# jnbraun/bcnn

Hardware: AMD Instinct MI355X
Metric: images/sec fwd+bwd (higher is better)
Workload: dtype f32; 1 GPU; ResNet-18 224x224 (BASELINE configs[2]), N=128 per GPU, fwd+bwd+SGD through bcnn_net C API; CIFAR-example topology + ImageNet stem, fc-1000; batch_per_gpu=128, global_batch=128, parallelism=dp1, comm=none (one rank)

## Files before the change

### bcnn_amd/_lib.py

```python
import ctypes as C
import os
import subprocess

_HERE = os.path.dirname(os.path.abspath(__file__))
LIB_PATH = os.environ.get("BCNN_HIP_LIB", os.path.join(_HERE, "lib", "libbcnn_hip.so"))
CSRC = os.path.join(_HERE, "csrc")

vp, i, f, sz, u64 = C.c_void_p, C.c_int, C.c_float, C.c_size_t, C.c_uint64

SIGNATURES = {
    "bcnn_hip_device_count": (i, []),
    "bcnn_hip_set_device": (None, [i]),
    "bcnn_hip_get_device": (i, []),
    "bcnn_hip_device_name": (C.c_char_p, []),
    "bcnn_hip_malloc_f32": (vp, [sz]),
    "bcnn_hip_malloc_i32": (vp, [sz]),
    "bcnn_hip_free": (None, [vp]),
    "bcnn_hip_memcpy_h2d": (None, [vp, vp, sz]),
    "bcnn_hip_memcpy_d2h": (None, [vp, vp, sz]),
    "bcnn_hip_memcpy_d2d": (None, [vp, vp, sz]),
    "bcnn_hip_fill_f32": (None, [vp, sz, f]),
    "bcnn_hip_sync": (None, []),
    "bcnn_hip_stream_create": (vp, []),
    "bcnn_hip_stream_destroy": (None, [vp]),
    "bcnn_hip_set_stream": (None, [vp]),
    "bcnn_hip_get_stream": (vp, []),
    "bcnn_hip_event_create": (vp, []),
    "bcnn_hip_event_destroy": (None, [vp]),
    "bcnn_hip_event_record": (None, [vp]),
    "bcnn_hip_event_sync": (None, [vp]),
    "bcnn_hip_event_elapsed_ms": (f, [vp, vp]),
    "bcnn_hip_profile_enable": (None, [i]),
    "bcnn_hip_profile_reset": (None, []),
    "bcnn_hip_profile_num_classes": (i, []),
    "bcnn_hip_profile_class_name": (C.c_char_p, [i]),
    "bcnn_hip_profile_read": (None, [i, C.POINTER(C.c_double), C.POINTER(C.c_longlong), C.POINTER(C.c_double), C.POINTER(C.c_double)]),
    "bcnn_hip_profile_read_useful_flops": (C.c_double, [i]),
    "bcnn_hip_conv_side_stream_mode": (i, [i]),
    "bcnn_hip_conv_side_join": (None, []),
    "bcnn_hip_trace_enable": (None, [i]),
    "bcnn_hip_trace_read": (C.c_size_t, [C.c_char_p, C.c_size_t]),
    "bcnn_hip_axpy": (None, [sz, f, vp, vp]),
    "bcnn_hip_scal": (None, [sz, f, vp]),
    "bcnn_hip_copy_f32": (None, [sz, vp, vp]),
    "bcnn_hip_add_bias": (None, [vp, vp, i, i, i]),
    "bcnn_hip_grad_bias": (None, [vp, vp, i, i, i]),
    "bcnn_hip_scales": (None, [vp, vp, i, i, i]),
    "bcnn_hip_grad_scales": (None, [vp, vp, i, i, i, vp]),
    "bcnn_hip_gemm": (None, [i, i, i, i, i, f, vp, i, vp, i, f, vp, i]),
    "bcnn_hip_im2col": (None, [vp, i, i, i, i, i, i, vp]),
    "bcnn_hip_col2im": (None, [vp, i, i, i, i, i, i, vp]),
    "bcnn_hip_activation_forward": (None, [vp, sz, i, vp, i, i]),
    "bcnn_hip_activation_backward": (None, [vp, vp, sz, i, vp, vp, i, i]),
    "bcnn_hip_batchnorm_forward": (None, [vp] * 10 + [i, i, i, i, i]),
    "bcnn_hip_batchnorm_backward": (None, [vp, vp, vp, i] + [vp] * 9 + [i, i, i]),
    "bcnn_hip_conv_workspace_size": (sz, [i] * 9),
    "bcnn_hip_conv_forward": (None, [vp, vp, vp, vp] + [i] * 10 + [vp, i, vp, vp, vp, vp, vp, vp, vp, i]),
    "bcnn_hip_conv_forward_bf16": (i, [vp, vp, vp, vp] + [i] * 10 + [vp, i, vp, vp, vp, vp, vp, vp, vp, i]),
    "bcnn_hip_conv_backward": (None, [vp] * 8 + [i] * 10 + [vp, vp, i] + [vp] * 8 + [vp, sz]),
    "bcnn_hip_maxpool_forward": (None, [vp, vp, vp] + [i] * 8),
    "bcnn_hip_maxpool_backward": (None, [vp, vp, vp] + [i] * 9),
    "bcnn_hip_avgpool_forward": (None, [vp, vp, i, i, i, i]),
    "bcnn_hip_avgpool_backward": (None, [vp, vp, i, i, i, i]),
    "bcnn_hip_depthwise_forward": (None, [vp, vp, vp, vp] + [i] * 8),
    "bcnn_hip_depthwise_backward": (None, [vp] * 7 + [i] * 9),
    "bcnn_hip_depthwise_stats_size": (sz, [i] * 7),
    "bcnn_hip_depthwise_forward_stats": (i, [vp, vp, vp, vp] + [i] * 8 + [vp, sz]),
    "bcnn_hip_batchnorm_forward_stats": (None, [vp] * 10 + [i, i, i, i, i, vp, i]),
    "bcnn_hip_batchnorm_forward_stats_only": (None, [vp] * 7 + [i, i, i, vp, i]),
    "bcnn_hip_conv_bnfold_fusable": (i, [i] * 5), "bcnn_hip_conv_set_input_bnfold": (None, [vp] * 4),
    "bcnn_hip_depthwise_bn_fusable": (i, [i] * 8),
    "bcnn_hip_batchnorm_backward_sums": (None, [vp] * 9 + [i, i, i]),
    "bcnn_hip_depthwise_backward_bn": (None, [vp] * 7 + [i] * 9 + [vp] * 5),
    "bcnn_hip_batchnorm_backward_apply": (None, [vp] * 8 + [i, i, i]),
    "bcnn_hip_depthwise_bnin_fusable": (i, [i] * 9),
    "bcnn_hip_conv_bnsums_size": (sz, [i] * 4),
    "bcnn_hip_conv_backward_bnsums": (i, [vp] * 8 + [i] * 10 + [vp, vp, i] + [vp] * 8 + [vp, sz] + [vp, vp, vp, sz]),
    "bcnn_hip_batchnorm_backward_finalize": (None, [vp, i] + [vp] * 6 + [i]),
    "bcnn_hip_depthwise_forward_bnin": (i, [vp, vp, vp, vp] + [i] * 8 + [vp, sz] + [vp] * 4 + [i]),
    "bcnn_hip_depthwise_backward_bnin": (None, [vp] * 7 + [i] * 9 + [vp] * 4 + [i]),
    "bcnn_hip_depthwise_backward_bn_bnin": (None, [vp] * 7 + [i] * 9 + [vp] * 5 + [vp] * 4 + [i]),
    "bcnn_hip_conv_residual_fusable": (i, [i, i, i, i, vp, vp, vp]),
    "bcnn_hip_conv_forward_residual": (None, [vp, vp, vp] + [i] * 9 + [vp] * 7 + [sz, i, vp]),
    "bcnn_hip_conv_backward_residual": (None, [vp] * 7 + [i] * 9 + [vp] * 7 + [vp, sz, vp, vp, i, vp, vp, sz]),
    "bcnn_hip_batchnorm_apply": (None, [vp] * 6 + [i, i, i, i]),
    "bcnn_hip_conv_prepack": (None, [vp, i, i]),
    "bcnn_hip_maxpool_forward_bn_keep": (None, [vp, vp, vp] + [i] * 8 + [vp] * 4 + [i, vp]),
    "bcnn_hip_maxpool_bn_backward_fusable": (i, [i] * 9 + [vp] * 4),
    "bcnn_hip_maxpool_bn_backward": (None, [vp] * 5 + [i] * 8 + [vp] * 8 + [i]),
    "bcnn_hip_conv_backward_bn_done": (None, [vp] * 5 + [i] * 9 + [vp, sz]),
    "bcnn_hip_depthwise_insums_size": (sz, [i] * 7),
    "bcnn_hip_depthwise_backward_bnin_sums": (i, [vp] * 7 + [i] * 9 + [vp] * 5 + [vp] * 4 + [i] + [vp, sz]),
    "bcnn_hip_conv_backward_presummed": (i, [vp] * 8 + [i] * 10 + [vp, vp, i] + [vp] * 8 + [vp, sz] + [vp, i] + [vp, vp, vp, sz]),
    "bcnn_hip_conv_prepack_reset": (None, []),
    "bcnn_hip_conv_prepack_discard": (None, []),
    "bcnn_hip_maxpool_bn_fusable": (i, [i] * 9 + [vp]),
    "bcnn_hip_conv_forward_stats_only": (None, [vp, vp, vp] + [i] * 9 + [vp] * 6),
    "bcnn_hip_maxpool_forward_bn": (None, [vp, vp, vp] + [i] * 8 + [vp] * 4 + [i]),
    "bcnn_hip_sgd_update": (None, [vp, vp, vp, vp, sz, sz, i, f, f, f]),
    "bcnn_hip_sgd_update_chunks": (None, [vp, i, i, f, f, f]),
    "bcnn_hip_zero_chunks": (None, [vp, i]),
    "bcnn_hip_adam_update": (None, [vp, vp, vp, vp, vp, vp, sz, sz, i, i, f, f, f, f, f]),
    "bcnn_hip_eltwise_forward": (None, [vp, vp, vp, sz, sz, i]),
    "bcnn_hip_eltwise_backward": (None, [vp, vp, vp, vp, sz, sz, i, i]),
    "bcnn_hip_cost_metric": (None, [i, vp, vp, vp, i, i, vp]),
    "bcnn_hip_axpy_strided": (None, [i, f, vp, vp] + [i] * 11),
    "bcnn_hip_add_rowvec": (None, [vp, vp, i, i]),
    "bcnn_hip_softmax_forward": (None, [vp, vp, i, i, i]),
    "bcnn_hip_concat_forward": (None, [i, vp, vp, vp, i, i]),
    "bcnn_hip_concat_backward": (None, [i, vp, vp, vp, i, i]),
    "bcnn_hip_upsample_forward": (None, [vp, vp, i, i, i, i, i]),
    "bcnn_hip_upsample_backward": (None, [vp, vp, i, i, i, i, i]),
    "bcnn_hip_yolo_activate": (None, [vp, vp, i, i, i, i, i]),
    "bcnn_hip_yolo_nms_capacity": (i, []),
    "bcnn_hip_yolo_detect_result_words": (sz, [i, i, i]),
    "bcnn_hip_yolo_detect_batch": (i, [vp, i, i, vp, i, i, i, i, f, i, f, i, i, vp]),
    "bcnn_hip_yolo_train_workspace_size": (sz, [vp]),
    "bcnn_hip_yolo_train_forward": (i, [vp, vp, vp, vp, vp, vp, vp]),
    "bcnn_hip_fill_images": (i, [vp, i, i, i, i, i, vp, vp, vp, vp, i, f, i, f, f, f]),
    "bcnn_hip_jpeg_stage_begin": (i, [i, i, i, i, i, vp, i, vp, vp]),
    "bcnn_hip_jpeg_stage_run": (i, [vp, f, i, f, f, f]),
    "bcnn_hip_jpeg_stage_cancel": (None, []),
    "bcnn_hip_augment_batch": (i, [vp, i, i, i, i, i, i, i, vp, vp, vp, i]),
    "bcnn_hip_augment_jpeg_begin": (i, [i, i, i, i, i, vp, vp]),
    "bcnn_hip_augment_jpeg_run": (i, [vp, vp, vp, vp, vp, vp, i]),
    "bcnn_hip_augment_jpeg_cancel": (None, []),
    "bcnn_hip_augment_letterbox_batch": (i, [vp, i, i, i, i, i, vp, vp, vp, i]),
    "bcnn_hip_augment_effects_begin": (i, [i, i, i, vp, vp, vp, vp, i, vp, sz]),
    "bcnn_hip_augment_effects_cancel": (None, []),
    "bcnn_hip_deconv_workspace_size": (sz, [i] * 8),
    "bcnn_hip_deconv_forward": (None, [vp, vp, vp, vp] + [i] * 9),
    "bcnn_hip_deconv_backward": (None, [vp] * 7 + [i] * 9 + [vp, sz]),
    "bcnn_hip_lrn_forward": (None, [vp, vp] + [i] * 5 + [f] * 3),
    "bcnn_hip_lrn_backward": (None, [vp, vp, vp] + [i] * 5 + [f] * 3 + [i]),
    "bcnn_hip_dropout_forward": (None, [vp, sz, f, u64, u64]),
    "bcnn_hip_dropout_backward": (None, [vp, sz, f, u64, u64]),
    "bcnn_hip_lifted_struct_workspace_size": (sz, [i, i]),
    "bcnn_hip_lifted_struct_forward": (None, [vp, vp, vp, i, i, f, i, vp, vp]),
    "bcnn_hip_lifted_struct_backward": (None, [vp, i, i, f, vp]),
    "bcnn_hip_comm_init": (None, [i, i, C.c_char_p]),
    "bcnn_hip_comm_destroy": (None, []),
    "bcnn_hip_comm_retain": (None, []),
    "bcnn_hip_rendezvous_publish": (i, [C.c_char_p, vp, sz, i]),
    "bcnn_hip_rendezvous_fetch": (i, [C.c_char_p, vp, sz, i, i]),
    "bcnn_hip_comm_world": (i, []),
    "bcnn_hip_comm_rank": (i, []),
    "bcnn_hip_allreduce_sum": (None, [vp, sz]),
    "bcnn_hip_broadcast": (None, [vp, sz, i]),
    "bcnn_hip_comm_join": (None, []),
}

_lib = None


def build(verbose=False):
    out = None if verbose else subprocess.DEVNULL
    subprocess.check_call(["make", "-C", CSRC, "-j8"], stdout=out)
    return LIB_PATH


def load():
    global _lib
    if _lib is not None:
        return _lib
    try:
        import torch
    except ImportError:
        pass
    if not os.path.exists(LIB_PATH):
        raise RuntimeError(
            "bcnn_amd: %s is missing -- build it with `python -c 'import __graft_entry__ as g; g.build()'` "
            "(there is no CPU fallback)" % LIB_PATH)
    lib = C.CDLL(LIB_PATH)
    for name, (res, args) in SIGNATURES.items():
        fn = getattr(lib, name)
        fn.restype = res
        fn.argtypes = args
    _lib = lib
    return lib


def declared_symbols():
    import re
    hdr = os.path.join(os.path.dirname(_HERE), "include", "bcnn_hip.h")
    text = open(hdr).read()
    text = re.sub(r"/\*.*?\*/", "", text, flags=re.S)
    return sorted(set(re.findall(r"\b(bcnn_hip_[a-z0-9_]+)\s*\(", text)))
```

### bcnn_amd/csrc/batchnorm.hip

```cpp
#include "chan_reduce.h"
#include "batchnorm.h"
#include "bn_math.h"

namespace bcnn_hip {

#ifdef NT_STORES
#define BN_ST4(p, v) do { typedef float f4_ __attribute__((ext_vector_type(4))); const f4_ t_ = {(v).x, (v).y, (v).z, (v).w}; \
                          __builtin_nontemporal_store(t_, reinterpret_cast<f4_*>(p)); } while (0)
#else
#define BN_ST4(p, v) (*reinterpret_cast<float4*>(p) = (v))
#endif


static float4* bn_consts_scratch(int channels) {
    if (BCNN_EXP_ENV("BCNN_HIP_BN_NO_CONSTS")) return nullptr;
    return scratch_f4(SCRATCH_BN_CONSTS, (size_t)channels * 3);
}
__device__ __forceinline__ void bn_fwd_consts_store(float4* consts, int c, float mean, float var, const float* scale,
                                                    const float* bias) {
    if (!consts) return;
    const BnDiv rs = bn_divisor(sqrtf(var + 0.000001f));
    consts[2 * c] = make_float4(mean, rs.d, rs.r, scale[c]);
    consts[2 * c + 1] = make_float4(bias[c], 0.f, 0.f, 0.f);
}
__device__ __forceinline__ void bn_bwd_consts_store(float4* consts, int c, const float* mean, float var, float sc,
                                                    const float* fwd_bias, float dmean, float dvar, float fM) {
    if (!consts) return;
    const BnDiv rs5 = bn_divisor(sqrtf(var + 0.00001f)), rs6 = bn_divisor(sqrtf(var + 0.000001f));
    consts[3 * c] = make_float4(mean[c], sc, rs5.d, rs5.r);
    consts[3 * c + 1] = make_float4(rs6.d, rs6.r, fwd_bias ? fwd_bias[c] : 0.f, __fdiv_rn(dmean, fM));
    consts[3 * c + 2] = make_float4(dvar, 0.f, 0.f, 0.f);
}

struct StatsF {
    static constexpr int kInFlight = 4;
    const float* x;
    __device__ void operator()(long long off, int, float (&acc)[2]) const {
        const float v = x[off];
        acc[0] += v;
        acc[1] += v * v;
    }
    __device__ void vec4(long long off, int, float (&acc)[2]) const {
        const float4 v = *reinterpret_cast<const float4*>(x + off);
        acc[0] += (v.x + v.y) + (v.z + v.w);
        acc[1] += (v.x * v.x + v.y * v.y) + (v.z * v.z + v.w * v.w);
    }
};

__global__ void bn_stats_finalize_kernel(const float* __restrict__ partials, int C, int splits, int M,
                                         float* __restrict__ saved_mean, float* __restrict__ saved_var,
                                         float* __restrict__ run_mean, float* __restrict__ run_var,
                                         float4* __restrict__ consts, const float* __restrict__ scale,
                                         const float* __restrict__ bias, const float* __restrict__ mean_shift) {
    const int c = blockIdx.x * blockDim.x + threadIdx.x;
    if (c >= C) return;
    double s = 0.0, ss = 0.0;
    for (int i = 0; i < splits; ++i) {
        s += (double)partials[((long long)c * splits + i) * 2 + 0];
        ss += (double)partials[((long long)c * splits + i) * 2 + 1];
    }
    const float inv = 1.0f / (float)M;
    const float mean = __fmul_rn((float)s, inv);
    const float var = __fsub_rn(__fmul_rn((float)ss, inv), __fmul_rn(mean, mean));
    saved_mean[c] = mean;
    saved_var[c] = var;
    const float vis = mean_shift ? __fadd_rn(mean, mean_shift[c]) : mean;
    run_mean[c] = __fadd_rn(__fmul_rn(vis, 0.1f), __fmul_rn(run_mean[c], 0.9f));
    run_var[c] = __fadd_rn(__fmul_rn(var, 0.1f), __fmul_rn(run_var[c], 0.9f));
    bn_fwd_consts_store(consts, c, mean, var, scale, bias);
}

constexpr int kFinalizeThreads = 1024;
__global__ __launch_bounds__(kFinalizeThreads) void bn_stats_finalize_wide_kernel(
    const float* __restrict__ partials, int C, int splits, int M, float* __restrict__ saved_mean,
    float* __restrict__ saved_var, float* __restrict__ run_mean, float* __restrict__ run_var,
    float4* __restrict__ consts, const float* __restrict__ scale, const float* __restrict__ bias,
    const float* __restrict__ mean_shift) {
    constexpr int NW = kFinalizeThreads / 64;
    __shared__ double red[NW][2];
    const int lane = threadIdx.x & 63, wid = threadIdx.x >> 6;
    const int c = blockIdx.x;
    const float2* p = reinterpret_cast<const float2*>(partials) + (long long)c * splits;
    double s = 0.0, ss = 0.0;
    int i = threadIdx.x;
    for (; i + 3 * kFinalizeThreads < splits; i += 4 * kFinalizeThreads) {
        const float2 v0 = p[i], v1 = p[i + kFinalizeThreads], v2 = p[i + 2 * kFinalizeThreads], v3 = p[i + 3 * kFinalizeThreads];
        s += ((double)v0.x + (double)v1.x) + ((double)v2.x + (double)v3.x);
        ss += ((double)v0.y + (double)v1.y) + ((double)v2.y + (double)v3.y);
    }
    for (; i < splits; i += kFinalizeThreads) {
        const float2 v = p[i];
        s += (double)v.x;
        ss += (double)v.y;
    }
#pragma unroll
    for (int o = 32; o > 0; o >>= 1) { s += __shfl_xor(s, o); ss += __shfl_xor(ss, o); }
    if (lane == 0) { red[wid][0] = s; red[wid][1] = ss; }
    __syncthreads();
    if (threadIdx.x != 0) return;
    s = 0.0;
    ss = 0.0;
    for (int w = 0; w < NW; ++w) { s += red[w][0]; ss += red[w][1]; }
    const float inv = 1.0f / (float)M;
    const float mean = __fmul_rn((float)s, inv);
    const float var = __fsub_rn(__fmul_rn((float)ss, inv), __fmul_rn(mean, mean));
    saved_mean[c] = mean;
    saved_var[c] = var;
    const float vis = mean_shift ? __fadd_rn(mean, mean_shift[c]) : mean;
    run_mean[c] = __fadd_rn(__fmul_rn(vis, 0.1f), __fmul_rn(run_mean[c], 0.9f));
    run_var[c] = __fadd_rn(__fmul_rn(var, 0.1f), __fmul_rn(run_var[c], 0.9f));
    bn_fwd_consts_store(consts, c, mean, var, scale, bias);
}

struct BnApplyArgs {
    const float* x;
    float* y;
    float* ws;
    float* xn;
    const float* mean;
    const float* var;
    const float* scale;
    const float* bias;
    int C, HW, predict, act;
    long long total;
    const float* res;
    unsigned res_count;
    int act2;
    const float4* consts;
};

struct BnApplyBody {
    BnApplyArgs a;
    bool al;
    __device__ void operator()(unsigned off, int c, int cnt) const {
        float mean, sc, b;
        BnDiv rs;
        if (a.consts) {
            const float4 k0 = a.consts[2 * c], k1 = a.consts[2 * c + 1];
            mean = k0.x; rs.d = k0.y; rs.r = k0.z; sc = k0.w; b = k1.x;
        } else {
            mean = a.predict ? 0.f : a.mean[c];
            rs = bn_divisor(a.predict ? 1.f : sqrtf(a.var[c] + 0.000001f));
            sc = a.scale[c]; b = a.bias[c];
        }
        const bool side_ws = a.ws && a.ws != a.x, side_xn = a.xn && !a.predict;
        if (cnt == 4 && al && (off & 3u) == 0) {
            const float4 xv = *reinterpret_cast<const float4*>(a.x + off);
            float4 yv, nv;
            yv.x = bn_one(xv.x, mean, rs, sc, b, a.predict, a.act, &nv.x);
            yv.y = bn_one(xv.y, mean, rs, sc, b, a.predict, a.act, &nv.y);
            yv.z = bn_one(xv.z, mean, rs, sc, b, a.predict, a.act, &nv.z);
            yv.w = bn_one(xv.w, mean, rs, sc, b, a.predict, a.act, &nv.w);
            if (side_ws) *reinterpret_cast<float4*>(a.ws + off) = xv;
            if (side_xn) *reinterpret_cast<float4*>(a.xn + off) = nv;
            if (a.res) {
                if (off + 4 <= a.res_count) {
                    const float4 r = *reinterpret_cast<const float4*>(a.res + off);
                    yv.x += r.x; yv.y += r.y; yv.z += r.z; yv.w += r.w;
                } else if (off < a.res_count) {
                    yv.x += a.res[off];
                    if (off + 1 < a.res_count) yv.y += a.res[off + 1];
                    if (off + 2 < a.res_count) yv.z += a.res[off + 2];
                }
                yv.x = act_fwd_cheap(yv.x, a.act2, 0.f); yv.y = act_fwd_cheap(yv.y, a.act2, 0.f);
                yv.z = act_fwd_cheap(yv.z, a.act2, 0.f); yv.w = act_fwd_cheap(yv.w, a.act2, 0.f);
            }
            BN_ST4(a.y + off, yv);
        } else {
            for (int k = 0; k < cnt; ++k) {
                const float xv = a.x[off + k];
                float nv = 0.f;
                float yv = bn_one(xv, mean, rs, sc, b, a.predict, a.act, &nv);
                if (a.res) yv = act_fwd_cheap(yv + (off + k < a.res_count ? a.res[off + k] : 0.f), a.act2, 0.f);
                if (side_ws) a.ws[off + k] = xv;
                if (side_xn) a.xn[off + k] = nv;
                a.y[off + k] = yv;
            }
        }
    }
};

__device__ __forceinline__ float bn_recompute_y(float x, float m, const BnDiv& rs, float sc, float b, int act, const float* res,
                                                unsigned res_count, unsigned long long off) {
    float dummy;
    if (!res) return bn_one(x, m, rs, sc, b, 0, act, &dummy);
    float v = bn_one(x, m, rs, sc, b, 0, BCNN_HIP_ACT_NONE, &dummy);
    if (off < res_count) v += res[off];
    return act_fwd_cheap(v, act, 0.f);
}

struct BwdSumsF {
    static constexpr int kInFlight = 2;
    const float* dy;
    const float* y;
    const float* x;
    const float* mean;
    const float* fwd_bias;
    const float* var;
    const float* scale;
    int act, C, HW;
    const float* res;
    unsigned res_count;
    __device__ float fwd_y(float xv, int c, long long off) const {
        return bn_recompute_y(xv, mean[c], bn_divisor(sqrtf(var[c] + 0.000001f)), scale[c], fwd_bias[c], act, res, res_count,
                              (unsigned long long)off);
    }
    __device__ void operator()(long long off, int c, float (&acc)[2]) const {
        float g = dy[off];
        const float xv = x[off];
        if (act != BCNN_HIP_ACT_NONE) g *= act_bwd_cheap(fwd_bias ? fwd_y(xv, c, off) : y[off], act, 0.f);
        acc[0] += g;
        acc[1] += g * (xv - mean[c]);
    }
    __device__ void vec4(long long off, int c, float (&acc)[2]) const {
        const float m = mean[c];
        float4 g = *reinterpret_cast<const float4*>(dy + off);
        const float4 xv = *reinterpret_cast<const float4*>(x + off);
        if (act != BCNN_HIP_ACT_NONE) {
            float4 yv;
            if (fwd_bias) {
                const BnDiv rs = bn_divisor(sqrtf(var[c] + 0.000001f));
                const float sc = scale[c], b = fwd_bias[c];
                const unsigned long long o = (unsigned long long)off;
                yv.x = bn_recompute_y(xv.x, m, rs, sc, b, act, res, res_count, o);
                yv.y = bn_recompute_y(xv.y, m, rs, sc, b, act, res, res_count, o + 1);
                yv.z = bn_recompute_y(xv.z, m, rs, sc, b, act, res, res_count, o + 2);
                yv.w = bn_recompute_y(xv.w, m, rs, sc, b, act, res, res_count, o + 3);
            } else {
                yv = *reinterpret_cast<const float4*>(y + off);
            }
            g.x *= act_bwd_cheap(yv.x, act, 0.f); g.y *= act_bwd_cheap(yv.y, act, 0.f);
            g.z *= act_bwd_cheap(yv.z, act, 0.f); g.w *= act_bwd_cheap(yv.w, act, 0.f);
        }
        acc[0] += (g.x + g.y) + (g.z + g.w);
        acc[1] += (g.x * (xv.x - m) + g.y * (xv.y - m)) + (g.z * (xv.z - m) + g.w * (xv.w - m));
    }
};

__global__ void bn_bwd_finalize_kernel(const float* __restrict__ partials, int C, int splits,
                                       const float* __restrict__ scale, const float* __restrict__ var,
                                       float* __restrict__ dbias, float* __restrict__ dscales,
                                       float* __restrict__ dmean, float* __restrict__ dvar,
                                       float4* __restrict__ consts, const float* __restrict__ mean,
                                       const float* __restrict__ fwd_bias, float fM) {
    const int c = blockIdx.x * blockDim.x + threadIdx.x;
    if (c >= C) return;
    double s1 = 0.0, s2 = 0.0;
    for (int i = 0; i < splits; ++i) {
        s1 += (double)partials[((long long)c * splits + i) * 2 + 0];
        s2 += (double)partials[((long long)c * splits + i) * 2 + 1];
    }
    const float v = var[c], sc = scale[c];
    dbias[c] += (float)s1;
    dscales[c] += (float)(s2 / (double)sqrtf(v + 0.000001f));
    float md = (float)(s1 * (double)sc);
    float vd = (float)(s2 * (double)sc);
    md *= (-1.0f / sqrtf(v + 0.00001f));
    vd *= -0.5f / (v * sqrtf(v) + 0.00001f);
    dmean[c] = md;
    dvar[c] = vd;
    bn_bwd_consts_store(consts, c, mean, v, sc, fwd_bias, md, vd, fM);
}

__global__ __launch_bounds__(1024) void bn_bwd_finalize_wide_kernel(const float* __restrict__ partials, int C, int splits,
                                                                   const float* __restrict__ scale,
                                                                   const float* __restrict__ var, float* __restrict__ dbias,
                                                                   float* __restrict__ dscales, float* __restrict__ dmean,
                                                                   float* __restrict__ dvar, float4* __restrict__ consts,
                                                                   const float* __restrict__ mean,
                                                                   const float* __restrict__ fwd_bias, float fM) {
    __shared__ double red[16][2];
    const int lane = threadIdx.x & 63, wid = threadIdx.x >> 6, c = blockIdx.x;
    const float2* p = reinterpret_cast<const float2*>(partials) + (long long)c * splits;
    double s1 = 0.0, s2 = 0.0;
    int i = threadIdx.x;
    for (; i + 3 * 1024 < splits; i += 4 * 1024) {
        const float2 v0 = p[i], v1 = p[i + 1024], v2 = p[i + 2048], v3 = p[i + 3072];
        s1 += ((double)v0.x + (double)v1.x) + ((double)v2.x + (double)v3.x);
        s2 += ((double)v0.y + (double)v1.y) + ((double)v2.y + (double)v3.y);
    }
    for (; i < splits; i += 1024) {
        const float2 v = p[i];
        s1 += (double)v.x;
        s2 += (double)v.y;
    }
#pragma unroll
    for (int o = 32; o > 0; o >>= 1) { s1 += __shfl_xor(s1, o); s2 += __shfl_xor(s2, o); }
    if (lane == 0) { red[wid][0] = s1; red[wid][1] = s2; }
    __syncthreads();
    if (threadIdx.x != 0) return;
    s1 = 0.0;
    s2 = 0.0;
    for (int w = 0; w < 16; ++w) { s1 += red[w][0]; s2 += red[w][1]; }
    const float v = var[c], sc = scale[c];
    dbias[c] += (float)s1;
    dscales[c] += (float)(s2 / (double)sqrtf(v + 0.000001f));
    float md = (float)(s1 * (double)sc);
    float vd = (float)(s2 * (double)sc);
    md *= (-1.0f / sqrtf(v + 0.00001f));
    vd *= -0.5f / (v * sqrtf(v) + 0.00001f);
    dmean[c] = md;
    dvar[c] = vd;
    bn_bwd_consts_store(consts, c, mean, v, sc, fwd_bias, md, vd, fM);
}

struct BnBwdApplyArgs {
    float* dy;
    float* dx;
    const float* y;
    const float* x;
    const float* mean;
    const float* var;
    const float* scale;
    const float* dmean;
    const float* dvar;
    const float* fwd_bias;
    int C, HW, act, M;
    long long total;
    int keep_dy;
    const float* res;
    unsigned res_count;
    const float4* consts;
    float rM;
};

struct BnBwdApplyBody {
    BnBwdApplyArgs a;
    bool al;
    __device__ void operator()(unsigned off, int c, int cnt) const {
        const BnDiv fM{(float)a.M, a.rM};
        const bool use_act = a.act != BCNN_HIP_ACT_NONE, use_y = use_act && a.fwd_bias == nullptr;
        float mean, sc, fb, dmm, dv;
        BnDiv rs, rs_fwd;
        if (a.consts) {
            const float4 k0 = a.consts[3 * c], k1 = a.consts[3 * c + 1], k2 = a.consts[3 * c + 2];
            mean = k0.x; sc = k0.y; rs.d = k0.z; rs.r = k0.w;
            rs_fwd.d = k1.x; rs_fwd.r = k1.y; fb = k1.z; dmm = k1.w; dv = k2.x;
        } else {
            mean = a.mean[c]; sc = a.scale[c];
            rs = bn_divisor(sqrtf(a.var[c] + 0.00001f));
            rs_fwd = bn_divisor(use_act && !use_y ? sqrtf(a.var[c] + 0.000001f) : 1.0f);
            fb = a.fwd_bias ? a.fwd_bias[c] : 0.f;
            dmm = __fdiv_rn(a.dmean[c], fM.d); dv = a.dvar[c];
        }
        if (cnt == 4 && al && (off & 3u) == 0) {
            const float4 g = *reinterpret_cast<const float4*>(a.dy + off);
            const float4 xv = *reinterpret_cast<const float4*>(a.x + off);
            float4 yv = make_float4(0.f, 0.f, 0.f, 0.f);
            if (use_y) yv = *reinterpret_cast<const float4*>(a.y + off);
            else if (use_act) {
                yv.x = bn_recompute_y(xv.x, mean, rs_fwd, sc, fb, a.act, a.res, a.res_count, off);
                yv.y = bn_recompute_y(xv.y, mean, rs_fwd, sc, fb, a.act, a.res, a.res_count, off + 1ull);
                yv.z = bn_recompute_y(xv.z, mean, rs_fwd, sc, fb, a.act, a.res, a.res_count, off + 2ull);
                yv.w = bn_recompute_y(xv.w, mean, rs_fwd, sc, fb, a.act, a.res, a.res_count, off + 3ull);
            }
            float4 o;
            o.x = bn_bwd_one(g.x, yv.x, xv.x, mean, rs, sc, dmm, dv, fM, a.act);
            o.y = bn_bwd_one(g.y, yv.y, xv.y, mean, rs, sc, dmm, dv, fM, a.act);
            o.z = bn_bwd_one(g.z, yv.z, xv.z, mean, rs, sc, dmm, dv, fM, a.act);
            o.w = bn_bwd_one(g.w, yv.w, xv.w, mean, rs, sc, dmm, dv, fM, a.act);
            if (!a.keep_dy) BN_ST4(a.dy + off, o);
            if (a.dx) BN_ST4(a.dx + off, o);
        } else {
            for (int k = 0; k < cnt; ++k) {
                const float xk = a.x[off + k];
                const float yk = use_y ? a.y[off + k]
                                       : (use_act ? bn_recompute_y(xk, mean, rs_fwd, sc, fb, a.act, a.res, a.res_count, off + k) : 0.f);
                const float o = bn_bwd_one(a.dy[off + k], yk, xk, mean, rs, sc, dmm, dv, fM, a.act);
                if (!a.keep_dy) a.dy[off + k] = o;
                if (a.dx) a.dx[off + k] = o;
            }
        }
    }
};

void batchnorm_forward_impl(const BnFwdCall& f) {
    const int n = f.e.n, c = f.e.c, hw = f.e.hw, mode = f.mode;
    const long long M = (long long)n * hw, total = M * c;
    if (!total) return;
    const bool have_pre = f.pre && f.pre->splits > 0 && mode == BCNN_HIP_MODE_TRAIN;
    KTimer kt(K_BN_FWD, 0.0, 4.0 * ((have_pre ? 0.0 : 1.0) + (f.stats_only ? 0.0 : 2.0)) * (double)total);
    const int act = act_is_cheap(f.act) ? f.act : BCNN_HIP_ACT_NONE;
    BnApplyArgs a;
    a.x = f.x; a.y = f.y; a.ws = f.workspace; a.xn = f.x_norm; a.scale = f.p.scales; a.bias = f.p.bias;
    a.C = c; a.HW = hw; a.act = act; a.total = total;
    a.res = nullptr; a.res_count = 0; a.act2 = BCNN_HIP_ACT_NONE;
    if (f.res) {
        a.res = f.res->res;
        a.res_count = (unsigned)(f.res->count < (size_t)total ? f.res->count : (size_t)total);
        a.act2 = f.res->act;
    }
    a.predict = (mode == BCNN_HIP_MODE_PREDICT);
    a.mean = f.run.run_mean; a.var = f.run.run_var;
    a.consts = nullptr;
    float4* consts = (mode == BCNN_HIP_MODE_TRAIN && !f.stats_only) ? bn_consts_scratch(c) : nullptr;
    if (mode == BCNN_HIP_MODE_PREDICT) a.ws = nullptr;
    if (mode == BCNN_HIP_MODE_VALID) a.xn = nullptr;
    if (mode == BCNN_HIP_MODE_TRAIN) {
        if (have_pre) {
            bn_stats_finalize_wide_kernel<<<c, kFinalizeThreads, 0, current_stream()>>>(
                f.pre->partials, c, f.pre->splits, (int)M, f.saved_mean, f.saved_var, f.run.run_mean, f.run.run_var, consts,
                f.p.scales, f.p.bias, f.mean_shift);
        } else {
            const int splits = chan_splits(c, M);
            float* part = scratch(SCRATCH_REDUCE, (size_t)c * splits * 2);
            launch_chan_reduce<2>(StatsF{f.x}, c, hw, M, splits, part);
            bn_stats_finalize_kernel<<<ceil_div(c, 256), 256, 0, current_stream()>>>(
                part, c, splits, (int)M, f.saved_mean, f.saved_var, f.run.run_mean, f.run.run_var, consts, f.p.scales, f.p.bias,
                f.mean_shift);
        }
        KERNEL_CHECK();
        a.mean = f.saved_mean; a.var = f.saved_var; a.consts = consts;
    }
    if (f.stats_only) return;
#ifdef BCNN_HIP_EXPERIMENT
    static const int skip_fw = getenv("BCNN_HIP_SKIP_SWEEPS") ? atoi(getenv("BCNN_HIP_SKIP_SWEEPS")) : 0;
    if (!(skip_fw & 4))
#endif
    launch_chan_map(BnApplyBody{a, al16(f.x) && al16(f.y) && al16(a.ws) && al16(a.xn) && al16(a.res)}, n, c, hw);
    if (f.act != act) bcnn_hip_activation_forward(f.y, (size_t)total, f.act, nullptr, hw, c);
}

}

using namespace bcnn_hip;

extern "C" {

void bcnn_hip_batchnorm_forward_stats(const float* x, float* y, float* run_mean, float* run_var, const float* scales,
                                      const float* bias, float* saved_mean, float* saved_var, float* x_norm,
                                      float* workspace, int n, int c, int hw, int mode, int act, const float* stats,
                                      int splits) {
    ConvStats st;
    st.partials = const_cast<float*>(stats); st.splits = stats ? splits : 0; st.capacity = 0;
    BnFwdCall f{};
    f.x = x; f.y = y; f.workspace = workspace; f.x_norm = x_norm; f.mode = mode; f.act = act; f.pre = &st;
    f.e.n = n; f.e.c = c; f.e.hw = hw; f.p.scales = scales; f.p.bias = bias;
    f.saved_mean = saved_mean; f.saved_var = saved_var; f.run.run_mean = run_mean; f.run.run_var = run_var;
    batchnorm_forward_impl(f);
}

void bcnn_hip_batchnorm_forward(const float* x, float* y, float* run_mean, float* run_var,
                                const float* scales, const float* bias, float* saved_mean,
                                float* saved_var, float* x_norm, float* workspace, int n, int c, int hw,
                                int mode, int act) {
    bcnn_hip_batchnorm_forward_stats(x, y, run_mean, run_var, scales, bias, saved_mean, saved_var, x_norm, workspace, n, c, hw,
                                     mode, act, nullptr, 0);
}

void bcnn_hip_batchnorm_forward_stats_only(const float* x, float* run_mean, float* run_var, const float* scales,
                                           const float* bias, float* saved_mean, float* saved_var, int n, int c, int hw,
                                           const float* stats, int splits) {
    ConvStats st;
    st.partials = const_cast<float*>(stats); st.splits = stats ? splits : 0; st.capacity = 0;
    BnFwdCall f{};
    f.x = x; f.mode = BCNN_HIP_MODE_TRAIN; f.act = BCNN_HIP_ACT_NONE; f.pre = &st; f.stats_only = true;
    f.e.n = n; f.e.c = c; f.e.hw = hw; f.p.scales = scales; f.p.bias = bias;
    f.saved_mean = saved_mean; f.saved_var = saved_var; f.run.run_mean = run_mean; f.run.run_var = run_var;
    batchnorm_forward_impl(f);
}

}

namespace bcnn_hip {
void batchnorm_backward_sums(const BnBwdCall& b) {
    const int c = b.e.c, hw = b.e.hw;
    const long long M = (long long)b.e.n * hw;
    const int splits = chan_splits(c, M);
    float* part = scratch(SCRATCH_REDUCE, (size_t)c * splits * 2);
    BwdSumsF f;
    f.dy = b.dout ? b.dout : b.dy; f.y = b.y; f.x = b.workspace; f.mean = b.s.mean; f.act = b.act; f.C = c; f.HW = hw;
    f.fwd_bias = b.p.bias; f.var = b.s.var; f.scale = b.p.scales; f.res = b.res; f.res_count = (unsigned)b.res_count;
#ifdef BCNN_HIP_EXPERIMENT
    static const int skip_exp = getenv("BCNN_HIP_SKIP_C1_SUMS") ? 1 : 0;
    static const int skip_all = getenv("BCNN_HIP_SKIP_SWEEPS") ? atoi(getenv("BCNN_HIP_SKIP_SWEEPS")) : 0;
    if (!(skip_all & 1))
    if (!(skip_exp && b.res == nullptr && b.act == BCNN_HIP_ACT_RELU && ((hw == 3136 && c == 64) || (hw == 784 && c == 128))))
#endif
    launch_chan_reduce<2>(f, c, hw, M, splits, part);
    bn_bwd_finalize_kernel<<<ceil_div(c, 256), 256, 0, current_stream()>>>(part, c, splits, b.p.scales, b.s.var, b.g.dbias,
                                                                          b.g.dscales, b.g.dmean, b.g.dvar, b.consts, b.s.mean,
                                                                          b.p.bias, b.consts_fM > 0.f ? b.consts_fM : (float)M);
    KERNEL_CHECK();
}

static void batchnorm_backward_apply(const BnBwdCall& b) {
    const long long M = (long long)b.e.n * b.e.hw, total = M * b.e.c;
    BnBwdApplyArgs a;
    a.consts = b.consts;
    a.rM = 1.0f / (float)M;
    a.dy = b.dout ? const_cast<float*>(b.dout) : b.dy;
    a.dx = (b.dx && b.dx != a.dy) ? b.dx : nullptr; a.y = b.y; a.x = b.workspace;
    a.mean = b.s.mean; a.var = b.s.var; a.scale = b.p.scales; a.dmean = b.g.dmean; a.dvar = b.g.dvar;
    a.C = b.e.c; a.HW = b.e.hw; a.act = b.act; a.M = (int)M; a.total = total; a.fwd_bias = b.p.bias;
    a.keep_dy = b.dout != nullptr; a.res = b.res; a.res_count = (unsigned)b.res_count;
#ifdef BCNN_HIP_EXPERIMENT
    static const int skip_bw = getenv("BCNN_HIP_SKIP_SWEEPS") ? atoi(getenv("BCNN_HIP_SKIP_SWEEPS")) : 0;
    if (skip_bw & 2) return;
#endif
    launch_chan_map(BnBwdApplyBody{a, al16(a.dy) && al16(a.dx) && al16(b.workspace) && al16(b.y)}, b.e.n, b.e.c, b.e.hw);
}

__global__ __launch_bounds__(256) void bn_residual_grad_kernel(const float* __restrict__ out, const float* __restrict__ dout,
                                                               float* __restrict__ dres, unsigned count, int act) {
    for (unsigned i = blockIdx.x * 256u + threadIdx.x; i < count; i += gridDim.x * 256u)
        dres[i] += dout[i] * act_bwd_cheap(out[i], act, 0.f);
}

void batchnorm_backward_impl(const BnBwdCall& call) {
    BnBwdCall b = call;
    const int c = b.e.c, hw = b.e.hw;
    const long long M = (long long)b.e.n * hw, total = M * c;
    if (!total) return;
    if (!b.dout && (b.act == BCNN_HIP_ACT_NONE || !act_bwd_is_cheap(b.act))) b.p.bias = nullptr;
    const bool reads_y = b.act != BCNN_HIP_ACT_NONE && !b.p.bias;
    KTimer kt(K_BN_BWD, 0.0, 4.0 * (b.dout ? 5.0 : b.sums ? (reads_y ? 4.0 : 3.0) : (reads_y ? 7.0 : 5.0)) * (double)total);
    if (b.dout) {
        b.res_count = b.res_count < (size_t)total ? b.res_count : (size_t)total;
        if (b.dres && b.res_count) {
            bn_residual_grad_kernel<<<stream_grid(b.res_count, 256), 256, 0, current_stream()>>>(b.y, b.dout, b.dres,
                                                                                                 (unsigned)b.res_count, b.act);
            KERNEL_CHECK();
        }
    } else if (!act_bwd_is_cheap(b.act)) {
        bcnn_hip_activation_backward(b.y, b.dy, (size_t)total, b.act, nullptr, nullptr, hw, c);
        b.act = BCNN_HIP_ACT_NONE;
    }
    b.consts = bn_consts_scratch(c);
    if (b.sums) {
        bn_bwd_finalize_wide_kernel<<<c, 1024, 0, current_stream()>>>(b.sums, c, b.splits, b.p.scales, b.s.var, b.g.dbias, b.g.dscales,
                                                                      b.g.dmean, b.g.dvar, b.consts, b.s.mean, b.p.bias, (float)M);
        KERNEL_CHECK();
    } else {
        batchnorm_backward_sums(b);
    }
    batchnorm_backward_apply(b);
}

}

extern "C" {

void bcnn_hip_batchnorm_apply(const float* x, float* y, const float* scales, const float* bias, const float* saved_mean,
                              const float* saved_var, int n, int c, int hw, int act) {
    const long long total = (long long)n * hw * c;
    if (!total) return;
    BnApplyArgs a;
    a.x = x; a.y = y; a.ws = nullptr; a.xn = nullptr; a.scale = scales; a.bias = bias; a.mean = saved_mean; a.var = saved_var;
    a.C = c; a.HW = hw; a.act = act_is_cheap(act) ? act : BCNN_HIP_ACT_NONE; a.total = total; a.predict = 0;
    a.res = nullptr; a.res_count = 0; a.act2 = BCNN_HIP_ACT_NONE; a.consts = nullptr;
    launch_chan_map(BnApplyBody{a, al16(x) && al16(y)}, n, c, hw);
    if (a.act != act) bcnn_hip_activation_forward(y, (size_t)total, act, nullptr, hw, c);
}

void bcnn_hip_batchnorm_backward_finalize(const float* sums, int splits, const float* scales, float* dscales, float* dbias,
                                          const float* saved_var, float* dmean, float* dvar, int c) {
    if (c <= 0 || splits <= 0) return;
    bn_bwd_finalize_wide_kernel<<<c, 1024, 0, current_stream()>>>(sums, c, splits, scales, saved_var, dbias, dscales, dmean,
                                                                  dvar, nullptr, nullptr, nullptr, 1.0f);
    KERNEL_CHECK();
}

void bcnn_hip_batchnorm_backward_sums(const float* dy, const float* scales, float* dscales, float* dbias,
                                      const float* saved_mean, const float* saved_var, float* dmean, float* dvar,
                                      const float* x, int n, int c, int hw) {
    const long long total = (long long)n * hw * c;
    if (!total) return;
    KTimer kt(K_BN_BWD, 0.0, 4.0 * 2.0 * (double)total);
    BnBwdCall b{};
    b.dout = dy; b.workspace = x; b.act = BCNN_HIP_ACT_NONE; b.e.n = n; b.e.c = c; b.e.hw = hw;
    b.p.scales = scales; b.s.mean = saved_mean; b.s.var = saved_var;
    b.g.dscales = dscales; b.g.dbias = dbias; b.g.dmean = dmean; b.g.dvar = dvar;
    batchnorm_backward_sums(b);
}

void bcnn_hip_batchnorm_backward_apply(float* dy, float* dx, const float* scales, const float* saved_mean,
                                       const float* saved_var, const float* dmean, const float* dvar, const float* x,
                                       int n, int c, int hw) {
    if (!(long long)n * hw * c) return;
    BnBwdCall b{};
    b.dy = dy; b.dx = dx; b.workspace = x; b.act = BCNN_HIP_ACT_NONE; b.e.n = n; b.e.c = c; b.e.hw = hw;
    b.p.scales = scales; b.s.mean = saved_mean; b.s.var = saved_var;
    b.g.dmean = const_cast<float*>(dmean); b.g.dvar = const_cast<float*>(dvar);
    batchnorm_backward_apply(b);
}

void bcnn_hip_batchnorm_backward(float* dy, float* dx, const float* y, int act, const float* scales,
                                 float* dscales, float* dbias, const float* saved_mean,
                                 const float* saved_var, float* dmean, float* dvar, const float* x_norm,
                                 const float* workspace, int n, int c, int hw) {
    (void)x_norm;
    BnBwdCall b{};
    b.dy = dy; b.dx = dx; b.y = y; b.workspace = workspace; b.act = act; b.e.n = n; b.e.c = c; b.e.hw = hw;
    b.p.scales = scales; b.s.mean = saved_mean; b.s.var = saved_var;
    b.g.dscales = dscales; b.g.dbias = dbias; b.g.dmean = dmean; b.g.dvar = dvar;
    batchnorm_backward_impl(b);
}

}
```

### bcnn_amd/csrc/next.hip

```cpp
#include <cfloat>

#include "chan_reduce.h"
#include "common.h"

namespace bcnn_hip {

__global__ __launch_bounds__(256) void axpy_strided_kernel(float a, const float* __restrict__ x, float* __restrict__ y,
                                                           int sy, int sx, int xc, int xh, int xw, int yc, int yh,
                                                           int yw, int mc, int mh, int mw, unsigned total) {
    const unsigned gs = gridDim.x * blockDim.x;
    for (unsigned t = blockIdx.x * blockDim.x + threadIdx.x; t < total; t += gs) {
        const unsigned i = t % (unsigned)mw, t1 = t / (unsigned)mw;
        const unsigned j = t1 % (unsigned)mh, t2 = t1 / (unsigned)mh;
        const unsigned k = t2 % (unsigned)mc, n = t2 / (unsigned)mc;
        const size_t di = (size_t)i * sy + (size_t)yw * ((size_t)j * sy + (size_t)yh * ((size_t)yc * n + k));
        const size_t si = (size_t)i * sx + (size_t)xw * ((size_t)j * sx + (size_t)xh * ((size_t)xc * n + k));
        y[di] += a * x[si];
    }
}

__global__ __launch_bounds__(256) void add_rowvec_kernel(float* __restrict__ y, const float* __restrict__ v, int cols,
                                                         unsigned total) {
    const unsigned gs = gridDim.x * blockDim.x;
    for (unsigned t = blockIdx.x * blockDim.x + threadIdx.x; t < total; t += gs) y[t] += v[t % (unsigned)cols];
}

__global__ __launch_bounds__(256) void eltwise_fwd_kernel(const float* __restrict__ a, const float* __restrict__ b,
                                                          float* __restrict__ y, size_t n, size_t b_count, int act) {
    const size_t stride = (size_t)gridDim.x * blockDim.x * 4;
    for (size_t i = ((size_t)blockIdx.x * blockDim.x + threadIdx.x) * 4; i < n; i += stride) {
        if (i + 4 <= n) {
            float4 v = *reinterpret_cast<const float4*>(a + i);
            if (i + 4 <= b_count) {
                const float4 w = *reinterpret_cast<const float4*>(b + i);
                v.x += w.x; v.y += w.y; v.z += w.z; v.w += w.w;
            } else if (i < b_count) {
                if (i < b_count) v.x += b[i];
                if (i + 1 < b_count) v.y += b[i + 1];
                if (i + 2 < b_count) v.z += b[i + 2];
            }
            v.x = act_fwd_cheap(v.x, act, 0.f); v.y = act_fwd_cheap(v.y, act, 0.f);
            v.z = act_fwd_cheap(v.z, act, 0.f); v.w = act_fwd_cheap(v.w, act, 0.f);
            *reinterpret_cast<float4*>(y + i) = v;
        } else {
            for (size_t k = i; k < n; ++k) y[k] = act_fwd_cheap(a[k] + (k < b_count ? b[k] : 0.f), act, 0.f);
        }
    }
}

__global__ __launch_bounds__(256) void eltwise_bwd_kernel(const float* __restrict__ y, float* __restrict__ dy,
                                                          float* __restrict__ da, float* __restrict__ db, size_t n,
                                                          size_t b_count, int act, int overwrite_a) {
    const size_t stride = (size_t)gridDim.x * blockDim.x * 4;
    for (size_t i = ((size_t)blockIdx.x * blockDim.x + threadIdx.x) * 4; i < n; i += stride) {
        if (i + 4 <= n) {
            float4 g = *reinterpret_cast<const float4*>(dy + i);
            if (act != BCNN_HIP_ACT_NONE) {
                const float4 yv = *reinterpret_cast<const float4*>(y + i);
                g.x *= act_bwd_cheap(yv.x, act, 0.f); g.y *= act_bwd_cheap(yv.y, act, 0.f);
                g.z *= act_bwd_cheap(yv.z, act, 0.f); g.w *= act_bwd_cheap(yv.w, act, 0.f);
                *reinterpret_cast<float4*>(dy + i) = g;
            }
            if (da) {
                float4 t = overwrite_a ? make_float4(0.f, 0.f, 0.f, 0.f) : *reinterpret_cast<const float4*>(da + i);
                t.x += g.x; t.y += g.y; t.z += g.z; t.w += g.w;
                *reinterpret_cast<float4*>(da + i) = t;
            }
            if (db && i < b_count) {
                if (i + 4 <= b_count) {
                    float4 t = *reinterpret_cast<const float4*>(db + i);
                    t.x += g.x; t.y += g.y; t.z += g.z; t.w += g.w;
                    *reinterpret_cast<float4*>(db + i) = t;
                } else {
                    db[i] += g.x;
                    if (i + 1 < b_count) db[i + 1] += g.y;
                    if (i + 2 < b_count) db[i + 2] += g.z;
                }
            }
        } else {
            for (size_t k = i; k < n; ++k) {
                float gk = dy[k];
                if (act != BCNN_HIP_ACT_NONE) { gk *= act_bwd_cheap(y[k], act, 0.f); dy[k] = gk; }
                if (da) da[k] = (overwrite_a ? 0.f : da[k]) + gk;
                if (db && k < b_count) db[k] += gk;
            }
        }
    }
}

__global__ __launch_bounds__(256) void softmax_kernel(const float* __restrict__ x, float* __restrict__ y, int C, int HW,
                                                      unsigned total) {
    const int lane = threadIdx.x & 63;
    const unsigned wave = blockIdx.x * 4u + (threadIdx.x >> 6), nwaves = gridDim.x * 4u;
    for (unsigned t = wave; t < total; t += nwaves) {
        const unsigned i = t % (unsigned)HW, n = t / (unsigned)HW;
        const float* px = x + (size_t)n * C * HW + i;
        float* py = y + (size_t)n * C * HW + i;
        float vmax = -FLT_MAX;
        for (int c = lane; c < C; c += 64) vmax = fmaxf(vmax, px[(size_t)c * HW]);
#pragma unroll
        for (int o = 32; o > 0; o >>= 1) vmax = fmaxf(vmax, __shfl_xor(vmax, o));
        double part = 0.0;
        for (int c = lane; c < C; c += 64) part += (double)(float)exp((double)(px[(size_t)c * HW] - vmax));
#pragma unroll
        for (int o = 32; o > 0; o >>= 1) part += __shfl_xor(part, o);
        float sum = (float)part;
        sum = (sum != 0.f) ? vmax + (float)log((double)sum) : vmax - 100.0f;
        for (int c = lane; c < C; c += 64) py[(size_t)c * HW] = (float)exp((double)(px[(size_t)c * HW] - sum));
    }
}

__global__ __launch_bounds__(1024) void cost_metric_kernel(int metric, const float* __restrict__ pred,
                                                           const float* __restrict__ label,
                                                           const float* __restrict__ grad, int B, int per,
                                                           double* __restrict__ partials) {
    __shared__ double red[16];
    const int lane = threadIdx.x & 63, wave = threadIdx.x >> 6;
    const int nrow = 16 * gridDim.x, row0 = blockIdx.x * 16 + wave;
    double acc = 0.0;
    if (metric == 0) {
        for (int i = row0; i < B; i += nrow) {
            const float* row = pred + (size_t)i * per;
            float pm = FLT_MIN;
            int best = 0;
            for (int j = lane; j < per; j += 64)
                if (row[j] > pm) { pm = row[j]; best = j; }
#pragma unroll
            for (int off = 32; off > 0; off >>= 1) {
                const float om = __shfl_xor(pm, off);
                const int ob = __shfl_xor(best, off);
                if (om > pm || (om == pm && ob < best)) { pm = om; best = ob; }
            }
            if (lane == 0 && label[(size_t)i * per + best] == 0) acc += 1.0;
        }
    } else if (metric == 5) {
        for (int i = row0; i < B; i += nrow) {
            int n = 0, d = 0;
            for (int j = lane; j < per; j += 64) {
                const float l = label[(size_t)i * per + j];
                const float t = pred[(size_t)i * per + j] > 0.5f ? 1.f : 0.f;
                n += (int)(l * t);
                d += (int)(l + t);
            }
#pragma unroll
            for (int off = 32; off > 0; off >>= 1) { n += __shfl_xor(n, off); d += __shfl_xor(d, off); }
            if (lane == 0) acc += (2.0f * n + 1.0f) / (d + 1.0f);
        }
    } else {
        const size_t sz = (size_t)B * per;
        for (size_t i = (size_t)blockIdx.x * 1024 + threadIdx.x; i < sz; i += (size_t)gridDim.x * 1024) {
            if (metric == 1) {
                if (label[i] > 0.0f) {
                    float q = pred[i];
                    q = q < 1e-8f ? 1e-8f : (q > 1.0f - 1e-8f ? 1.0f - 1e-8f : q);
                    acc += -log((double)q);
                }
            } else {
                acc += (double)grad[i] * grad[i];
            }
        }
#pragma unroll
        for (int off = 32; off > 0; off >>= 1) acc += __shfl_xor(acc, off);
    }
    if (lane == 0) red[wave] = acc;
    __syncthreads();
    if (threadIdx.x == 0) {
        double t = 0.0;
        for (int w = 0; w < 16; ++w) t += red[w];
        partials[blockIdx.x] = t;
    }
}
__global__ void cost_metric_final_kernel(int metric, const double* __restrict__ partials, int n, int per,
                                         float* __restrict__ out) {
    double t = 0.0;
    for (int i = 0; i < n; ++i) t += partials[i];
    out[0] = (float)(metric == 3 ? t / per : t);
}

}

using namespace bcnn_hip;

extern "C" {

void bcnn_hip_axpy_strided(int num_batches, float a, const float* x, float* y, int stride_y, int stride_x, int x_c,
                           int x_h, int x_w, int y_c, int y_h, int y_w, int min_c, int min_h, int min_w) {
    const long long total = (long long)num_batches * min_c * min_h * min_w;
    if (total <= 0) return;
    axpy_strided_kernel<<<stream_grid((size_t)total, 256), 256, 0, current_stream()>>>(
        a, x, y, stride_y, stride_x, x_c, x_h, x_w, y_c, y_h, y_w, min_c, min_h, min_w, (unsigned)total);
    KERNEL_CHECK();
}

void bcnn_hip_add_rowvec(float* y, const float* v, int rows, int cols) {
    const long long total = (long long)rows * cols;
    if (total <= 0) return;
    add_rowvec_kernel<<<stream_grid((size_t)total, 256), 256, 0, current_stream()>>>(y, v, cols, (unsigned)total);
    KERNEL_CHECK();
}

void bcnn_hip_softmax_forward(const float* x, float* y, int n, int c, int hw) {
    const long long total = (long long)n * hw;
    if (total <= 0) return;
    softmax_kernel<<<stream_grid((size_t)total * 64, 256), 256, 0, current_stream()>>>(x, y, c, hw, (unsigned)total);
    KERNEL_CHECK();
}

static bool aligned16(const void* p) { return p == nullptr || (reinterpret_cast<uintptr_t>(p) & 15) == 0; }

void bcnn_hip_eltwise_forward(const float* a, const float* b, float* y, size_t n, size_t b_count, int act) {
    if (!n) return;
    if (!act_is_cheap(act) || !aligned16(a) || !aligned16(b) || !aligned16(y)) {
        bcnn_hip_copy_f32(n, a, y);
        bcnn_hip_axpy(b_count, 1.0f, b, y);
        bcnn_hip_activation_forward(y, n, act, nullptr, 1, 1);
        return;
    }
    eltwise_fwd_kernel<<<stream_grid(n / 4 + 1, 256), 256, 0, current_stream()>>>(a, b, y, n, b_count, act);
    KERNEL_CHECK();
}

void bcnn_hip_eltwise_backward(const float* y, float* dy, float* da, float* db, size_t n, size_t b_count, int act,
                               int overwrite_a) {
    if (!n) return;
    if (!act_bwd_is_cheap(act) || !aligned16(y) || !aligned16(dy) || !aligned16(da) || !aligned16(db)) {
        bcnn_hip_activation_backward(y, dy, n, act, nullptr, nullptr, 1, 1);
        if (da && overwrite_a) bcnn_hip_fill_f32(da, n, 0.f);
        if (da) bcnn_hip_axpy(n, 1.0f, dy, da);
        if (db) bcnn_hip_axpy(b_count, 1.0f, dy, db);
        return;
    }
    eltwise_bwd_kernel<<<stream_grid(n / 4 + 1, 256), 256, 0, current_stream()>>>(y, dy, da, db, n, b_count, act,
                                                                                   overwrite_a);
    KERNEL_CHECK();
}

void bcnn_hip_cost_metric(int metric, const float* pred, const float* label, const float* grad, int batch, int per,
                          float* out) {
    const long long sz = (long long)batch * per;
    int blocks = (int)((sz + 8191) / 8192);
    if (blocks > 64) blocks = 64;
    if (blocks < 1) blocks = 1;
    double* partials = reinterpret_cast<double*>(scratch(SCRATCH_REDUCE, 2 * 64));
    cost_metric_kernel<<<blocks, 1024, 0, current_stream()>>>(metric, pred, label, grad, batch, per, partials);
    KERNEL_CHECK();
    cost_metric_final_kernel<<<1, 1, 0, current_stream()>>>(metric, partials, blocks, per, out);
    KERNEL_CHECK();
}

}
```

### bcnn_amd/csrc/runtime.hip

```cpp
#include "common.h"

#include <cstring>
#include <vector>

namespace bcnn_hip {
static thread_local hipStream_t g_stream = nullptr;
hipStream_t current_stream() { return g_stream; }
void set_current_stream(hipStream_t st) { g_stream = st; }

int current_device() {
    int dev = 0;
    HIP_CHECK(hipGetDevice(&dev));
    if (dev < 0 || dev >= kMaxDevices) { fprintf(stderr, "[bcnn_hip] device ordinal %d out of range\n", dev); exit(1); }
    return dev;
}

struct ScratchPolicy { size_t min_floats; unsigned grow_num, grow_den; };
static constexpr ScratchPolicy kScratchPolicy[] = {
     {1u << 16, 2, 1},
     {4096 * 4, 2, 1},
     {8192, 2, 1},
     {0, 1, 1},
     {1u << 20, 3, 2},
     {1u << 20, 3, 2},
     {0, 1, 1},
     {0, 1, 1},
     {1u << 20, 1, 1},
     {0, 1, 1},
     {1u << 20, 1, 1},
     {0, 1, 1},
     {1u << 20, 1, 1},
     {0, 1, 1},
     {1u << 16, 1, 1},
     {1u << 18, 5, 4},
     {1u << 18, 1, 1},
};
static_assert(sizeof(kScratchPolicy) / sizeof(kScratchPolicy[0]) == SCRATCH_SLOTS, "one policy row per ScratchSlot");
struct ScratchBlock { float* p = nullptr; size_t cap = 0; };
static thread_local ScratchBlock g_scratch[kMaxDevices][SCRATCH_SLOTS];

float* scratch(ScratchSlot slot, size_t floats) {
    ScratchBlock& b = g_scratch[current_device()][slot];
    if (b.p == nullptr || b.cap < floats) {
        const ScratchPolicy& pol = kScratchPolicy[slot];
        if (b.p) {
            HIP_CHECK(hipDeviceSynchronize());
            HIP_CHECK(hipFree(b.p));
        }
        b.cap = floats < pol.min_floats ? pol.min_floats : floats * pol.grow_num / pol.grow_den;
        HIP_CHECK(hipMalloc((void**)&b.p, b.cap * sizeof(float)));
    }
    return b.p;
}

struct KRecord { int cls; hipEvent_t a, b; double flops, bytes, useful; };
static thread_local bool g_prof_on = false;
static thread_local std::vector<KRecord>* g_records = nullptr;
static thread_local std::vector<hipEvent_t>* g_event_pool = nullptr;
static hipEvent_t pool_event() {
    if (!g_event_pool) g_event_pool = new std::vector<hipEvent_t>();
    if (!g_event_pool->empty()) { hipEvent_t e = g_event_pool->back(); g_event_pool->pop_back(); return e; }
    hipEvent_t e;
    HIP_CHECK(hipEventCreate(&e));
    return e;
}
KTimer::KTimer(int cls, double flops, double bytes, double useful_flops) : idx(-1) {
    if (!g_prof_on) return;
    if (!g_records) g_records = new std::vector<KRecord>();
    KRecord r{cls, pool_event(), pool_event(), flops, bytes, useful_flops < 0 ? flops : useful_flops};
    HIP_CHECK(hipEventRecord(r.a, g_stream));
    idx = (int)g_records->size();
    g_records->push_back(r);
}
KTimer::~KTimer() {
    if (idx >= 0) HIP_CHECK(hipEventRecord((*g_records)[idx].b, g_stream));
}

thread_local bool g_trace_on = false;
static thread_local std::vector<char>* g_trace_log = nullptr;
void trace_kernel_slow(const char* name) {
    if (!g_trace_log) g_trace_log = new std::vector<char>();
    if (g_trace_log->size() > (8u << 20)) return;
    g_trace_log->insert(g_trace_log->end(), name, name + strlen(name));
    g_trace_log->push_back('\n');
}

__global__ void warm_kernel(float* p) { if (p && threadIdx.x == 0) p[0] = 1.0f; }

static void warm_device_keeping_rand_state() {
    static thread_local unsigned long long warmed = 0;
    static thread_local bool any = false;
    int dev = 0;
    if (any) {
        if (hipGetDevice(&dev) != hipSuccess || dev < 0 || dev >= 64 || ((warmed >> dev) & 1ull)) return;
    }
    char scratch_state[256];
    char* user_state = initstate(1u, scratch_state, sizeof(scratch_state));
    void* p = nullptr;
    (void)hipFree(nullptr);
    if (hipGetDevice(&dev) != hipSuccess) dev = 0;
    if (hipMalloc(&p, 256) == hipSuccess) {
        float h = 0.f;
        (void)hipMemsetAsync(p, 0, 256, nullptr);
        warm_kernel<<<1, 64, 0, nullptr>>>((float*)p);
        (void)hipMemcpy(&h, p, sizeof(float), hipMemcpyDeviceToHost);
        (void)hipDeviceSynchronize();
        (void)hipFree(p);
    }
    (void)hipDeviceSynchronize();
    if (user_state) setstate(user_state);
    any = true;
    if (dev >= 0 && dev < 64) warmed |= 1ull << dev;
}

__global__ void fill_f32_kernel(float* __restrict__ x, size_t n, float v) {
    size_t head = ((16 - (reinterpret_cast<uintptr_t>(x) & 15)) & 15) / 4;
    if (head > n) head = n;
    const size_t i = (size_t)blockIdx.x * blockDim.x + threadIdx.x;
    const size_t stride = (size_t)gridDim.x * blockDim.x;
    if (i < head) x[i] = v;
    float* body = x + head;
    const size_t nb = n - head, n4 = nb / 4;
    float4* b4 = reinterpret_cast<float4*>(body);
    const float4 v4 = make_float4(v, v, v, v);
    for (size_t j = i; j < n4; j += stride) b4[j] = v4;
    for (size_t j = n4 * 4 + i; j < nb; j += stride) body[j] = v;
}
}

using namespace bcnn_hip;

extern "C" {

int bcnn_hip_device_count(void) {
    int n = 0;
    if (hipGetDeviceCount(&n) != hipSuccess) return 0;
    return n;
}

void bcnn_hip_set_device(int id) {
    HIP_CHECK(hipSetDevice(id));
    warm_device_keeping_rand_state();
}

int bcnn_hip_get_device(void) {
    int id = 0;
    HIP_CHECK(hipGetDevice(&id));
    return id;
}

const char* bcnn_hip_device_name(void) {
    static thread_local char name[256];
    hipDeviceProp_t prop;
    HIP_CHECK(hipGetDeviceProperties(&prop, bcnn_hip_get_device()));
    snprintf(name, sizeof(name), "%s", prop.gcnArchName);
    return name;
}

float* bcnn_hip_malloc_f32(size_t n) {
    float* p = nullptr;
    if (n == 0) return nullptr;
    warm_device_keeping_rand_state();
    HIP_CHECK(hipMalloc((void**)&p, n * sizeof(float)));
    HIP_CHECK(hipMemsetAsync(p, 0, n * sizeof(float), current_stream()));
    return p;
}

int* bcnn_hip_malloc_i32(size_t n) {
    int* p = nullptr;
    if (n == 0) return nullptr;
    warm_device_keeping_rand_state();
    HIP_CHECK(hipMalloc((void**)&p, n * sizeof(int)));
    HIP_CHECK(hipMemsetAsync(p, 0, n * sizeof(int), current_stream()));
    return p;
}

void bcnn_hip_free(void* p) {
    if (p) HIP_CHECK(hipFree(p));
}

void bcnn_hip_memcpy_h2d(void* dst, const void* src, size_t bytes) {
    HIP_CHECK(hipMemcpyAsync(dst, src, bytes, hipMemcpyHostToDevice, current_stream()));
    HIP_CHECK(hipStreamSynchronize(current_stream()));
}

void bcnn_hip_memcpy_d2h(void* dst, const void* src, size_t bytes) {
    HIP_CHECK(hipMemcpyAsync(dst, src, bytes, hipMemcpyDeviceToHost, current_stream()));
    HIP_CHECK(hipStreamSynchronize(current_stream()));
}

void bcnn_hip_memcpy_d2d(void* dst, const void* src, size_t bytes) {
    HIP_CHECK(hipMemcpyAsync(dst, src, bytes, hipMemcpyDeviceToDevice, current_stream()));
}

void bcnn_hip_fill_f32(float* x, size_t n, float value) {
    if (n == 0) return;
    if (value == 0.0f) {
        HIP_CHECK(hipMemsetAsync(x, 0, n * sizeof(float), current_stream()));
        return;
    }
    fill_f32_kernel<<<stream_grid(n / 4 + 1, 256), 256, 0, current_stream()>>>(x, n, value);
    KERNEL_CHECK();
}

void bcnn_hip_sync(void) { HIP_CHECK(hipStreamSynchronize(current_stream())); }

void* bcnn_hip_stream_create(void) {
    hipStream_t s;
    warm_device_keeping_rand_state();
    int prio_lo = 0, prio_hi = 0;
    HIP_CHECK(hipDeviceGetStreamPriorityRange(&prio_lo, &prio_hi));
    HIP_CHECK(hipStreamCreateWithPriority(&s, hipStreamNonBlocking, prio_hi));
    return (void*)s;
}

void bcnn_hip_stream_destroy(void* stream) {
    if (stream) HIP_CHECK(hipStreamDestroy((hipStream_t)stream));
}

void bcnn_hip_set_stream(void* stream) { g_stream = (hipStream_t)stream; }
void* bcnn_hip_get_stream(void) { return (void*)g_stream; }

void* bcnn_hip_event_create(void) {
    hipEvent_t e;
    HIP_CHECK(hipEventCreate(&e));
    return (void*)e;
}

void bcnn_hip_event_destroy(void* ev) {
    if (ev) HIP_CHECK(hipEventDestroy((hipEvent_t)ev));
}

void bcnn_hip_event_record(void* ev) { HIP_CHECK(hipEventRecord((hipEvent_t)ev, current_stream())); }
void bcnn_hip_event_sync(void* ev) { HIP_CHECK(hipEventSynchronize((hipEvent_t)ev)); }

float bcnn_hip_event_elapsed_ms(void* start, void* stop) {
    float ms = 0.f;
    HIP_CHECK(hipEventElapsedTime(&ms, (hipEvent_t)start, (hipEvent_t)stop));
    return ms;
}

void bcnn_hip_profile_enable(int on) { g_prof_on = (on != 0); }

void bcnn_hip_profile_reset(void) {
    if (!g_records) return;
    HIP_CHECK(hipStreamSynchronize(current_stream()));
    for (auto& r : *g_records) { g_event_pool->push_back(r.a); g_event_pool->push_back(r.b); }
    g_records->clear();
}

int bcnn_hip_profile_num_classes(void) { return K_NUM; }

const char* bcnn_hip_profile_class_name(int cls) {
    static const char* names[K_NUM] = {"conv_fwd", "conv_dw", "conv_dx", "bn_fwd", "bn_bwd", "pool",
                                       "eltwise_act", "gemm", "sgd", "depthwise_fwd", "depthwise_bwd",
                                       "conv_fwd_winograd", "conv_dx_winograd", "conv_dw_winograd",
                                       "conv_fwd_winograd43", "conv_dx_winograd43", "conv_dw_winograd43"};
    return (cls >= 0 && cls < K_NUM) ? names[cls] : "?";
}

void bcnn_hip_profile_read(int cls, double* ms, long long* launches, double* flops, double* bytes) {
    double t = 0, f = 0, b = 0;
    long long n = 0;
    if (g_records) {
        HIP_CHECK(hipStreamSynchronize(current_stream()));
        for (auto& r : *g_records) {
            if (r.cls != cls) continue;
            float e = 0.f;
            HIP_CHECK(hipEventElapsedTime(&e, r.a, r.b));
            t += e; f += r.flops; b += r.bytes; ++n;
        }
    }
    if (ms) *ms = t;
    if (launches) *launches = n;
    if (flops) *flops = f;
    if (bytes) *bytes = b;
}

void bcnn_hip_trace_enable(int on) {
    g_trace_on = (on != 0);
    if (on && g_trace_log) g_trace_log->clear();
}

size_t bcnn_hip_trace_read(char* buf, size_t cap) {
    const size_t len = g_trace_log ? g_trace_log->size() : 0;
    if (buf && cap > 0) {
        const size_t n = len < cap - 1 ? len : cap - 1;
        if (n) memcpy(buf, g_trace_log->data(), n);
        buf[n] = 0;
    }
    return len;
}

double bcnn_hip_profile_read_useful_flops(int cls) {
    double u = 0;
    if (g_records)
        for (auto& r : *g_records)
            if (r.cls == cls) u += r.useful;
    return u;
}

}
```

### bcnn_amd/host/bcnn_core.c

```c
#include <math.h>
#include <stdarg.h>
#include <string.h>

#include "bcnn_internal.h"
#include "../../include/bcnn_hip.h"

#ifndef BCNN_USE_HIP
#error "this runtime is the device build: compile with -DBCNN_USE_HIP"
#endif

void bcnn_log(bcnn_log_context ctx, bcnn_log_level level, const char *fmt, ...) {
    if (level < ctx.lvl) return;
    char msg[2048];
    va_list ap;
    va_start(ap, fmt);
    vsnprintf(msg, sizeof(msg), fmt, ap);
    va_end(ap);
    if (ctx.fct) {
        ctx.fct("%s", msg);
        return;
    }
    static const char *tag[] = {"[INFO] ", "[WARNING] ", "[ERROR] ", ""};
    fprintf(stderr, "%s%s", tag[level > 3 ? 3 : level], msg);
}
// ... 101 lines not shown

static bcnn_hip_context *hctx(bcnn_net *net) { return (bcnn_hip_context *)net->hip_ctx; }

bcnn_status bcnn_net_add_tensor(bcnn_net *net, bcnn_tensor tensor) {
    bcnn_tensor *p = (bcnn_tensor *)realloc(net->tensors, (size_t)(net->num_tensors + 1) * sizeof(bcnn_tensor));
    if (!p) return BCNN_FAILED_ALLOC;
    net->tensors = p;
    net->tensors[net->num_tensors++] = tensor;
    return BCNN_SUCCESS;
}

static void invalidate_sgd_table(bcnn_net *net) {
    bcnn_hip_context *hc = hctx(net);
    if (!hc) return;
    if (hc->sgd_chunks_gpu) {
        bcnn_hip_sync();
        bcnn_hip_free(hc->sgd_chunks_gpu);
        hc->sgd_chunks_gpu = NULL;
    }
    hc->num_sgd_chunks = 0;
    if (hc->fill_chunks_gpu) {
        bcnn_hip_sync();
        bcnn_hip_free(hc->fill_chunks_gpu);
        hc->fill_chunks_gpu = NULL;
    }
    hc->num_fill_chunks = -1;
}

static void relink_graph(bcnn_net *net);

bcnn_status bcnn_net_add_node(bcnn_net *net, bcnn_node node) {
    bcnn_hip_context *hc = hctx(net);
    if (hc && hc->compiled) {
        bcnn_materialize_data(net, -1);
        bcnn_materialize_gradients(net, -1);
    }
    bcnn_node *p = (bcnn_node *)realloc(net->nodes, (size_t)(net->num_nodes + 1) * sizeof(bcnn_node));
    if (!p) return BCNN_FAILED_ALLOC;
    net->nodes = p;
    net->nodes[net->num_nodes++] = node;
    invalidate_sgd_table(net);
    if (hc) {
        free(hc->node_grad_first);
        hc->node_grad_first = NULL;
        if (hc->compiled) relink_graph(net);
        else hc->grad_fill_count = 0;
    }
    return BCNN_SUCCESS;
}

static bcnn_status push_index(int **arr, int *count, int index) {
    int *p = (int *)realloc(*arr, (size_t)(*count + 1) * sizeof(int));
    if (!p) return BCNN_FAILED_ALLOC;
    p[(*count)++] = index;
    *arr = p;
    return BCNN_SUCCESS;
}

bcnn_status bcnn_node_add_input(bcnn_net *net, bcnn_node *node, int index) {
    (void)net;
    return push_index(&node->src, &node->num_src, index);
}

bcnn_status bcnn_node_add_output(bcnn_net *net, bcnn_node *node, int index) {
    (void)net;
    return push_index(&node->dst, &node->num_dst, index);
}

int bcnn_net_find_tensor(bcnn_net *net, const char *name) {
    for (int i = net->num_tensors - 1; i >= 0; --i)
        if (net->tensors[i].name && strcmp(net->tensors[i].name, name) == 0) return i;
    return -1;
}

void bcnn_net_register_param(bcnn_net *net, int index) {
    bcnn_hip_context *hc = hctx(net);
    push_index(&hc->param_ids, &hc->num_params, index);
}

bcnn_status bcnn_init_net(bcnn_net **net, bcnn_mode mode) {
    bcnn_net *p = (bcnn_net *)calloc(1, sizeof(bcnn_net));
    if (!p) return BCNN_FAILED_ALLOC;
    p->mode = mode;
    p->hip_ctx = calloc(1, sizeof(bcnn_hip_context));
    if (!p->hip_ctx) { free(p); return BCNN_FAILED_ALLOC; }
    hctx(p)->dp_world = 1;
    hctx(p)->num_fill_chunks = -1;
    bcnn_tensor in = {0}, lab = {0};
    in.name = dup_name("input");
    lab.name = dup_name("label");
    bcnn_net_add_tensor(p, in);
    bcnn_net_add_tensor(p, lab);
    if (mode != BCNN_MODE_PREDICT) {
        p->learner = (bcnn_learner *)calloc(1, sizeof(bcnn_learner));
        p->data_aug = (bcnn_data_augmenter *)calloc(1, sizeof(bcnn_data_augmenter));
    }
    p->num_inputs = 1;
    p->inputs = (int *)calloc(1, sizeof(int));
    p->num_threads = 1;
    *net = p;
    return BCNN_SUCCESS;
}

void bcnn_end_net(bcnn_net **pnet) {
    bcnn_net *net = *pnet;
    if (!net) return;
    bcnn_hip_sync();
    bcnn_hip_conv_prepack_reset();
    bcnn_hip_context *hc = hctx(net);
    if (hc->comm_active) bcnn_hip_comm_destroy();
    if (hc->compiled) {
        for (int i = 0; i < hc->arena_members; ++i) {
            bcnn_tensor *t = &net->tensors[hc->param_ids[i]];
            t->data_gpu = NULL;
            t->grad_data_gpu = NULL;
        }
        bcnn_hip_free(hc->param_arena_gpu);
        bcnn_hip_free(hc->grad_arena_gpu);
        bcnn_hip_free(hc->sgd_chunks_gpu);
        bcnn_hip_free(hc->fill_chunks_gpu);
        free(hc->sgd_chunks_host);
        free(hc->grad_fill_dead);
        free(hc->node_grad_first);
    }
    for (int i = 0; i < net->num_nodes; ++i) {
        bcnn_node *nd = &net->nodes[i];
        if (nd->release_param) nd->release_param(nd);
        free(nd->src); free(nd->dst); free(nd->param);
    }
    free(net->nodes);
    for (int i = 0; i < net->num_tensors; ++i) bcnn_tensor_destroy(&net->tensors[i]);
    free(net->tensors);
    bcnn_hip_free(hc->workspace_gpu);
    bcnn_free_loader_stage(net);
    free(hc->param_ids);
    free(hc);
    free(net->learner); free(net->data_aug); bcnn_destroy_data_loader(net); free(net->inputs);
    free(net);
    *pnet = NULL;
}

bcnn_status bcnn_set_num_threads(bcnn_net *net, int num_threads, const int *cpu_ids) {
    (void)cpu_ids;
    net->num_threads = num_threads > 0 ? num_threads : 1;
    return BCNN_SUCCESS;
}
int bcnn_get_num_threads(bcnn_net *net) { return net->num_threads; }
int bcnn_get_batch_size(bcnn_net *net) { return net->batch_size; }

void bcnn_set_input_shape(bcnn_net *net, int width, int height, int channels, int batch_size) {
    net->batch_size = batch_size;
    bcnn_tensor_set_shape(&net->tensors[0], batch_size, channels, height, width, 0);
}

bcnn_status bcnn_add_input(bcnn_net *net, int width, int height, int channels, const char *name) {
    bcnn_tensor t = {0};
    bcnn_tensor_set_shape(&t, net->batch_size, channels, height, width, 0);
    BCNN_CHECK_STATUS(bcnn_tensor_allocate(&t, net->mode));
    t.name = dup_name(name);
    BCNN_CHECK_STATUS(bcnn_net_add_tensor(net, t));
    int *p = (int *)realloc(net->inputs, (size_t)(net->num_inputs + 1) * sizeof(int));
    if (!p) return BCNN_FAILED_ALLOC;
    net->inputs = p;
    net->inputs[net->num_inputs++] = net->num_tensors - 1;
    return BCNN_SUCCESS;
}

static void build_arenas(bcnn_net *net) {
    bcnn_hip_context *hc = hctx(net);
    size_t total = 0;
    for (int i = 0; i < hc->num_params; ++i) {
        total += ((size_t)bcnn_tensor_size(&net->tensors[hc->param_ids[i]]) + 3) & ~(size_t)3;
    }
    if (total == 0) return;
    float *old_p = hc->param_arena_gpu, *old_g = hc->grad_arena_gpu;
    float *new_p = bcnn_hip_malloc_f32(total);
    float *new_g = (net->mode != BCNN_MODE_PREDICT) ? bcnn_hip_malloc_f32(total) : NULL;
    size_t off = 0;
    for (int i = 0; i < hc->num_params; ++i) {
        bcnn_tensor *t = &net->tensors[hc->param_ids[i]];
        const size_t sz = (size_t)bcnn_tensor_size(t);
        const int member = i < hc->arena_members;
        bcnn_hip_memcpy_d2d(new_p + off, t->data_gpu, sz * sizeof(float));
        bcnn_hip_sync();
        if (!member) bcnn_hip_free(t->data_gpu);
        t->data_gpu = new_p + off;
        if (new_g && t->grad_data_gpu) {
            bcnn_hip_memcpy_d2d(new_g + off, t->grad_data_gpu, sz * sizeof(float));
            bcnn_hip_sync();
            if (!member) bcnn_hip_free(t->grad_data_gpu);
            t->grad_data_gpu = new_g + off;
        }
        off += (sz + 3) & ~(size_t)3;
    }
    bcnn_hip_free(old_p);
    bcnn_hip_free(old_g);
    hc->param_arena_gpu = new_p;
    hc->grad_arena_gpu = new_g;
    hc->arena_size = total;
    hc->arena_members = hc->num_params;
}

static void mark_dead_grad_fills(bcnn_net *net) {
    bcnn_hip_context *hc = hctx(net);
    free(hc->grad_fill_dead);
    hc->grad_fill_dead = (unsigned char *)calloc((size_t)net->num_tensors + 1, 1);
    hc->grad_fill_count = net->num_tensors;
    if (BCNN_EXP_ENV("BCNN_KEEP_ALL_GRAD_FILLS")) return;
    for (int t = 0; t < net->num_tensors; ++t) {
        int first = -1, uses = 0;
        for (int i = 0; i < net->num_nodes; ++i)
            for (int k = 0; k < net->nodes[i].num_src; ++k)
                if (net->nodes[i].src[k] == t) {
                    if (first < 0) first = i;
                    ++uses;
                }
        if (first < 0) continue;
        int lifted_src = 0;
        for (int i = 0; i < net->num_nodes; ++i)
            lifted_src |= net->nodes[i].type == BCNN_LAYER_COST && net->nodes[i].src[0] == t &&
                          ((const bcnn_cost_param *)net->nodes[i].param)->loss == BCNN_LOSS_LIFTED_STRUCT;
        if (lifted_src) continue;
        const bcnn_node *nd = &net->nodes[first];
        if (nd->src[0] != t) continue;
        if (uses == 1 && (nd->type == BCNN_LAYER_MAXPOOL || nd->type == BCNN_LAYER_DEPTHWISE_CONV2D ||
                          nd->type == BCNN_LAYER_LRN)) {
            hc->grad_fill_dead[t] = 2;
            continue;
        }
        if (uses == 1 && nd->type == BCNN_LAYER_ELTWISE) {
            const bcnn_eltwise_param *ep = (const bcnn_eltwise_param *)nd->param;
            if (ep->stride[0] == 1 && ep->stride[1] == 1 &&
                bcnn_tensor_size(&net->tensors[t]) == bcnn_tensor_size(&net->tensors[nd->dst[0]]))
                hc->grad_fill_dead[t] = 2;
            continue;
        }
        if (nd->type == BCNN_LAYER_BATCHNORM) {
            hc->grad_fill_dead[t] = 1;
            continue;
        }
        if (nd->type != BCNN_LAYER_CONV2D) continue;
        const bcnn_conv_param *p = (const bcnn_conv_param *)nd->param;
        const bcnn_tensor *x = &net->tensors[t], *y = &net->tensors[nd->dst[0]];
        if (p->size == 1 && y->h * y->w != x->h * x->w) continue;
        hc->grad_fill_dead[t] = 1;
    }
}

int bcnn_grad_sole_writer(bcnn_net *net, int tensor) {
    const bcnn_hip_context *hc = hctx(net);
    return hc->grad_fill_dead && tensor >= 0 && tensor < hc->grad_fill_count && hc->grad_fill_dead[tensor] == 2;
}

static void comm_sync_parameters(bcnn_net *net);

bcnn_status bcnn_compile_net(bcnn_net *net) {
    bcnn_hip_context *hc = hctx(net);
    BCNN_CHECK_STATUS(bcnn_tensor_allocate(&net->tensors[0], net->mode));
    size_t need = 0;
    for (int i = 0; i < net->num_nodes; ++i) {
        if (net->nodes[i].type != BCNN_LAYER_CONV2D) continue;
        bcnn_conv_param *p = (bcnn_conv_param *)net->nodes[i].param;
        const bcnn_tensor *s = &net->tensors[net->nodes[i].src[0]];
        const size_t ws = bcnn_hip_conv_workspace_size(s->n, s->c, s->h, s->w, p->num, p->size, p->stride, p->pad,
                                                       p->num_groups);
        if (ws > need) need = ws;
    }
    if (need > hc->workspace_size) {
        bcnn_hip_free(hc->workspace_gpu);
        hc->workspace_gpu = bcnn_hip_malloc_f32(need);
        hc->workspace_size = need;
    }
    for (int i = 0; i < net->num_nodes; ++i)
        if (net->nodes[i].type == BCNN_LAYER_CONV2D)
            ((bcnn_conv_param *)net->nodes[i].param)->conv_workspace_gpu = hc->workspace_gpu;
    if (!hc->compiled || hc->num_params != hc->arena_members) {
        invalidate_sgd_table(net);
        build_arenas(net);
        hc->compiled = 1;
        if (hc->grad_ready_fn) bcnn_set_gradient_ready_callback(net, hc->grad_ready_fn, hc->grad_ready_user);
        comm_sync_parameters(net);
    }
    relink_graph(net);
    bcnn_hip_sync();
    return BCNN_SUCCESS;
}

static void relink_graph(bcnn_net *net) {
    bcnn_hip_context *hc = hctx(net);
    mark_dead_grad_fills(net);
    for (int i = 0; i < net->num_nodes; ++i) {
        if (net->nodes[i].type != BCNN_LAYER_CONV2D) continue;
        const int t = net->nodes[i].dst[0];
        int rewritten = 0;
        for (int j = 0; j < net->num_nodes; ++j)
            rewritten |= net->nodes[j].type == BCNN_LAYER_DROPOUT && net->nodes[j].dst[0] == t;
        ((bcnn_conv_param *)net->nodes[i].param)->out_rewritten = rewritten;
    }
    bcnn_link_depthwise_batchnorm(net);
    bcnn_link_conv_eltwise(net);
    bcnn_link_conv_maxpool(net);
    bcnn_link_conv_depthwise(net);
    bcnn_link_batchnorm_conv(net);
    if (hc->fill_chunks_gpu) {
        bcnn_hip_sync();
        bcnn_hip_free(hc->fill_chunks_gpu);
        hc->fill_chunks_gpu = NULL;
    }
    hc->num_fill_chunks = -1;
}

static bcnn_status resize_private_f32(float **buf, size_t old_elems, size_t new_elems, int need_realloc) {
    if (!*buf || new_elems <= old_elems) return BCNN_SUCCESS;
    if (!need_realloc) return BCNN_INVALID_PARAMETER;
    bcnn_hip_sync();
    bcnn_hip_free(*buf);
    *buf = bcnn_hip_malloc_f32(new_elems);
    return *buf ? BCNN_SUCCESS : BCNN_FAILED_ALLOC;
}

bcnn_status bcnn_resize_net(bcnn_net *net, int w, int h, int c, int need_realloc) {
    if (!net || w <= 0 || h <= 0 || c <= 0) return BCNN_INVALID_PARAMETER;
    for (int i = 0; i < net->num_nodes; ++i) {
        const bcnn_layer_type t = net->nodes[i].type;
        BCNN_CHECK_AND_LOG(net->log_ctx, t != BCNN_LAYER_CONCAT && t != BCNN_LAYER_UPSAMPLE && t != BCNN_LAYER_YOLOV3 &&
                                             t != BCNN_LAYER_TRANSPOSE_CONV2D,
                           BCNN_INVALID_PARAMETER,
                           "bcnn_resize_net: node %d is a concat / upsample / YOLO / deconvolution node, whose resize is "
                           "not supported\n", i);
        BCNN_CHECK_AND_LOG(net->log_ctx,
                           t != BCNN_LAYER_COST || ((const bcnn_cost_param *)net->nodes[i].param)->loss != BCNN_LOSS_LIFTED_STRUCT,
                           BCNN_INVALID_PARAMETER,
                           "bcnn_resize_net: node %d is a lifted-structure cost node, whose resize is not supported\n", i);
    }
    bcnn_set_input_shape(net, w, h, c, 1);
    for (int i = 0; i < net->num_nodes; ++i) {
        bcnn_node *nd = &net->nodes[i];
        if (nd->num_src < 1 || nd->num_dst < 1) continue;
        if (nd->type == BCNN_LAYER_DROPOUT) continue;
        const bcnn_tensor *s = &net->tensors[nd->src[0]];
        bcnn_tensor *d = &net->tensors[nd->dst[0]];
        const size_t old_elems = (size_t)bcnn_tensor_size(d);
        if (nd->type == BCNN_LAYER_CONV2D) {
            const bcnn_conv_param *p = (const bcnn_conv_param *)nd->param;
            bcnn_tensor_set_shape(d, s->n, p->num, (s->h + 2 * p->pad - p->size) / p->stride + 1,
                                  (s->w + 2 * p->pad - p->size) / p->stride + 1, 1);
        } else if (nd->type == BCNN_LAYER_MAXPOOL) {
            const bcnn_maxpool_param *p = (const bcnn_maxpool_param *)nd->param;
            bcnn_tensor_set_shape(d, s->n, s->c, (s->h - 1) / p->stride + 1, (s->w - 1) / p->stride + 1, 1);
        } else {
            bcnn_tensor_set_shape(d, s->n, s->c, s->h, s->w, 1);
        }
        if (need_realloc) BCNN_CHECK_STATUS(bcnn_tensor_allocate(d, net->mode));
        const size_t new_elems = (size_t)bcnn_tensor_size(d);
        if (nd->type == BCNN_LAYER_CONV2D) {
            bcnn_conv_param *p = (bcnn_conv_param *)nd->param;
            BCNN_CHECK_STATUS(resize_private_f32(&p->bn_workspace_gpu, old_elems, new_elems, need_realloc));
            BCNN_CHECK_STATUS(resize_private_f32(&p->x_norm_gpu, old_elems, new_elems, need_realloc));
        } else if (nd->type == BCNN_LAYER_BATCHNORM) {
            bcnn_batchnorm_param *p = (bcnn_batchnorm_param *)nd->param;
            BCNN_CHECK_STATUS(resize_private_f32(&p->workspace_gpu, old_elems, new_elems, need_realloc));
            BCNN_CHECK_STATUS(resize_private_f32(&p->x_norm_gpu, old_elems, new_elems, need_realloc));
        } else if (nd->type == BCNN_LAYER_MAXPOOL && new_elems > old_elems) {
            bcnn_maxpool_param *p = (bcnn_maxpool_param *)nd->param;
            if (!need_realloc) return BCNN_INVALID_PARAMETER;
            bcnn_hip_sync();
            bcnn_hip_free(p->indexes_gpu);
            p->indexes_gpu = bcnn_hip_malloc_i32(new_elems);
            int *host = (int *)realloc(p->indexes, new_elems * sizeof(int));
            if (!host || !p->indexes_gpu) return BCNN_FAILED_ALLOC;
            p->indexes = host;
            if (p->raw_at_max_gpu) {
                bcnn_hip_free(p->raw_at_max_gpu);
                p->raw_at_max_gpu = NULL;
            }
        }
    }
    if (hctx(net)->compiled) return bcnn_compile_net(net);
    return BCNN_SUCCESS;
}

bcnn_status bcnn_set_mode(bcnn_net *net, bcnn_mode mode) {
    if (net->mode == mode) return BCNN_SUCCESS;
    if (mode == BCNN_MODE_TRAIN && !hctx(net)->detector_training)
        for (int i = 0; i < net->num_nodes; ++i)
            BCNN_CHECK_AND_LOG(net->log_ctx, net->nodes[i].type != BCNN_LAYER_YOLOV3, BCNN_INVALID_PARAMETER,
                               "bcnn_set_mode: the net holds a YOLO node, whose TRAIN-mode loss is not built\n");
    if (mode == BCNN_MODE_TRAIN)
        BCNN_CHECK_AND_LOG(net->log_ctx, bcnn_yolo_heads_trainable(net), BCNN_INVALID_PARAMETER,
                           "bcnn_set_mode: a YOLO node was built without detector training or has no gradient buffer\n");
    net->mode = mode;
    if (net->data_loader) bcnn_switch_data_handles(net, net->data_loader);
    return BCNN_SUCCESS;
}

static void build_fill_table(bcnn_net *net) {
    bcnn_hip_context *hc = hctx(net);
    int cap = 256, n = 0;
    bcnn_hip_fill_chunk *tab = (bcnn_hip_fill_chunk *)malloc((size_t)cap * sizeof(*tab));
    unsigned char *seen = (unsigned char *)calloc((size_t)net->num_tensors + 1, 1);
    for (int i = 0; i < net->num_nodes; ++i)
        for (int d = 0; d < net->nodes[i].num_dst; ++d) {
            const int id = net->nodes[i].dst[d];
            bcnn_tensor *t = &net->tensors[id];
            if (seen[id] || !t->grad_data_gpu) continue;
            seen[id] = 1;
            if (hc->grad_fill_dead && id < hc->grad_fill_count && hc->grad_fill_dead[id]) continue;
            const size_t sz = (size_t)bcnn_tensor_size(t);
            for (size_t off = 0; off < sz; off += BCNN_HIP_FILL_CHUNK) {
                if (n == cap) {
                    cap *= 2;
                    tab = (bcnn_hip_fill_chunk *)realloc(tab, (size_t)cap * sizeof(*tab));
                }
                tab[n].p_d = t->grad_data_gpu + off;
                tab[n].count = (unsigned int)((sz - off < BCNN_HIP_FILL_CHUNK) ? (sz - off) : BCNN_HIP_FILL_CHUNK);
                tab[n].reserved = 0;
                ++n;
            }
        }
    free(seen);
    hc->num_fill_chunks = n;
    if (n > 0) {
        hc->fill_chunks_gpu = bcnn_hip_malloc_f32(((size_t)n * sizeof(*tab) + 3) / 4);
        bcnn_hip_memcpy_h2d(hc->fill_chunks_gpu, tab, (size_t)n * sizeof(*tab));
    }
    free(tab);
}

void bcnn_forward(bcnn_net *net) {
    bcnn_hip_context *hc = hctx(net);
    if (net->mode == BCNN_MODE_TRAIN) {
        if (hc->num_fill_chunks < 0) build_fill_table(net);
        bcnn_hip_zero_chunks((const bcnn_hip_fill_chunk *)hc->fill_chunks_gpu, hc->num_fill_chunks);
    }
    bcnn_drop_pending_gradients(net);
    bcnn_prepack_conv_weights(net, 0);
    hc->in_pass = 1;
    for (int i = 0; i < net->num_nodes; ++i) net->nodes[i].forward(net, &net->nodes[i]);
    hc->in_pass = 0;
    bcnn_hip_conv_prepack_discard();
}

static void comm_flush(bcnn_hip_context *hc) {
    if (hc->comm_lo < hc->comm_hi) {
        bcnn_hip_allreduce_sum(hc->grad_arena_gpu + hc->comm_lo, hc->comm_hi - hc->comm_lo);
        hc->comm_hi = hc->comm_lo;
    }
}

static void comm_on_ready(size_t first, size_t count, void *user) {
    bcnn_hip_context *hc = (bcnn_hip_context *)user;
    (void)count;
    hc->comm_lo = first;
    if (hc->comm_hi - hc->comm_lo >= hc->comm_bucket) comm_flush(hc);
}

void bcnn_backward(bcnn_net *net) {
    bcnn_hip_context *hc = hctx(net);
    size_t ready_from = hc->arena_size;
    if (hc->comm_active) hc->comm_lo = hc->comm_hi = hc->arena_size;
    bcnn_prepack_conv_weights(net, 1);
    hc->in_pass = 2;
    const int side_prev = bcnn_hip_conv_side_stream_mode((hc->no_side_stream || BCNN_EXP_ENV("BCNN_NO_SIDE_STREAM")) ? 0 : 2);
    for (int i = net->num_nodes - 1; i >= 0; --i) {
        net->nodes[i].backward(net, &net->nodes[i]);
        if (hc->grad_ready_fn && hc->node_grad_first && hc->node_grad_first[i] < ready_from) {
            bcnn_hip_conv_side_join();
            hc->grad_ready_fn(hc->node_grad_first[i], ready_from - hc->node_grad_first[i], hc->grad_ready_user);
            ready_from = hc->node_grad_first[i];
        }
    }
    hc->in_pass = 0;
    bcnn_hip_conv_side_join();
    bcnn_hip_conv_side_stream_mode(side_prev);
    bcnn_hip_conv_prepack_discard();
    if (hc->grad_ready_fn && ready_from > 0 && hc->arena_size > 0)
        hc->grad_ready_fn(0, ready_from, hc->grad_ready_user);
    if (hc->comm_active) {
        comm_flush(hc);
        bcnn_hip_comm_join();
    }
}

void bcnn_set_weight_gradient_stream(bcnn_net *net, int enable) { hctx(net)->no_side_stream = enable ? 0 : 1; }

bcnn_status bcnn_set_inference_precision(bcnn_net *net, bcnn_precision p) {
    if (!net || (p != BCNN_PRECISION_FP32 && p != BCNN_PRECISION_BF16)) return BCNN_INVALID_PARAMETER;
    hctx(net)->inference_precision = (int)p;
    return BCNN_SUCCESS;
}

bcnn_precision bcnn_get_inference_precision(const bcnn_net *net) {
    return (bcnn_precision)((const bcnn_hip_context *)net->hip_ctx)->inference_precision;
}

bcnn_status bcnn_set_loader_on_device(bcnn_net *net, int on) {
    if (!net) return BCNN_INVALID_PARAMETER;
    hctx(net)->loader_on_device = on ? 1 : 0;
    return BCNN_SUCCESS;
}

int bcnn_get_loader_on_device(const bcnn_net *net) {
    return net ? ((const bcnn_hip_context *)net->hip_ctx)->loader_on_device : 0;
}

bcnn_status bcnn_set_loader_decode_on_device(bcnn_net *net, int on) {
    if (!net) return BCNN_INVALID_PARAMETER;
    hctx(net)->loader_decode_on_device = on ? 1 : 0;
    return BCNN_SUCCESS;
}

int bcnn_get_loader_decode_on_device(const bcnn_net *net) {
    return net ? ((const bcnn_hip_context *)net->hip_ctx)->loader_decode_on_device : 0;
}

int bcnn_get_loader_device_decoded(const bcnn_net *net) {
    return net ? ((const bcnn_hip_context *)net->hip_ctx)->loader_device_decoded : 0;
}

bcnn_status bcnn_set_loader_detection_on_device(bcnn_net *net, int on) {
    if (!net) return BCNN_INVALID_PARAMETER;
    hctx(net)->loader_detection_on_device = on ? 1 : 0;
    return BCNN_SUCCESS;
}

int bcnn_get_loader_detection_on_device(const bcnn_net *net) {
    return net ? ((const bcnn_hip_context *)net->hip_ctx)->loader_detection_on_device : 0;
}

int bcnn_get_loader_device_letterboxed(const bcnn_net *net) {
    return net ? ((const bcnn_hip_context *)net->hip_ctx)->loader_device_letterboxed : 0;
}

bcnn_status bcnn_set_loader_effects(bcnn_net *net, int on) {
    if (!net) return BCNN_INVALID_PARAMETER;
    hctx(net)->loader_effects = on ? 1 : 0;
    return BCNN_SUCCESS;
}

int bcnn_get_loader_effects(const bcnn_net *net) {
    return net ? ((const bcnn_hip_context *)net->hip_ctx)->loader_effects : 0;
}

bcnn_status bcnn_set_detector_training(bcnn_net *net, int on) {
    if (!net) return BCNN_INVALID_PARAMETER;
    hctx(net)->detector_training = on ? 1 : 0;
    return BCNN_SUCCESS;
}

int bcnn_get_detector_training(const bcnn_net *net) {
    return net ? ((const bcnn_hip_context *)net->hip_ctx)->detector_training : 0;
}

void bcnn_set_gradient_ready_callback(bcnn_net *net, bcnn_gradient_ready_fn fn, void *user) {
    bcnn_hip_context *hc = hctx(net);
    hc->grad_ready_fn = fn;
    hc->grad_ready_user = user;
    free(hc->node_grad_first);
    hc->node_grad_first = NULL;
    if (!fn || !hc->grad_arena_gpu) return;
    hc->node_grad_first = (size_t *)malloc((size_t)net->num_nodes * sizeof(size_t));
    for (int i = 0; i < net->num_nodes; ++i) {
        size_t first = (size_t)-1;
        for (int k = 0; k < net->nodes[i].num_src; ++k) {
            const bcnn_tensor *t = &net->tensors[net->nodes[i].src[k]];
            if (!t->grad_data_gpu || t->grad_data_gpu < hc->grad_arena_gpu ||
                t->grad_data_gpu >= hc->grad_arena_gpu + hc->arena_size)
                continue;
            const size_t off = (size_t)(t->grad_data_gpu - hc->grad_arena_gpu);
            if (off < first) first = off;
        }
        hc->node_grad_first[i] = first;
    }
}

static void step_learning_rate(bcnn_net *net) {
    bcnn_learner *ln = net->learner;
    const int global_batch = net->batch_size * hctx(net)->dp_world;
    ln->seen += global_batch;
    const int iter = ln->seen / global_batch;
    switch (ln->decay_type) {
        case BCNN_LR_DECAY_STEP:
            ln->learning_rate = ln->base_learning_rate * (float)pow(ln->scale, iter / ln->step);
            break;
        case BCNN_LR_DECAY_INV:
            ln->learning_rate = ln->base_learning_rate * (float)pow(1.0f + ln->gamma * iter, -ln->power);
            break;
        case BCNN_LR_DECAY_EXP:
            ln->learning_rate = ln->base_learning_rate * (float)pow(ln->gamma, iter);
            break;
        case BCNN_LR_DECAY_POLY:
            ln->learning_rate = ln->base_learning_rate * (float)pow(1 - (float)iter / ln->max_batches, ln->power);
            break;
        case BCNN_LR_DECAY_SIGMOID:
            ln->learning_rate = ln->base_learning_rate * (1.0f / (1.0f + (float)exp(ln->gamma * (iter - ln->step))));
            break;
        default:
            break;
    }
}

static void sgd_table_add(bcnn_hip_context *hc, float *w, float *g, size_t n, int use_decay) {
    for (size_t off = 0; off < n; off += BCNN_HIP_SGD_CHUNK) {
        if (hc->num_sgd_chunks == hc->cap_sgd_chunks) {
            hc->cap_sgd_chunks = hc->cap_sgd_chunks ? 2 * hc->cap_sgd_chunks : 1024;
            hc->sgd_chunks_host = (bcnn_hip_sgd_chunk *)realloc(hc->sgd_chunks_host,
// ... 325 lines not shown
```

### bcnn_amd/host/bcnn_internal.h

```cpp
#ifndef BCNN_INTERNAL_H
#define BCNN_INTERNAL_H

#include <stdbool.h>
#include <stdio.h>
#include <stdlib.h>

#include <bcnn/bcnn.h>
#include <bip/bip.h>

#ifdef __cplusplus
extern "C" {
#endif

typedef struct {
    bcnn_log_callback fct;
    bcnn_log_level lvl;
} bcnn_log_context;

void bcnn_log(bcnn_log_context ctx, bcnn_log_level level, const char *fmt, ...);

#define BCNN_CHECK(exp, err) do { if (!(exp)) return (err); } while (0)
#define BCNN_CHECK_AND_LOG(ctx, exp, err, fmt, ...) \
    do { if (!(exp)) { bcnn_log((ctx), BCNN_LOG_ERROR, (fmt), ##__VA_ARGS__); return (err); } } while (0)
#define BCNN_CHECK_STATUS(s) do { bcnn_status ret_ = (s); if (ret_ != BCNN_SUCCESS) return ret_; } while (0)
// ... 4 lines not shown
#ifdef BCNN_HIP_EXPERIMENT
#define BCNN_EXP_ENV(name) getenv(name)
#else
#define BCNN_EXP_ENV(name) ((const char *)NULL)
#endif

typedef struct {
    int state;
    float r;
} bcnn_gauss_gen;
float bcnn_rng_gaussian(bcnn_gauss_gen *g);

struct bcnn_node {
    int num_src;
    int num_dst;
    bcnn_layer_type type;
    size_t param_size;
    int *src;
    int *dst;
    void *param;
    void (*forward)(struct bcnn_net *net, struct bcnn_node *node);
    void (*backward)(struct bcnn_net *net, struct bcnn_node *node);
    void (*update)(struct bcnn_net *net, struct bcnn_node *node);
    void (*release_param)(struct bcnn_node *node);
};
typedef struct bcnn_node bcnn_node;

typedef struct {
    int step;
    int seen;
    int max_batches;
    float momentum;
    float decay;
    float base_learning_rate;
    float learning_rate;
    float gamma;
    float scale;
    float power;
    float beta1;
    float beta2;
    bcnn_optimizer optimizer;
    bcnn_lr_decay decay_type;
} bcnn_learner;

typedef struct {
    int input_width;
    int input_height;
    int input_depth;
    bool has_extra_data;
    bcnn_loader_type type;
    uint8_t *input_uchar;
    uint8_t *input_net;
    FILE *f_train;
    FILE *f_train_extra;
    FILE *f_test;
    FILE *f_test_extra;
    FILE *f_current;
    FILE *f_current_extra;
} bcnn_loader;

typedef struct {
    int range_shift_x, range_shift_y, random_fliph, min_brightness, max_brightness, swap_to_bgr, no_input_norm,
        max_random_spots;
    float min_scale, max_scale, rotation_range, min_contrast, max_contrast, max_distortion, mean_r, mean_g, mean_b;
    int use_precomputed, brightness, apply_fliph, shift_x, shift_y;
    float rotation, scale, contrast, distortion, distortion_kx, distortion_ky;
} bcnn_data_augmenter;

struct bcnn_net;
bcnn_status bcnn_loader_next(struct bcnn_net *net);
void bcnn_convert_img_to_float(const uint8_t *src, int w, int h, int c, float norm_coeff, int swap_to_bgr, float mean_r,
                               float mean_g, float mean_b, float *dst);
#define BCNN_MAX_SPOTS 64
bcnn_status bcnn_apply_data_augmentation(unsigned char *img, int width, int height, int depth, bcnn_data_augmenter *param,
                                         unsigned char *buffer);
bcnn_status bcnn_open_dataset(bcnn_loader *iter, struct bcnn_net *net, const char *train_path, const char *train_path_extra,
                              const char *test_path, const char *test_path_extra, bool has_extra);
bcnn_status bcnn_switch_data_handles(struct bcnn_net *net, bcnn_loader *iter);
void bcnn_fill_input_tensor(struct bcnn_net *net, bcnn_loader *iter, char *path_img, int idx);
void bcnn_destroy_data_loader(struct bcnn_net *net);
void bcnn_free_loader_stage(struct bcnn_net *net);

typedef struct bcnn_hip_context {
    size_t workspace_size;
    float *workspace_gpu;
    float *param_arena_gpu;
    float *grad_arena_gpu;
    size_t arena_size;
    int *param_ids;
    int num_params;
    int arena_members;
    int dp_rank;
    int dp_world;
    int compiled;
    void (*grad_ready_fn)(size_t, size_t, void *);
    void *grad_ready_user;
    size_t *node_grad_first;
    unsigned char *grad_fill_dead;
    int grad_fill_count;
    struct bcnn_hip_sgd_chunk *sgd_chunks_host;
    void *sgd_chunks_gpu;
    int num_sgd_chunks, cap_sgd_chunks;
    int sgd_collecting;
    void *fill_chunks_gpu;
    int num_fill_chunks;
    int comm_active;
    size_t comm_bucket, comm_lo, comm_hi;
    int in_pass;
    int no_side_stream;
    uint64_t dropout_seed;
    int inference_precision;
    int loader_on_device;
    void *loader_stage;
    int loader_decode_on_device;
    int loader_device_decoded;
    int loader_detection_on_device;
    int loader_device_letterboxed;
    int loader_effects;
    int detector_training;
    int detect_capacity;
} bcnn_hip_context;

struct bcnn_net {
    int batch_size;
    int num_nodes;
    int num_tensors;
    int num_inputs;
    int *inputs;
    bcnn_mode mode;
    bcnn_log_context log_ctx;
    bcnn_node *nodes;
    bcnn_tensor *tensors;
    bcnn_learner *learner;
    bcnn_loader *data_loader;
    bcnn_data_augmenter *data_aug;
    void *gemm_ctx;
#ifdef BCNN_USE_HIP
    void *hip_ctx;
#endif
    int num_threads;
};

bcnn_status bcnn_net_add_node(bcnn_net *net, bcnn_node node);
bcnn_status bcnn_net_add_tensor(bcnn_net *net, bcnn_tensor tensor);
bcnn_status bcnn_node_add_input(bcnn_net *net, bcnn_node *node, int index);
bcnn_status bcnn_node_add_output(bcnn_net *net, bcnn_node *node, int index);
bcnn_status bcnn_node_new_output(bcnn_net *net, bcnn_node *node, int n, int c, int h, int w, const char *dst_id);

typedef struct tensor_filler {
    int range;
    float value;
    bcnn_filler_type type;
} bcnn_tensor_filler;

void bcnn_tensor_create(bcnn_tensor *t, int n, int c, int h, int w, int has_grad, const char *name, int net_state);
void bcnn_tensor_fill(bcnn_tensor *t, bcnn_tensor_filler filler);
void bcnn_tensor_destroy(bcnn_tensor *t);
void bcnn_tensor_set_shape(bcnn_tensor *t, int n, int c, int h, int w, int has_grad);
bcnn_status bcnn_tensor_allocate_buffer(bcnn_tensor *t, int net_state, size_t size);
bcnn_status bcnn_tensor_allocate(bcnn_tensor *t, int net_state);
void bcnn_tensor_free(bcnn_tensor *t);
int bcnn_tensor_size(const bcnn_tensor *t);
int bcnn_tensor_size3d(const bcnn_tensor *t);
int bcnn_tensor_size2d(const bcnn_tensor *t);

void bcnn_net_register_param(bcnn_net *net, int index);
int bcnn_net_find_tensor(bcnn_net *net, const char *name);

bcnn_status bcnn_loader_next(bcnn_net *net);
void bcnn_convert_img_to_float(const uint8_t *src, int w, int h, int c, float norm_coeff, int swap_to_bgr,
                               float mean_r, float mean_g, float mean_b, float *dst);
void bcnn_draw_color_box(unsigned char *img, int w_img, int h_img, float cx_box, float cy_box, float w_box,
                         float h_box, unsigned char color[3]);

static inline const char *bcnn_act2str(bcnn_activation a) {
    switch (a) {
        case BCNN_ACT_TANH: return "Tanh";
        case BCNN_ACT_RELU: return "ReLU";
        case BCNN_ACT_RAMP: return "Ramp";
        case BCNN_ACT_SOFTPLUS: return "Softplus";
        case BCNN_ACT_LRELU: return "Leaky-ReLU";
        case BCNN_ACT_ABS: return "AbsVal";
        case BCNN_ACT_CLAMP: return "Clamp";
        case BCNN_ACT_PRELU: return "PReLU";
        case BCNN_ACT_LOGISTIC: return "Logistic";
        default: return "None";
    }
}

typedef struct bcnn_conv_param {
    int num, size, stride, pad, num_groups, batch_norm, post_func;
    size_t workspace_size;
    bcnn_activation activation;
    bcnn_tensor saved_mean;
    bcnn_tensor saved_variance;
    float *conv_workspace;
    float *workspace;
    float *x_norm;
    float *adam_m, *adam_v;
#ifdef BCNN_USE_HIP
    float *conv_workspace_gpu;
    float *bn_workspace_gpu;
    float *x_norm_gpu;
    float *adam_m_gpu, *adam_v_gpu;
    int elt_node;
    int pool_node;
    int bnsums_node;
    int dw_node;
    int apply_skipped;
    int fold_bn;
    int folded;
    int pool_bwd_pending;
    float *insums_gpu;
    size_t insums_floats;
    int insums_splits;
    int data_pending;
    int out_rewritten;
#endif
} bcnn_conv_param;

typedef struct bcnn_depthwise_conv_param {
    int size, stride, pad, batch_norm;
    bcnn_activation activation;
    float *adam_m, *adam_v;
#ifdef BCNN_USE_HIP
    float *adam_m_gpu, *adam_v_gpu;
    int bn_node;
    int bn_fused_bwd;
    float *stats_gpu;
    size_t stats_floats;
    int stats_splits;
    int conv_node;
    int raw_input;
    int grads_pending;
#endif
} bcnn_depthwise_conv_param;

typedef struct bcnn_batchnorm_param {
    bcnn_tensor saved_mean;
    bcnn_tensor saved_variance;
    float *workspace;
    float *x_norm;
#ifdef BCNN_USE_HIP
    float *workspace_gpu;
    float *x_norm_gpu;
    int dw_node;
    int dw_fused_bwd;
    int sums_conv;
    float *bsums_gpu;
    size_t bsums_floats;
    int bsums_splits;
    int input_kept;
    int fold_conv;
    int apply_skipped;
    int data_pending;
#endif
} bcnn_batchnorm_param;

typedef struct bcnn_maxpool_param {
    int size, stride;
    bcnn_padding padding;
    int *indexes;
#ifdef BCNN_USE_HIP
    int *indexes_gpu;
    int conv_node;
    float *raw_at_max_gpu;
    int raw_fwd;
#endif
} bcnn_maxpool_param;

typedef struct bcnn_activation_param {
    bcnn_activation activation;
} bcnn_activation_param;

typedef struct bcnn_eltwise_param {
    bcnn_activation activation;
    int stride[2];
    int min_dim[3];
#ifdef BCNN_USE_HIP
    int conv_node;
    int done_forward;
    int deferred;
    int grad_pending;
#endif
} bcnn_eltwise_param;

typedef struct bcnn_fullc_param {
    bcnn_activation activation;
    float *adam_m, *adam_v;
#ifdef BCNN_USE_HIP
    float *adam_m_gpu, *adam_v_gpu;
#endif
} bcnn_fullc_param;

typedef struct bcnn_cost_param {
    float scale;
    bcnn_loss loss;
    bcnn_loss_metric loss_metric;
    float num_constraints;
#ifdef BCNN_USE_HIP
    float *lifted_workspace_gpu;
    size_t lifted_workspace_size;
    void *lifted_record_gpu;
#endif
} bcnn_cost_param;

typedef struct bcnn_upsample_param {
    int size;
} bcnn_upsample_param;

typedef struct bcnn_deconv_param {
    int num, size, stride, pad;
    bcnn_activation activation;
    float *conv_workspace;
    float *adam_m, *adam_v;
#ifdef BCNN_USE_HIP
    float *conv_workspace_gpu;
    size_t workspace_size;
    float *adam_m_gpu, *adam_v_gpu;
#endif
} bcnn_deconv_param;

typedef struct bcnn_lrn_param {
    int local_size;
    float alpha;
    float beta;
    float k;
} bcnn_lrn_param;

typedef struct bcnn_dropout_param {
    float dropout_rate;
    float scale;
    uint64_t step;
    uint64_t last_key;
    uint64_t last_step;
    int has_mask;
} bcnn_dropout_param;

typedef struct bcnn_yolo_param {
    int num, classes, coords, total;
    int *mask;
    float *biases;
    float *cost;
    int max_boxes, truths;
#ifdef BCNN_USE_HIP
    void *train_record_gpu;
    float *train_workspace_gpu;
    size_t train_workspace_size;
#endif
} bcnn_yolo_param;

void bcnn_forward_conv_layer(bcnn_net *net, bcnn_node *node);
void bcnn_backward_conv_layer(bcnn_net *net, bcnn_node *node);
void bcnn_update_conv_layer(bcnn_net *net, bcnn_node *node);
void bcnn_release_param_conv_layer(bcnn_node *node);
void bcnn_forward_depthwise_conv_layer(bcnn_net *net, bcnn_node *node);
void bcnn_backward_depthwise_conv_layer(bcnn_net *net, bcnn_node *node);
void bcnn_update_depthwise_conv_layer(bcnn_net *net, bcnn_node *node);
void bcnn_release_param_depthwise_conv_layer(bcnn_node *node);
void bcnn_forward_batchnorm_layer(bcnn_net *net, bcnn_node *node);
void bcnn_backward_batchnorm_layer(bcnn_net *net, bcnn_node *node);
void bcnn_release_param_batchnorm_layer(bcnn_node *node);
void bcnn_forward_maxpool_layer(bcnn_net *net, bcnn_node *node);
void bcnn_backward_maxpool_layer(bcnn_net *net, bcnn_node *node);
void bcnn_release_param_maxpool_layer(bcnn_node *node);
void bcnn_forward_avgpool_layer(bcnn_net *net, bcnn_node *node);
void bcnn_backward_avgpool_layer(bcnn_net *net, bcnn_node *node);
void bcnn_forward_activation_layer(bcnn_net *net, bcnn_node *node);
void bcnn_backward_activation_layer(bcnn_net *net, bcnn_node *node);
void bcnn_update_activation_layer(bcnn_net *net, bcnn_node *node);
void bcnn_forward_eltwise_layer(bcnn_net *net, bcnn_node *node);
void bcnn_backward_eltwise_layer(bcnn_net *net, bcnn_node *node);
void bcnn_forward_fullc_layer(bcnn_net *net, bcnn_node *node);
void bcnn_backward_fullc_layer(bcnn_net *net, bcnn_node *node);
void bcnn_update_fullc_layer(bcnn_net *net, bcnn_node *node);
void bcnn_release_param_fullc_layer(bcnn_node *node);
void bcnn_forward_softmax_layer(bcnn_net *net, bcnn_node *node);
void bcnn_backward_softmax_layer(bcnn_net *net, bcnn_node *node);
void bcnn_forward_cost_layer(bcnn_net *net, bcnn_node *node);
void bcnn_backward_cost_layer(bcnn_net *net, bcnn_node *node);
void bcnn_release_param_cost_layer(bcnn_node *node);
void bcnn_forward_concat_layer(bcnn_net *net, bcnn_node *node);
void bcnn_backward_concat_layer(bcnn_net *net, bcnn_node *node);
void bcnn_forward_upsample_layer(bcnn_net *net, bcnn_node *node);
void bcnn_backward_upsample_layer(bcnn_net *net, bcnn_node *node);
void bcnn_forward_yolo_layer(bcnn_net *net, bcnn_node *node);
void bcnn_backward_yolo_layer(bcnn_net *net, bcnn_node *node);
void bcnn_release_param_yolo_layer(bcnn_node *node);
int bcnn_yolo_heads_trainable(bcnn_net *net);
int bcnn_yolo_refresh_costs(bcnn_net *net);
bcnn_status bcnn_yolo_detections_batch_worker(bcnn_net *net, const int *widths, const int *heights, int netw, int neth,
                                              float thresh, int relative, int record_cap, int nms_cap,
                                              bcnn_output_detection **dets, int *num_dets, int *passes);
void bcnn_forward_deconv_layer(bcnn_net *net, bcnn_node *node);
void bcnn_backward_deconv_layer(bcnn_net *net, bcnn_node *node);
void bcnn_update_deconv_layer(bcnn_net *net, bcnn_node *node);
void bcnn_release_param_deconv_layer(bcnn_node *node);
void bcnn_forward_lrn_layer(bcnn_net *net, bcnn_node *node);
void bcnn_backward_lrn_layer(bcnn_net *net, bcnn_node *node);
void bcnn_release_param_lrn_layer(bcnn_node *node);
void bcnn_forward_dropout_layer(bcnn_net *net, bcnn_node *node);
void bcnn_backward_dropout_layer(bcnn_net *net, bcnn_node *node);
void bcnn_release_param_dropout_layer(bcnn_node *node);
uint64_t bcnn_dropout_key(uint64_t seed, int node, int rank);

void bcnn_link_depthwise_batchnorm(bcnn_net *net);
void bcnn_link_conv_eltwise(bcnn_net *net);
void bcnn_link_conv_maxpool(bcnn_net *net);
void bcnn_link_conv_depthwise(bcnn_net *net);
void bcnn_link_batchnorm_conv(bcnn_net *net);
int bcnn_jpeg_read_batch(int num_images, const uint8_t *const *buffers, const size_t *lengths, const bip_jpeg_info *infos,
                         int16_t *const *coeff, int num_threads);
struct bcnn_hip_jpeg_frame;
void bcnn_jpeg_frame_from_info(const bip_jpeg_info *info, struct bcnn_hip_jpeg_frame *f);
int bcnn_jpeg_read_batch_each(int num_images, const uint8_t *const *buffers, const size_t *lengths,
                              const bip_jpeg_info *infos, int16_t *const *coeff, int num_threads, int *status);
void bcnn_materialize_data(bcnn_net *net, int tensor);
void bcnn_materialize_gradients(bcnn_net *net, int tensor);
void bcnn_drop_pending_gradients(bcnn_net *net);
void bcnn_prepack_conv_weights(bcnn_net *net, int data_gradient);
int bcnn_grad_sole_writer(bcnn_net *net, int tensor);
void bcnn_node_sgd_step(bcnn_net *net, bcnn_tensor *weights, bcnn_tensor *biases);
void bcnn_node_optim_step(bcnn_net *net, bcnn_tensor *weights, bcnn_tensor *biases, float **adam_m_gpu,
                          float **adam_v_gpu);

#ifdef __cplusplus
}
#endif
#endif
```

### bcnn_amd/host/bcnn_layers_next.c

```c
#include <float.h>
#include <math.h>
#include <string.h>

#include "bcnn_internal.h"
#include "../../include/bcnn_hip.h"

static int imin(int a, int b) { return a < b ? a : b; }
static int imax(int a, int b) { return a > b ? a : b; }

bcnn_status bcnn_node_new_output(bcnn_net *net, bcnn_node *node, int n, int c, int h, int w, const char *dst_id) {
    bcnn_tensor t = {0};
    bcnn_tensor_set_shape(&t, n, c, h, w, 1);
    BCNN_CHECK_STATUS(bcnn_tensor_allocate(&t, net->mode));
    t.name = (char *)malloc(strlen(dst_id) + 1);
    strcpy(t.name, dst_id);
    BCNN_CHECK_STATUS(bcnn_net_add_tensor(net, t));
    return bcnn_node_add_output(net, node, net->num_tensors - 1);
}

static bcnn_hip_context *hctx(bcnn_net *net) { return (bcnn_hip_context *)net->hip_ctx; }

bcnn_status bcnn_add_eltwise_layer(bcnn_net *net, bcnn_activation activation, const char *src_id1,
                                   const char *src_id2, const char *dst_id) {
    bcnn_node node = {0};
    int found1 = 0, found2 = 0;
    for (int i = net->num_tensors - 1; i >= 0 && !(found1 && found2); --i) {
        const char *nm = net->tensors[i].name;
        if (!nm) continue;
        if (strcmp(nm, src_id1) == 0) { bcnn_node_add_input(net, &node, i); found1 = 1; }
        if (strcmp(nm, src_id2) == 0) { bcnn_node_add_input(net, &node, i); found2 = 1; }
    }
    BCNN_CHECK_AND_LOG(net->log_ctx, found1, BCNN_INVALID_PARAMETER, "Eltwise layer: invalid input node name %s\n", src_id1);
    BCNN_CHECK_AND_LOG(net->log_ctx, found2, BCNN_INVALID_PARAMETER, "Eltwise layer: invalid input node name %s\n", src_id2);
    const bcnn_tensor a = net->tensors[node.src[0]], b = net->tensors[node.src[1]];
    const int st0 = a.w / b.w, st1 = b.w / a.w;
    BCNN_CHECK_AND_LOG(net->log_ctx, st0 == a.h / b.h && st1 == b.h / a.h, BCNN_INVALID_PARAMETER,
                       "Eltwise layer: inconsistent spatial size between tensor %s and tensor %s\n", src_id1, src_id2);
    node.type = BCNN_LAYER_ELTWISE;
    node.param_size = sizeof(bcnn_eltwise_param);
    bcnn_eltwise_param *param = (bcnn_eltwise_param *)calloc(1, node.param_size);
    node.param = param;
    param->activation = activation;
    param->conv_node = -1;
    param->min_dim[0] = imin(a.c, b.c); param->min_dim[1] = imin(a.h, b.h); param->min_dim[2] = imin(a.w, b.w);
    param->stride[0] = imax(1, st0); param->stride[1] = imax(1, st1);
    node.forward = bcnn_forward_eltwise_layer;
    node.backward = bcnn_backward_eltwise_layer;
    BCNN_CHECK_STATUS(bcnn_node_new_output(net, &node, a.n, a.c, a.h, a.w, dst_id));
    BCNN_CHECK_STATUS(bcnn_net_add_node(net, node));
    BCNN_INFO(net->log_ctx, "[EltWiseAdd] %-8s , %-8s -> %-8s (%4d x%4d x%4d)\n", a.name, b.name, dst_id, a.w, a.h, a.c);
    return BCNN_SUCCESS;
}

void bcnn_forward_eltwise_layer(bcnn_net *net, bcnn_node *node) {
    bcnn_eltwise_param *p = (bcnn_eltwise_param *)node->param;
    if (p->done_forward) {
        p->done_forward = 0;
        if (hctx(net)->in_pass == 1) return;
    }
    bcnn_tensor *a = &net->tensors[node->src[0]], *b = &net->tensors[node->src[1]], *y = &net->tensors[node->dst[0]];
    const size_t sz = (size_t)bcnn_tensor_size(y);
    if (p->stride[0] == 1 && p->stride[1] == 1) {
        bcnn_hip_eltwise_forward(a->data_gpu, b->data_gpu, y->data_gpu, sz, (size_t)p->min_dim[0] * y->h * y->w,
                                 (int)p->activation);
        return;
    }
    bcnn_hip_copy_f32(sz, a->data_gpu, y->data_gpu);
    {
        bcnn_hip_axpy_strided(a->n, 1.0f, b->data_gpu, y->data_gpu, p->stride[0], p->stride[1], b->c, b->h, b->w, y->c,
                              y->h, y->w, p->min_dim[0], p->min_dim[1], p->min_dim[2]);
    }
    bcnn_hip_activation_forward(y->data_gpu, sz, (int)p->activation, NULL, y->w * y->h, y->c);
}

void bcnn_backward_eltwise_layer(bcnn_net *net, bcnn_node *node) {
    bcnn_eltwise_param *p = (bcnn_eltwise_param *)node->param;
    if (hctx(net)->in_pass == 2 && p->conv_node >= 0) {
        p->deferred = 1;
        return;
    }
    bcnn_tensor *a = &net->tensors[node->src[0]], *b = &net->tensors[node->src[1]], *y = &net->tensors[node->dst[0]];
    const size_t sz = (size_t)bcnn_tensor_size(y);
    if (p->stride[0] == 1 && p->stride[1] == 1) {
        bcnn_hip_eltwise_backward(y->data_gpu, y->grad_data_gpu, a->grad_data_gpu, b->grad_data_gpu, sz,
                                  (size_t)p->min_dim[0] * y->h * y->w, (int)p->activation,
                                  bcnn_grad_sole_writer(net, node->src[0]));
        return;
    }
    bcnn_hip_activation_backward(y->data_gpu, y->grad_data_gpu, sz, (int)p->activation, NULL, NULL, y->w * y->h, y->c);
    if (a->grad_data_gpu) bcnn_hip_axpy(sz, 1.0f, y->grad_data_gpu, a->grad_data_gpu);
    if (!b->grad_data_gpu) return;
    {
        bcnn_hip_axpy_strided(a->n, 1.0f, y->grad_data_gpu, b->grad_data_gpu, p->stride[1], p->stride[0], y->c, y->h,
                              y->w, b->c, b->h, b->w, p->min_dim[0], p->min_dim[1], p->min_dim[2]);
    }
}

bcnn_status bcnn_add_fullc_layer(bcnn_net *net, int output_size, bcnn_filler_type init, bcnn_activation activation,
                                 int quantize, const char *src_id, const char *dst_id) {
    (void)quantize;
    bcnn_node node = {0};
    if (net->num_nodes > 0) {
        const int idx = bcnn_net_find_tensor(net, src_id);
        BCNN_CHECK_AND_LOG(net->log_ctx, idx >= 0, BCNN_INVALID_PARAMETER,
                           "Full-connected layer: invalid input node name %s\n", src_id);
        bcnn_node_add_input(net, &node, idx);
    } else {
        bcnn_node_add_input(net, &node, 0);
    }
    const bcnn_tensor s = net->tensors[node.src[0]];
    char name[256];
    snprintf(name, sizeof(name), "%s_w", src_id);
    bcnn_tensor weights = {0};
    bcnn_tensor_create(&weights, output_size, s.c, s.h, s.w, 1, name, net->mode);
    bcnn_tensor_filler wf = {.range = bcnn_tensor_size3d(&s), .type = init};
    bcnn_tensor_fill(&weights, wf);
    BCNN_CHECK_STATUS(bcnn_net_add_tensor(net, weights));
    BCNN_CHECK_STATUS(bcnn_node_add_input(net, &node, net->num_tensors - 1));
    bcnn_net_register_param(net, net->num_tensors - 1);
    snprintf(name, sizeof(name), "%s_b", src_id);
    bcnn_tensor biases = {0};
    bcnn_tensor_create(&biases, 1, 1, 1, output_size, 1, name, net->mode);
    BCNN_CHECK_STATUS(bcnn_net_add_tensor(net, biases));
    BCNN_CHECK_STATUS(bcnn_node_add_input(net, &node, net->num_tensors - 1));
    bcnn_net_register_param(net, net->num_tensors - 1);
    BCNN_CHECK_STATUS(bcnn_node_new_output(net, &node, s.n, output_size, 1, 1, dst_id));
    node.type = BCNN_LAYER_FULL_CONNECTED;
    node.param_size = sizeof(bcnn_fullc_param);
    bcnn_fullc_param *param = (bcnn_fullc_param *)calloc(1, node.param_size);
    node.param = param;
    param->activation = activation;
    node.forward = bcnn_forward_fullc_layer;
    node.backward = bcnn_backward_fullc_layer;
    node.update = bcnn_update_fullc_layer;
    node.release_param = bcnn_release_param_fullc_layer;
    BCNN_CHECK_STATUS(bcnn_net_add_node(net, node));
    BCNN_INFO(net->log_ctx, "[Dense] %-8s (%4d x%4d x%4d) -> %-8s (%d)\n", src_id, s.w, s.h, s.c, dst_id, output_size);
    return BCNN_SUCCESS;
}

void bcnn_forward_fullc_layer(bcnn_net *net, bcnn_node *node) {
    bcnn_fullc_param *p = (bcnn_fullc_param *)node->param;
    bcnn_tensor *x = &net->tensors[node->src[0]], *w = &net->tensors[node->src[1]];
    bcnn_tensor *b = &net->tensors[node->src[2]], *y = &net->tensors[node->dst[0]];
    const int B = y->n, S = bcnn_tensor_size3d(x), P = y->c;
    bcnn_hip_gemm(0, 1, B, P, S, 1.0f, x->data_gpu, S, w->data_gpu, S, 0.0f, y->data_gpu, P);
    bcnn_hip_add_rowvec(y->data_gpu, b->data_gpu, B, P);
    bcnn_hip_activation_forward(y->data_gpu, (size_t)B * P, (int)p->activation, NULL, 1, P);
}

void bcnn_backward_fullc_layer(bcnn_net *net, bcnn_node *node) {
    bcnn_fullc_param *p = (bcnn_fullc_param *)node->param;
    bcnn_tensor *x = &net->tensors[node->src[0]], *w = &net->tensors[node->src[1]];
    bcnn_tensor *b = &net->tensors[node->src[2]], *y = &net->tensors[node->dst[0]];
    const int B = y->n, S = bcnn_tensor_size3d(x), P = y->c;
    bcnn_hip_activation_backward(y->data_gpu, y->grad_data_gpu, (size_t)B * P, (int)p->activation, NULL, NULL, 1, P);
    bcnn_hip_grad_bias(b->grad_data_gpu, y->grad_data_gpu, B, P, 1);
    bcnn_hip_gemm(1, 0, P, S, B, 1.0f, y->grad_data_gpu, P, x->data_gpu, S, 1.0f, w->grad_data_gpu, S);
    if (x->grad_data_gpu)
        bcnn_hip_gemm(0, 0, B, S, P, 1.0f, y->grad_data_gpu, P, w->data_gpu, S, 1.0f, x->grad_data_gpu, S);
}

void bcnn_update_fullc_layer(bcnn_net *net, bcnn_node *node) {
    bcnn_fullc_param *p = (bcnn_fullc_param *)node->param;
    bcnn_node_optim_step(net, &net->tensors[node->src[1]], &net->tensors[node->src[2]], &p->adam_m_gpu, &p->adam_v_gpu);
}

void bcnn_release_param_fullc_layer(bcnn_node *node) {
    bcnn_fullc_param *p = (bcnn_fullc_param *)node->param;
    bcnn_hip_free(p->adam_m_gpu);
    bcnn_hip_free(p->adam_v_gpu);
}

bcnn_status bcnn_add_softmax_layer(bcnn_net *net, const char *src_id, const char *dst_id) {
    bcnn_node node = {0};
    if (net->num_nodes > 0) {
        const int idx = bcnn_net_find_tensor(net, src_id);
        BCNN_CHECK_AND_LOG(net->log_ctx, idx >= 0, BCNN_INVALID_PARAMETER, "Softmax layer: invalid input node name %s\n", src_id);
        bcnn_node_add_input(net, &node, idx);
    } else {
        bcnn_node_add_input(net, &node, 0);
    }
    const bcnn_tensor s = net->tensors[node.src[0]];
    BCNN_CHECK_STATUS(bcnn_node_new_output(net, &node, s.n, s.c, s.h, s.w, dst_id));
    node.type = BCNN_LAYER_SOFTMAX;
    node.forward = bcnn_forward_softmax_layer;
    node.backward = bcnn_backward_softmax_layer;
    BCNN_CHECK_STATUS(bcnn_net_add_node(net, node));
    BCNN_INFO(net->log_ctx, "[Softmax] %-8s -> %-8s (%4d x%4d x%4d)\n", src_id, dst_id, s.w, s.h, s.c);
    return BCNN_SUCCESS;
}

void bcnn_forward_softmax_layer(bcnn_net *net, bcnn_node *node) {
    bcnn_tensor *x = &net->tensors[node->src[0]], *y = &net->tensors[node->dst[0]];
    bcnn_hip_softmax_forward(x->data_gpu, y->data_gpu, x->n, x->c, x->h * x->w);
}

void bcnn_backward_softmax_layer(bcnn_net *net, bcnn_node *node) {
    bcnn_tensor *x = &net->tensors[node->src[0]], *y = &net->tensors[node->dst[0]];
    if (x->grad_data_gpu) bcnn_hip_axpy((size_t)bcnn_tensor_size(x), 1.0f, y->grad_data_gpu, x->grad_data_gpu);
}

bcnn_status bcnn_add_cost_layer(bcnn_net *net, bcnn_loss loss, bcnn_loss_metric loss_metric, float scale,
                                const char *src_id, const char *label_id, const char *dst_id) {
    (void)label_id;
    bcnn_node node = {0};
    BCNN_CHECK_AND_LOG(net->log_ctx, net->num_nodes >= 1, BCNN_INVALID_PARAMETER,
                       "Cost layer can't be the first layer of the network\n");
    BCNN_CHECK_AND_LOG(net->log_ctx, loss == BCNN_LOSS_EUCLIDEAN || loss == BCNN_LOSS_LIFTED_STRUCT, BCNN_INVALID_PARAMETER,
                       "Cost layer: unknown loss %d\n", (int)loss);
    const int idx = bcnn_net_find_tensor(net, src_id);
    BCNN_CHECK_AND_LOG(net->log_ctx, idx >= 0, BCNN_INVALID_PARAMETER, "Cost layer: invalid input node name %s\n", src_id);
    BCNN_CHECK_AND_LOG(net->log_ctx,
                       loss != BCNN_LOSS_LIFTED_STRUCT || (net->tensors[idx].h == 1 && net->tensors[idx].w == 1),
                       BCNN_INVALID_PARAMETER,
                       "Cost layer: the lifted-structure loss needs a [n][c][1][1] embedding, %s is %d x %d x %d\n", src_id,
                       net->tensors[idx].w, net->tensors[idx].h, net->tensors[idx].c);
    bcnn_node_add_input(net, &node, idx);
    node.type = BCNN_LAYER_COST;
    node.param_size = sizeof(bcnn_cost_param);
    bcnn_cost_param *param = (bcnn_cost_param *)calloc(1, node.param_size);
    node.param = param;
    param->scale = scale; param->loss = loss; param->loss_metric = loss_metric;
    node.forward = bcnn_forward_cost_layer;
    node.backward = bcnn_backward_cost_layer;
    node.release_param = bcnn_release_param_cost_layer;
    const bcnn_tensor s = net->tensors[idx];
    bcnn_tensor_set_shape(&net->tensors[1], s.n, s.c, s.h, s.w, 0);
    BCNN_CHECK_STATUS(bcnn_tensor_allocate(&net->tensors[1], net->mode));
    bcnn_node_add_input(net, &node, 1);
    BCNN_CHECK_STATUS(bcnn_node_new_output(net, &node, s.n, s.c, s.h, s.w, dst_id));
    return bcnn_net_add_node(net, node);
}

static float host_metric(const bcnn_cost_param *p, const bcnn_tensor *pred, const bcnn_tensor *label,
                         const bcnn_tensor *dst) {
    const int per = pred->w * pred->h * pred->c, B = pred->n, sz = per * B;
    double acc = 0.0;
    switch (p->loss_metric) {
        case BCNN_METRIC_ERROR_RATE:
            for (int i = 0; i < B; ++i) {
                float pm = FLT_MIN;
                int best = 0;
                for (int j = 0; j < per; ++j)
                    if (pred->data[i * per + j] > pm) { pm = pred->data[i * per + j]; best = j; }
                if (label->data[i * per + best] == 0) acc += 1.0;
            }
            return (float)acc;
        case BCNN_METRIC_LOGLOSS:
            for (int i = 0; i < sz; ++i)
                if (label->data[i] > 0.0f) {
                    float q = pred->data[i];
                    q = q < 1e-8f ? 1e-8f : (q > 1.0f - 1e-8f ? 1.0f - 1e-8f : q);
                    acc += -log(q);
                }
            return (float)acc;
        case BCNN_METRIC_MSE:
        case BCNN_METRIC_SSE:
        case BCNN_METRIC_CRPS:
            for (int i = 0; i < sz; ++i) acc += (double)dst->grad_data[i] * dst->grad_data[i];
            return (float)(p->loss_metric == BCNN_METRIC_MSE ? acc / per : acc);
        case BCNN_METRIC_DICE:
            for (int i = 0; i < B; ++i) {
                int n = 0, d = 0;
                for (int j = 0; j < per; ++j) {
                    n += (int)(label->data[i * per + j] * (pred->data[i * per + j] > 0.5f));
                    d += (int)(label->data[i * per + j] + (pred->data[i * per + j] > 0.5f));
                }
                acc += (2.0f * n + 1.0f) / (d + 1.0f);
            }
            return (float)acc;
    }
    return 0.f;
}

void bcnn_forward_cost_layer(bcnn_net *net, bcnn_node *node) {
    bcnn_cost_param *p = (bcnn_cost_param *)node->param;
    bcnn_tensor *pred = &net->tensors[node->src[0]], *label = &net->tensors[1], *dst = &net->tensors[node->dst[0]];
    if (!label->data) return;
    const size_t sz = (size_t)bcnn_tensor_size(pred);
    if (p->loss == BCNN_LOSS_LIFTED_STRUCT) {
        if (pred->grad_data_gpu && label->data_gpu && net->mode != BCNN_MODE_PREDICT) {
            const size_t need = bcnn_hip_lifted_struct_workspace_size(pred->n, pred->c);
            if (p->lifted_workspace_size < need) {
                bcnn_hip_sync();
                bcnn_hip_free(p->lifted_workspace_gpu);
                p->lifted_workspace_gpu = bcnn_hip_malloc_f32(need);
                p->lifted_workspace_size = need;
            }
            if (!p->lifted_record_gpu) p->lifted_record_gpu = bcnn_hip_malloc_f32(2);
            bcnn_hip_lifted_struct_forward(pred->data_gpu, label->data_gpu, pred->grad_data_gpu, pred->n, pred->c, 1.0f, 1,
                                           (bcnn_hip_lifted_struct_record *)p->lifted_record_gpu,
                                           p->lifted_workspace_gpu);
        }
    } else if (dst->grad_data_gpu) {
        bcnn_hip_copy_f32(sz, pred->data_gpu, dst->grad_data_gpu);
        bcnn_hip_axpy(sz, -1.0f, label->data_gpu, dst->grad_data_gpu);
    }
    if (net->mode == BCNN_MODE_PREDICT) return;
    static int host_loop = -1;
    if (host_loop < 0) host_loop = BCNN_EXP_ENV("BCNN_HOST_COST_METRIC") != NULL;
    if (host_loop || !label->data_gpu || !dst->grad_data_gpu) {
        if (dst->grad_data_gpu) bcnn_hip_memcpy_d2h(dst->grad_data, dst->grad_data_gpu, sz * sizeof(float));
        bcnn_hip_memcpy_d2h(pred->data, pred->data_gpu, sz * sizeof(float));
        dst->data[0] = host_metric(p, pred, label, dst);
        bcnn_hip_memcpy_h2d(dst->data_gpu, dst->data, sizeof(float));
        return;
    }
    bcnn_hip_cost_metric((int)p->loss_metric, pred->data_gpu, label->data_gpu, dst->grad_data_gpu, pred->n,
                         pred->w * pred->h * pred->c, dst->data_gpu);
    bcnn_hip_memcpy_d2h(dst->data, dst->data_gpu, sizeof(float));
}

void bcnn_backward_cost_layer(bcnn_net *net, bcnn_node *node) {
    bcnn_cost_param *p = (bcnn_cost_param *)node->param;
    bcnn_tensor *pred = &net->tensors[node->src[0]], *dst = &net->tensors[node->dst[0]];
    if (p->loss == BCNN_LOSS_LIFTED_STRUCT) {
        if (pred->grad_data_gpu && p->lifted_record_gpu)
            bcnn_hip_lifted_struct_backward(pred->grad_data_gpu, pred->n, pred->c, p->scale,
                                            (const bcnn_hip_lifted_struct_record *)p->lifted_record_gpu);
        return;
    }
    if (pred->grad_data_gpu)
        bcnn_hip_axpy((size_t)bcnn_tensor_size(pred), p->scale, dst->grad_data_gpu, pred->grad_data_gpu);
}

void bcnn_release_param_cost_layer(bcnn_node *node) {
    bcnn_cost_param *p = (bcnn_cost_param *)node->param;
    bcnn_hip_free(p->lifted_workspace_gpu);
    bcnn_hip_free(p->lifted_record_gpu);
}

bcnn_status bcnn_get_lifted_struct_loss(bcnn_net *net, float *loss, int *num_constraints) {
    if (!net) return BCNN_INVALID_PARAMETER;
    for (int i = net->num_nodes - 1; i >= 0; --i) {
        if (net->nodes[i].type != BCNN_LAYER_COST) continue;
        bcnn_cost_param *p = (bcnn_cost_param *)net->nodes[i].param;
        if (p->loss != BCNN_LOSS_LIFTED_STRUCT) continue;
        bcnn_hip_lifted_struct_record rec = {0.f, 0};
        if (p->lifted_record_gpu) bcnn_hip_memcpy_d2h(&rec, p->lifted_record_gpu, sizeof(rec));
        p->num_constraints = (float)rec.num_constraints;
        if (loss) *loss = rec.loss;
        if (num_constraints) *num_constraints = rec.num_constraints;
        return BCNN_SUCCESS;
    }
    return BCNN_INVALID_PARAMETER;
}
```

### include/bcnn_hip.h

```cpp
#ifndef BCNN_HIP_H
#define BCNN_HIP_H

#include <stddef.h>
#include <stdint.h>

#ifdef __cplusplus
extern "C" {
#endif

enum {
    BCNN_HIP_ACT_NONE = 0, BCNN_HIP_ACT_TANH, BCNN_HIP_ACT_RELU, BCNN_HIP_ACT_RAMP,
    BCNN_HIP_ACT_SOFTPLUS, BCNN_HIP_ACT_LRELU, BCNN_HIP_ACT_ABS, BCNN_HIP_ACT_CLAMP,
    BCNN_HIP_ACT_PRELU, BCNN_HIP_ACT_LOGISTIC
};
enum { BCNN_HIP_MODE_PREDICT = 0, BCNN_HIP_MODE_TRAIN = 1, BCNN_HIP_MODE_VALID = 2 };

int bcnn_hip_device_count(void);
void bcnn_hip_set_device(int id);
int bcnn_hip_get_device(void);
const char *bcnn_hip_device_name(void);
float *bcnn_hip_malloc_f32(size_t n);
int *bcnn_hip_malloc_i32(size_t n);
void bcnn_hip_free(void *p_d);
void bcnn_hip_memcpy_h2d(void *dst_d, const void *src_h, size_t bytes);
void bcnn_hip_memcpy_d2h(void *dst_h, const void *src_d, size_t bytes);
void bcnn_hip_memcpy_d2d(void *dst_d, const void *src_d, size_t bytes);
void bcnn_hip_fill_f32(float *x_d, size_t n, float value);
void bcnn_hip_sync(void);
void *bcnn_hip_stream_create(void);
void bcnn_hip_stream_destroy(void *stream);
void bcnn_hip_set_stream(void *stream);
void *bcnn_hip_get_stream(void);
void *bcnn_hip_event_create(void);
void bcnn_hip_event_destroy(void *ev);
void bcnn_hip_event_record(void *ev);
void bcnn_hip_event_sync(void *ev);
float bcnn_hip_event_elapsed_ms(void *start, void *stop);

void bcnn_hip_profile_enable(int on);
void bcnn_hip_profile_reset(void);
int bcnn_hip_profile_num_classes(void);
const char *bcnn_hip_profile_class_name(int cls);
void bcnn_hip_profile_read(int cls, double *ms, long long *launches, double *flops, double *bytes);
double bcnn_hip_profile_read_useful_flops(int cls);

int bcnn_hip_conv_side_stream_mode(int mode);
void bcnn_hip_conv_side_join(void);

void bcnn_hip_trace_enable(int on);
size_t bcnn_hip_trace_read(char *buf, size_t cap);

void bcnn_hip_axpy(size_t n, float a, const float *x_d, float *y_d);
void bcnn_hip_scal(size_t n, float a, float *x_d);
void bcnn_hip_copy_f32(size_t n, const float *x_d, float *y_d);
void bcnn_hip_add_bias(float *y_d, const float *bias_d, int n, int c, int hw);
void bcnn_hip_grad_bias(float *dbias_d, const float *g_d, int n, int c, int hw);
void bcnn_hip_scales(float *y_d, const float *scales_d, int n, int c, int hw);
void bcnn_hip_grad_scales(const float *x_norm_d, const float *g_d, int n, int c, int hw,
                          float *dscales_d);

void bcnn_hip_gemm(int trans_a, int trans_b, int m, int n, int k, float alpha, const float *a_d,
                   int lda, const float *b_d, int ldb, float beta, float *c_d, int ldc);
void bcnn_hip_im2col(const float *im_d, int channels, int height, int width, int ksize, int pad,
                     int stride, float *col_d);
void bcnn_hip_col2im(const float *col_d, int channels, int height, int width, int ksize, int pad,
                     int stride, float *im_d);

void bcnn_hip_activation_forward(float *x_d, size_t size, int act, const float *slopes_d,
                                 int spatial, int channels);
void bcnn_hip_activation_backward(const float *x_d, float *dx_d, size_t size, int act,
                                  const float *slopes_d, float *dslopes_d, int spatial, int channels);

void bcnn_hip_batchnorm_forward(const float *x_d, float *y_d, float *run_mean_d, float *run_var_d,
                                const float *scales_d, const float *bias_d, float *saved_mean_d,
                                float *saved_var_d, float *x_norm_d, float *workspace_d, int n, int c,
                                int hw, int mode, int act);
void bcnn_hip_batchnorm_backward(float *dy_d, float *dx_d, const float *y_d, int act,
                                 const float *scales_d, float *dscales_d, float *dbias_d,
                                 const float *saved_mean_d, const float *saved_var_d, float *dmean_d,
                                 float *dvar_d, const float *x_norm_d, const float *workspace_d, int n,
                                 int c, int hw);

size_t bcnn_hip_conv_workspace_size(int n, int c, int h, int w, int f, int k, int stride, int pad,
                                    int groups);
void bcnn_hip_conv_forward(const float *x_d, const float *w_d, const float *bias_d, float *y_d, int n,
                           int c, int h, int w, int f, int k, int stride, int pad, int groups, int act,
                           const float *slopes_d,
                           int batch_norm, float *run_mean_d, float *run_var_d, const float *scales_d,
                           float *saved_mean_d, float *saved_var_d, float *x_norm_d,
                           float *bn_workspace_d, int mode);
void bcnn_hip_conv_backward(const float *x_d, const float *w_d, const float *bias_d, const float *y_d,
                            float *dy_d, float *dx_d, float *dw_d, float *dbias_d, int n, int c, int h, int w, int f,
                            int k, int stride, int pad, int groups, int act, const float *slopes_d,
                            float *dslopes_d, int batch_norm, const float *scales_d, float *dscales_d,
                            const float *saved_mean_d, const float *saved_var_d, float *dmean_d,
                            float *dvar_d, const float *x_norm_d, const float *bn_workspace_d,
                            float *workspace_d, size_t workspace_elems);
int bcnn_hip_conv_forward_bf16(const float *x_d, const float *w_d, const float *bias_d, float *y_d, int n, int c, int h,
                               int w, int f, int k, int stride, int pad, int groups, int act, const float *slopes_d,
                               int batch_norm, float *run_mean_d, float *run_var_d, const float *scales_d,
                               float *saved_mean_d, float *saved_var_d, float *x_norm_d, float *bn_workspace_d,
                               int mode);

int bcnn_hip_conv_residual_fusable(int batch_norm, int act, int res_act, int mode, const float *bn_workspace_d,
                                   const float *res_d, const float *res_out_d);
void bcnn_hip_conv_forward_residual(const float *x_d, const float *w_d, const float *bias_d, int n, int c, int h, int w,
                                    int f, int k, int stride, int pad, int groups, float *run_mean_d, float *run_var_d,
                                    const float *scales_d, float *saved_mean_d, float *saved_var_d,
                                    float *bn_workspace_d, const float *res_d, size_t res_count, int res_act,
                                    float *res_out_d);
void bcnn_hip_conv_backward_residual(const float *x_d, const float *w_d, const float *bias_d, float *dy_d, float *dx_d,
                                     float *dw_d, float *dbias_d, int n, int c, int h, int w, int f, int k, int stride,
                                     int pad, int groups, const float *scales_d, float *dscales_d,
                                     const float *saved_mean_d, const float *saved_var_d, float *dmean_d, float *dvar_d,
                                     const float *bn_workspace_d, float *workspace_d, size_t workspace_elems,
                                     const float *res_out_d, const float *dres_out_d, int res_act, const float *res_d,
                                     float *dres_d, size_t res_count);
void bcnn_hip_batchnorm_apply(const float *x_d, float *y_d, const float *scales_d, const float *bias_d,
                              const float *saved_mean_d, const float *saved_var_d, int n, int c, int hw, int act);

typedef struct {
    const float *w_d;
    int n, c, h, w, f, k, stride, pad, groups;
} bcnn_hip_conv_desc;
void bcnn_hip_conv_prepack(const bcnn_hip_conv_desc *layers, int count, int data_gradient);
void bcnn_hip_conv_prepack_reset(void);
void bcnn_hip_conv_prepack_discard(void);

void bcnn_hip_maxpool_forward(const float *x_d, float *y_d, int *indexes_d, int n, int c, int h, int w,
                              int out_h, int out_w, int size, int stride);
void bcnn_hip_maxpool_backward(const float *dy_d, const int *indexes_d, float *dx_d, int n, int c,
                               int h, int w, int out_h, int out_w, int size, int stride, int overwrite);
size_t bcnn_hip_conv_bnsums_size(int n, int c, int h, int w);
int bcnn_hip_conv_backward_bnsums(const float *x_d, const float *w_d, const float *bias_d, const float *y_d, float *dy_d,
                                  float *dx_d, float *dw_d, float *dbias_d, int n, int c, int h, int w, int f, int k,
                                  int stride, int pad, int groups, int act, const float *slopes_d, float *dslopes_d,
                                  int batch_norm, const float *scales_d, float *dscales_d, const float *saved_mean_d,
                                  const float *saved_var_d, float *dmean_d, float *dvar_d, const float *x_norm_d,
                                  const float *bn_workspace_d, float *workspace_d, size_t workspace_elems,
                                  const float *prev_y_d, const float *prev_mean_d, float *sums_d, size_t sums_floats);
size_t bcnn_hip_depthwise_insums_size(int n, int c, int h, int w, int k, int stride, int pad);
int bcnn_hip_depthwise_backward_bnin_sums(const float *x_raw_d, const float *w_d, const float *y_d, float *dy_d, float *dx_d,
                                          float *dw_d, float *dbias_d, int n, int c, int h, int w, int k, int stride, int pad,
                                          int act, int overwrite, const float *bn_mean_d, const float *bn_var_d,
                                          const float *bn_scales_d, const float *bn_dmean_d, const float *bn_dvar_d,
                                          const float *in_mean_d, const float *in_var_d, const float *in_scale_d,
                                          const float *in_bias_d, int in_act, float *in_sums_d, size_t in_sums_floats);
int bcnn_hip_conv_backward_presummed(const float *x_d, const float *w_d, const float *bias_d, const float *y_d, float *dy_d,
                                     float *dx_d, float *dw_d, float *dbias_d, int n, int c, int h, int w, int f, int k,
                                     int stride, int pad, int groups, int act, const float *slopes_d, float *dslopes_d,
                                     int batch_norm, const float *scales_d, float *dscales_d, const float *saved_mean_d,
                                     const float *saved_var_d, float *dmean_d, float *dvar_d, const float *x_norm_d,
                                     const float *bn_workspace_d, float *workspace_d, size_t workspace_elems,
                                     const float *own_sums_d, int own_splits, const float *prev_y_d,
                                     const float *prev_mean_d, float *prev_sums_d, size_t prev_sums_floats);
void bcnn_hip_batchnorm_backward_finalize(const float *sums_d, int splits, const float *scales_d, float *dscales_d,
                                          float *dbias_d, const float *saved_var_d, float *dmean_d, float *dvar_d, int c);

void bcnn_hip_conv_forward_stats_only(const float *x_d, const float *w_d, const float *bias_d, int n, int c, int h, int w,
                                      int f, int k, int stride, int pad, int groups, float *run_mean_d, float *run_var_d,
                                      const float *scales_d, float *saved_mean_d, float *saved_var_d,
                                      float *bn_workspace_d);
int bcnn_hip_maxpool_bn_fusable(int n, int c, int h, int w, int out_h, int out_w, int size, int stride, int act,
                                const float *x_d);
void bcnn_hip_maxpool_forward_bn(const float *x_d, float *y_d, int *indexes_d, int n, int c, int h, int w, int out_h,
                                 int out_w, int size, int stride, const float *scales_d, const float *bias_d,
                                 const float *saved_mean_d, const float *saved_var_d, int act);
void bcnn_hip_maxpool_forward_bn_keep(const float *x_d, float *y_d, int *indexes_d, int n, int c, int h, int w, int out_h,
                                      int out_w, int size, int stride, const float *scales_d, const float *bias_d,
                                      const float *saved_mean_d, const float *saved_var_d, int act, float *raw_at_max_d);
int bcnn_hip_maxpool_bn_backward_fusable(int n, int c, int h, int w, int out_h, int out_w, int size, int stride, int act,
                                         const float *raw_d, const float *dpool_d, const int *indexes_d, const float *dx_d);
void bcnn_hip_maxpool_bn_backward(const float *dpool_d, const int *indexes_d, const float *raw_at_max_d, const float *raw_d,
                                  float *dx_d, int n, int c, int h, int w, int out_h, int out_w, int size, int stride,
                                  const float *scales_d, float *dscales_d, const float *bias_d, float *dbias_d,
                                  const float *saved_mean_d, const float *saved_var_d, float *dmean_d, float *dvar_d, int act);
void bcnn_hip_conv_backward_bn_done(const float *x_d, const float *w_d, float *dy_d, float *dx_d, float *dw_d, int n, int c,
                                    int h, int w, int f, int k, int stride, int pad, int groups, float *workspace_d,
                                    size_t workspace_elems);
void bcnn_hip_avgpool_forward(const float *x_d, float *y_d, int n, int c, int h, int w);
void bcnn_hip_avgpool_backward(const float *dy_d, float *dx_d, int n, int c, int h, int w);

void bcnn_hip_depthwise_forward(const float *x_d, const float *w_d, const float *bias_d, float *y_d,
                                int n, int c, int h, int w, int k, int stride, int pad, int act);
void bcnn_hip_depthwise_backward(const float *x_d, const float *w_d, const float *y_d, float *dy_d,
                                 float *dx_d, float *dw_d, float *dbias_d, int n, int c, int h, int w,
                                 int k, int stride, int pad, int act, int overwrite);

size_t bcnn_hip_depthwise_stats_size(int n, int c, int h, int w, int k, int stride, int pad);
int bcnn_hip_depthwise_forward_stats(const float *x_d, const float *w_d, const float *bias_d, float *y_d, int n, int c,
                                     int h, int w, int k, int stride, int pad, int act, float *stats_d,
                                     size_t stats_floats);
void bcnn_hip_batchnorm_forward_stats(const float *x_d, float *y_d, float *run_mean_d, float *run_var_d,
                                      const float *scales_d, const float *bias_d, float *saved_mean_d,
                                      float *saved_var_d, float *x_norm_d, float *workspace_d, int n, int c, int hw,
                                      int mode, int act, const float *stats_d, int splits);
void bcnn_hip_batchnorm_forward_stats_only(const float *x_d, float *run_mean_d, float *run_var_d, const float *scales_d,
                                           const float *bias_d, float *saved_mean_d, float *saved_var_d, int n, int c,
                                           int hw, const float *stats_d, int splits);
int bcnn_hip_conv_bnfold_fusable(int n, int c, int h, int w, int f);
void bcnn_hip_conv_set_input_bnfold(const float *mean_d, const float *var_d, const float *scales_d, const float *bias_d);
int bcnn_hip_depthwise_bn_fusable(int n, int c, int h, int w, int k, int stride, int pad, int act);
void bcnn_hip_batchnorm_backward_sums(const float *dy_d, const float *scales_d, float *dscales_d, float *dbias_d,
                                      const float *saved_mean_d, const float *saved_var_d, float *dmean_d,
                                      float *dvar_d, const float *x_d, int n, int c, int hw);
void bcnn_hip_batchnorm_backward_apply(float *dy_d, float *dx_d, const float *scales_d, const float *saved_mean_d,
                                       const float *saved_var_d, const float *dmean_d, const float *dvar_d,
                                       const float *x_d, int n, int c, int hw);
void bcnn_hip_depthwise_backward_bn(const float *x_d, const float *w_d, const float *y_d, const float *dz_d,
                                    float *dx_d, float *dw_d, float *dbias_d, int n, int c, int h, int w, int k,
                                    int stride, int pad, int act, int overwrite, const float *bn_mean_d,
                                    const float *bn_var_d, const float *bn_scales_d, const float *bn_dmean_d,
                                    const float *bn_dvar_d);

int bcnn_hip_depthwise_bnin_fusable(int n, int c, int h, int w, int k, int stride, int pad, int act, int in_act);
int bcnn_hip_depthwise_forward_bnin(const float *x_raw_d, const float *w_d, const float *bias_d, float *y_d, int n, int c,
                                    int h, int w, int k, int stride, int pad, int act, float *stats_d, size_t stats_floats,
                                    const float *in_mean_d, const float *in_var_d, const float *in_scale_d,
                                    const float *in_bias_d, int in_act);
void bcnn_hip_depthwise_backward_bnin(const float *x_raw_d, const float *w_d, const float *y_d, float *dy_d, float *dx_d,
                                      float *dw_d, float *dbias_d, int n, int c, int h, int w, int k, int stride, int pad,
                                      int act, int overwrite, const float *in_mean_d, const float *in_var_d,
                                      const float *in_scale_d, const float *in_bias_d, int in_act);
void bcnn_hip_depthwise_backward_bn_bnin(const float *x_raw_d, const float *w_d, const float *y_d, const float *dz_d,
                                         float *dx_d, float *dw_d, float *dbias_d, int n, int c, int h, int w, int k,
                                         int stride, int pad, int act, int overwrite, const float *bn_mean_d,
                                         const float *bn_var_d, const float *bn_scales_d, const float *bn_dmean_d,
                                         const float *bn_dvar_d, const float *in_mean_d, const float *in_var_d,
                                         const float *in_scale_d, const float *in_bias_d, int in_act);

void bcnn_hip_sgd_update(float *w_d, float *b_d, float *dw_d, float *db_d, size_t w_size,
                         size_t b_size, int batch_size, float learning_rate, float momentum,
                         float decay);

void bcnn_hip_adam_update(float *w_d, float *b_d, float *dw_d, float *db_d, float *adam_m_d,
                          float *adam_v_d, size_t w_size, size_t b_size, int batch_size, int iter,
                          float beta1, float beta2, float learning_rate, float momentum, float decay);

#define BCNN_HIP_SGD_CHUNK 2048
typedef struct bcnn_hip_sgd_chunk {
    float *w_d;
    float *g_d;
    unsigned int count;
    unsigned int use_decay;
} bcnn_hip_sgd_chunk;
void bcnn_hip_sgd_update_chunks(const bcnn_hip_sgd_chunk *chunks_d, int num_chunks, int batch_size,
                                float learning_rate, float momentum, float decay);

#define BCNN_HIP_FILL_CHUNK 16384
typedef struct bcnn_hip_fill_chunk {
    float *p_d;
    unsigned int count;
    unsigned int reserved;
} bcnn_hip_fill_chunk;
void bcnn_hip_zero_chunks(const bcnn_hip_fill_chunk *chunks_d, int num_chunks);

void bcnn_hip_eltwise_forward(const float *a_d, const float *b_d, float *y_d, size_t n, size_t b_count, int act);
void bcnn_hip_eltwise_backward(const float *y_d, float *dy_d, float *da_d, float *db_d, size_t n, size_t b_count,
                               int act, int overwrite_a);
void bcnn_hip_cost_metric(int metric, const float *pred_d, const float *label_d, const float *grad_d, int batch,
                          int per, float *out_d);
void bcnn_hip_axpy_strided(int num_batches, float a, const float *x_d, float *y_d, int stride_y,
                           int stride_x, int x_c, int x_h, int x_w, int y_c, int y_h, int y_w, int min_c,
                           int min_h, int min_w);
void bcnn_hip_add_rowvec(float *y_d, const float *v_d, int rows, int cols);
void bcnn_hip_softmax_forward(const float *x_d, float *y_d, int n, int c, int hw);

void bcnn_hip_concat_forward(int num_src, const float *const *src_d, const int *src_size3d, float *dst_d,
                             int dst_size3d, int n);
void bcnn_hip_concat_backward(int num_src, float *const *src_grad_d, const int *src_size3d, const float *dst_grad_d,
                              int dst_size3d, int n);
void bcnn_hip_upsample_forward(const float *x_d, float *y_d, int n, int c, int h, int w, int size);
void bcnn_hip_upsample_backward(float *dx_d, const float *dy_d, int n, int c, int h, int w, int size);
void bcnn_hip_yolo_activate(const float *x_d, float *y_d, int n, int num, int coords, int classes, int hw);

#define BCNN_HIP_YOLO_MAX_HEADS 8
#define BCNN_HIP_YOLO_MAX_ANCHORS 16
#define BCNN_HIP_YOLO_RECORD_HEAD 6
typedef struct bcnn_hip_yolo_head {
    const float *out_d;
    int h, w, num, coords, classes;
    float anchor_w[BCNN_HIP_YOLO_MAX_ANCHORS], anchor_h[BCNN_HIP_YOLO_MAX_ANCHORS];
} bcnn_hip_yolo_head;
int bcnn_hip_yolo_nms_capacity(void);
size_t bcnn_hip_yolo_detect_result_words(int n, int record_cap, int max_classes);
int bcnn_hip_yolo_detect_batch(const bcnn_hip_yolo_head *heads, int num_heads, int n, const int *image_geom, int in_w,
                               int in_h, int netw, int neth, float thresh, int relative, float nms_thresh,
                               int record_cap, int nms_cap, void *result_host);

#define BCNN_HIP_YOLO_TRAIN_MAX_TRUTHS 50
#define BCNN_HIP_YOLO_TRAIN_MAX_TOTAL 32
typedef struct bcnn_hip_yolo_train_head {
    int n, h, w, num, coords, classes, total;
    int in_w, in_h;
    int label_stride;
    int mask[BCNN_HIP_YOLO_MAX_ANCHORS];
    float biases[2 * BCNN_HIP_YOLO_TRAIN_MAX_TOTAL];
} bcnn_hip_yolo_train_head;
typedef struct bcnn_hip_yolo_train_record {
    float cost, avg_iou, avg_cat, avg_obj, avg_anyobj, recall, recall75;
    int count;
} bcnn_hip_yolo_train_record;
size_t bcnn_hip_yolo_train_workspace_size(const bcnn_hip_yolo_train_head *head);
int bcnn_hip_yolo_train_forward(const bcnn_hip_yolo_train_head *head, const float *x_d, const float *label_d, float *y_d,
                                float *grad_d, bcnn_hip_yolo_train_record *record_d, float *workspace_d);

#define BCNN_HIP_IMAGE_FIT_STRETCH 0
#define BCNN_HIP_IMAGE_FIT_LETTERBOX 1
int bcnn_hip_fill_images(float *dst_d, int n, int c, int h, int w, int num_images, const uint8_t *const *images,
                         const int *widths, const int *heights, const int *strides, int fit, float norm_coeff,
                         int swap_to_bgr, float mean_r, float mean_g, float mean_b);

typedef struct bcnn_hip_jpeg_component {
    int h, v;
    int width, height;
    int pitch, rows;
    int blocks_w, blocks_h;
    int idct_w, idct_h;
} bcnn_hip_jpeg_component;
typedef struct bcnn_hip_jpeg_frame {
    int width, height, ncomp, hmax, vmax;
    bcnn_hip_jpeg_component comp[3];
} bcnn_hip_jpeg_frame;
int bcnn_hip_jpeg_stage_begin(int n, int c, int h, int w, int num_images, const bcnn_hip_jpeg_frame *frames, int fit,
                              int16_t **coeff, int *failed_image);
int bcnn_hip_jpeg_stage_run(float *dst_d, float norm_coeff, int swap_to_bgr, float mean_r, float mean_g, float mean_b);
void bcnn_hip_jpeg_stage_cancel(void);

#define BCNN_HIP_AUG_FLIP 1
#define BCNN_HIP_AUG_SHIFT 2
#define BCNN_HIP_AUG_SCALE 4
#define BCNN_HIP_AUG_ROTATE 8
#define BCNN_HIP_AUG_CONTRAST 16
typedef struct bcnn_hip_augment_record {
    int32_t flags;
    int32_t x_ul, y_ul;
    int32_t ca, sa;
    int32_t gain;
    int32_t brightness;
    int32_t reserved;
} bcnn_hip_augment_record;
int bcnn_hip_augment_batch(float *dst_d, int n, int c, int h, int w, int num_samples, int src_w, int src_h,
                           const uint8_t *pixels, const bcnn_hip_augment_record *records, const int32_t *taps,
                           int swap_to_bgr);

int bcnn_hip_augment_jpeg_begin(int n, int c, int h, int w, int num_samples, const bcnn_hip_jpeg_frame *frames,
                                int16_t **coeff);
int bcnn_hip_augment_jpeg_run(float *dst_d, const uint8_t *decoded, const uint8_t *pixels,
                              const bcnn_hip_augment_record *records, const int32_t *taps, const int32_t *origins,
                              int swap_to_bgr);
void bcnn_hip_augment_jpeg_cancel(void);

typedef struct bcnn_hip_letterbox_image {
    const uint8_t *pixels;
    int32_t w, h;
    int32_t new_w, new_h;
    int32_t x_off, y_off;
} bcnn_hip_letterbox_image;
int bcnn_hip_augment_letterbox_batch(float *dst_d, int n, int c, int h, int w, int num_samples,
                                     const bcnn_hip_letterbox_image *images, const bcnn_hip_augment_record *records,
                                     const int32_t *taps, int swap_to_bgr);

#define BCNN_HIP_AUG_DISTORT 32
#define BCNN_HIP_AUG_SPOTS 64
typedef struct bcnn_hip_augment_effect {
    int32_t flags;
    int32_t seed;
    float distortion;
    int32_t first_spot, num_spots;
} bcnn_hip_augment_effect;
typedef struct bcnn_hip_augment_spot {
    int32_t x0, y0, bw, bh;
    uint32_t table;
} bcnn_hip_augment_spot;
int bcnn_hip_augment_effects_begin(int num_samples, int src_w, int src_h, const bcnn_hip_augment_effect *effects,
                                   const float *perlin, const int32_t *cells, const bcnn_hip_augment_spot *spots,
                                   int num_spots, const float *spot_tables, size_t num_table_floats);
void bcnn_hip_augment_effects_cancel(void);

size_t bcnn_hip_deconv_workspace_size(int n, int c, int h, int w, int f, int k, int stride, int pad);
void bcnn_hip_deconv_forward(const float *x_d, const float *w_d, const float *bias_d, float *y_d, int n, int c, int h,
                             int w, int f, int k, int stride, int pad, int act);
void bcnn_hip_deconv_backward(const float *x_d, const float *w_d, const float *y_d, float *dy_d, float *dx_d,
                              float *dw_d, float *dbias_d, int n, int c, int h, int w, int f, int k, int stride, int pad,
                              int act, float *workspace_d, size_t workspace_elems);

void bcnn_hip_lrn_forward(const float *x_d, float *y_d, int n, int c, int h, int w, int local_size, float alpha,
                          float beta, float k);
void bcnn_hip_lrn_backward(const float *x_d, const float *dy_d, float *dx_d, int n, int c, int h, int w,
                           int local_size, float alpha, float beta, float k, int overwrite);

void bcnn_hip_dropout_forward(float *x_d, size_t size, float rate, uint64_t key, uint64_t step);
void bcnn_hip_dropout_backward(float *dx_d, size_t size, float rate, uint64_t key, uint64_t step);

typedef struct bcnn_hip_lifted_struct_record {
    float loss;
    int num_constraints;
} bcnn_hip_lifted_struct_record;
size_t bcnn_hip_lifted_struct_workspace_size(int batch, int k);
void bcnn_hip_lifted_struct_forward(const float *x_d, const float *label_d, float *g_d, int batch, int k, float margin,
                                    int accumulate, bcnn_hip_lifted_struct_record *record_d, float *workspace_d);
void bcnn_hip_lifted_struct_backward(float *g_d, int batch, int k, float scale,
                                     const bcnn_hip_lifted_struct_record *record_d);

void bcnn_hip_comm_init(int rank, int world, const char *id_path);
void bcnn_hip_comm_retain(void);
void bcnn_hip_comm_destroy(void);
int bcnn_hip_rendezvous_publish(const char *path, const void *blob, size_t n, int world);
int bcnn_hip_rendezvous_fetch(const char *path, void *blob, size_t n, int world, int timeout_ms);
int bcnn_hip_comm_world(void);
int bcnn_hip_comm_rank(void);
void bcnn_hip_allreduce_sum(float *buf_d, size_t n);
void bcnn_hip_broadcast(float *buf_d, size_t n, int root);
void bcnn_hip_comm_join(void);

#ifdef __cplusplus
}
#endif
#endif
```

Baseline: 14150 images/s.

## Fuse FC, softmax+cost, residual grad into finalize, and pin loss readback

Adds a dedicated fused FC forward/backward kernel that computes bias/activation in the epilogue and dx, dw, dbias in one launch. Pairs softmax with a Euclidean cost layer so a single kernel produces softmax, gradient and metric, and the backward pass skips the separate softmax axpy. Folds the BN residual-gradient kernel into the BN finalize launch as extra blocks, and reads the loss back through a pinned staging buffer with an event instead of a blocking memcpy. Together these cut kernel launches and small host syncs in the classifier head and the BN backward, at the cost of a hand-written FC GEMM that may be slower than the library GEMM it replaces.

```diff
diff --git a/bcnn_amd/_lib.py b/bcnn_amd/_lib.py
--- a/bcnn_amd/_lib.py
+++ b/bcnn_amd/_lib.py
@@ -19,6 +19,9 @@
     "bcnn_hip_memcpy_h2d": (None, [vp, vp, sz]),
     "bcnn_hip_memcpy_d2h": (None, [vp, vp, sz]),
     "bcnn_hip_memcpy_d2d": (None, [vp, vp, sz]),
+    "bcnn_hip_host_alloc": (vp, [sz]),
+    "bcnn_hip_host_free": (None, [vp]),
+    "bcnn_hip_memcpy_d2h_pinned": (None, [vp, vp, sz, vp]),
     "bcnn_hip_fill_f32": (None, [vp, sz, f]),
     "bcnn_hip_sync": (None, []),
     "bcnn_hip_stream_create": (vp, []),
@@ -48,6 +51,8 @@
     "bcnn_hip_scales": (None, [vp, vp, i, i, i]),
     "bcnn_hip_grad_scales": (None, [vp, vp, i, i, i, vp]),
     "bcnn_hip_gemm": (None, [i, i, i, i, i, f, vp, i, vp, i, f, vp, i]),
+    "bcnn_hip_fc_forward": (None, [vp, vp, vp, vp, i, i, i, i]),
+    "bcnn_hip_fc_backward": (None, [vp, vp, vp, vp, vp, vp, i, i, i]),
     "bcnn_hip_im2col": (None, [vp, i, i, i, i, i, i, vp]),
     "bcnn_hip_col2im": (None, [vp, i, i, i, i, i, i, vp]),
     "bcnn_hip_activation_forward": (None, [vp, sz, i, vp, i, i]),
@@ -107,6 +112,8 @@
     "bcnn_hip_axpy_strided": (None, [i, f, vp, vp] + [i] * 11),
     "bcnn_hip_add_rowvec": (None, [vp, vp, i, i]),
     "bcnn_hip_softmax_forward": (None, [vp, vp, i, i, i]),
+    "bcnn_hip_softmax_cost_forward": (None, [i, vp, vp, vp, vp, i, i, vp]),
+    "bcnn_hip_softmax_cost_backward": (None, [sz, f, vp, vp, vp]),
     "bcnn_hip_concat_forward": (None, [i, vp, vp, vp, i, i]),
     "bcnn_hip_concat_backward": (None, [i, vp, vp, vp, i, i]),
     "bcnn_hip_upsample_forward": (None, [vp, vp, i, i, i, i, i]),
diff --git a/bcnn_amd/csrc/batchnorm.hip b/bcnn_amd/csrc/batchnorm.hip
--- a/bcnn_amd/csrc/batchnorm.hip
+++ b/bcnn_amd/csrc/batchnorm.hip
@@ -237,12 +237,24 @@
     }
 };
 
+struct BnResGrad {
+    const float *out, *dout;
+    float* dres;
+    unsigned count;
+    int act;
+};
+__device__ __forceinline__ void bn_residual_grad(const BnResGrad& r, unsigned block, unsigned nblocks) {
+    for (unsigned i = block * blockDim.x + threadIdx.x; i < r.count; i += nblocks * blockDim.x)
+        r.dres[i] += r.dout[i] * act_bwd_cheap(r.out[i], r.act, 0.f);
+}
+
 __global__ void bn_bwd_finalize_kernel(const float* __restrict__ partials, int C, int splits,
                                        const float* __restrict__ scale, const float* __restrict__ var,
                                        float* __restrict__ dbias, float* __restrict__ dscales,
                                        float* __restrict__ dmean, float* __restrict__ dvar,
                                        float4* __restrict__ consts, const float* __restrict__ mean,
-                                       const float* __restrict__ fwd_bias, float fM) {
+                                       const float* __restrict__ fwd_bias, float fM, int nfin, const BnResGrad rg) {
+    if ((int)blockIdx.x >= nfin) return bn_residual_grad(rg, blockIdx.x - nfin, gridDim.x - nfin);
     const int c = blockIdx.x * blockDim.x + threadIdx.x;
     if (c >= C) return;
     double s1 = 0.0, s2 = 0.0;
@@ -268,7 +280,9 @@
                                                                    float* __restrict__ dscales, float* __restrict__ dmean,
                                                                    float* __restrict__ dvar, float4* __restrict__ consts,
                                                                    const float* __restrict__ mean,
-                                                                   const float* __restrict__ fwd_bias, float fM) {
+                                                                   const float* __restrict__ fwd_bias, float fM,
+                                                                   const BnResGrad rg) {
+    if ((int)blockIdx.x >= C) return bn_residual_grad(rg, blockIdx.x - C, gridDim.x - C);
     __shared__ double red[16][2];
     const int lane = threadIdx.x & 63, wid = threadIdx.x >> 6, c = blockIdx.x;
     const float2* p = reinterpret_cast<const float2*>(partials) + (long long)c * splits;
@@ -463,6 +477,13 @@
 }
 
 namespace bcnn_hip {
+static BnResGrad bn_res_grad_of(const BnBwdCall& b) {
+    BnResGrad r{b.y, b.dout, b.dres, 0u, b.act};
+    if (b.dout && b.dres) r.count = (unsigned)b.res_count;
+    return r;
+}
+static int bn_res_grad_blocks(const BnResGrad& r, int block) { return r.count ? stream_grid(r.count, block) : 0; }
+
 void batchnorm_backward_sums(const BnBwdCall& b) {
     const int c = b.e.c, hw = b.e.hw;
     const long long M = (long long)b.e.n * hw;
@@ -478,9 +499,11 @@
     if (!(skip_exp && b.res == nullptr && b.act == BCNN_HIP_ACT_RELU && ((hw == 3136 && c == 64) || (hw == 784 && c == 128))))
 #endif
     launch_chan_reduce<2>(f, c, hw, M, splits, part);
-    bn_bwd_finalize_kernel<<<ceil_div(c, 256), 256, 0, current_stream()>>>(part, c, splits, b.p.scales, b.s.var, b.g.dbias,
-                                                                          b.g.dscales, b.g.dmean, b.g.dvar, b.consts, b.s.mean,
-                                                                          b.p.bias, b.consts_fM > 0.f ? b.consts_fM : (float)M);
+    const BnResGrad rg = bn_res_grad_of(b);
+    const int nfin = ceil_div(c, 256);
+    bn_bwd_finalize_kernel<<<nfin + bn_res_grad_blocks(rg, 256), 256, 0, current_stream()>>>(
+        part, c, splits, b.p.scales, b.s.var, b.g.dbias, b.g.dscales, b.g.dmean, b.g.dvar, b.consts, b.s.mean, b.p.bias,
+        b.consts_fM > 0.f ? b.consts_fM : (float)M, nfin, rg);
     KERNEL_CHECK();
 }
 
@@ -501,12 +524,6 @@
     launch_chan_map(BnBwdApplyBody{a, al16(a.dy) && al16(a.dx) && al16(b.workspace) && al16(b.y)}, b.e.n, b.e.c, b.e.hw);
 }
 
-__global__ __launch_bounds__(256) void bn_residual_grad_kernel(const float* __restrict__ out, const float* __restrict__ dout,
-                                                               float* __restrict__ dres, unsigned count, int act) {
-    for (unsigned i = blockIdx.x * 256u + threadIdx.x; i < count; i += gridDim.x * 256u)
-        dres[i] += dout[i] * act_bwd_cheap(out[i], act, 0.f);
-}
-
 void batchnorm_backward_impl(const BnBwdCall& call) {
     BnBwdCall b = call;
     const int c = b.e.c, hw = b.e.hw;
@@ -517,19 +534,16 @@
     KTimer kt(K_BN_BWD, 0.0, 4.0 * (b.dout ? 5.0 : b.sums ? (reads_y ? 4.0 : 3.0) : (reads_y ? 7.0 : 5.0)) * (double)total);
     if (b.dout) {
         b.res_count = b.res_count < (size_t)total ? b.res_count : (size_t)total;
-        if (b.dres && b.res_count) {
-            bn_residual_grad_kernel<<<stream_grid(b.res_count, 256), 256, 0, current_stream()>>>(b.y, b.dout, b.dres,
-                                                                                                 (unsigned)b.res_count, b.act);
-            KERNEL_CHECK();
-        }
     } else if (!act_bwd_is_cheap(b.act)) {
         bcnn_hip_activation_backward(b.y, b.dy, (size_t)total, b.act, nullptr, nullptr, hw, c);
         b.act = BCNN_HIP_ACT_NONE;
     }
     b.consts = bn_consts_scratch(c);
     if (b.sums) {
-        bn_bwd_finalize_wide_kernel<<<c, 1024, 0, current_stream()>>>(b.sums, c, b.splits, b.p.scales, b.s.var, b.g.dbias, b.g.dscales,
-                                                                      b.g.dmean, b.g.dvar, b.consts, b.s.mean, b.p.bias, (float)M);
+        const BnResGrad rg = bn_res_grad_of(b);
+        bn_bwd_finalize_wide_kernel<<<c + bn_res_grad_blocks(rg, 1024), 1024, 0, current_stream()>>>(
+            b.sums, c, b.splits, b.p.scales, b.s.var, b.g.dbias, b.g.dscales, b.g.dmean, b.g.dvar, b.consts, b.s.mean, b.p.bias,
+            (float)M, rg);
         KERNEL_CHECK();
     } else {
         batchnorm_backward_sums(b);
@@ -557,7 +571,7 @@
                                           const float* saved_var, float* dmean, float* dvar, int c) {
     if (c <= 0 || splits <= 0) return;
     bn_bwd_finalize_wide_kernel<<<c, 1024, 0, current_stream()>>>(sums, c, splits, scales, saved_var, dbias, dscales, dmean,
-                                                                  dvar, nullptr, nullptr, nullptr, 1.0f);
+                                                                  dvar, nullptr, nullptr, nullptr, 1.0f, BnResGrad{});
     KERNEL_CHECK();
 }
 
diff --git a/bcnn_amd/csrc/fc.hip b/bcnn_amd/csrc/fc.hip
--- /dev/null
+++ b/bcnn_amd/csrc/fc.hip
@@ -0,0 +1,236 @@
+#include "common.h"
+
+namespace bcnn_hip {
+
+constexpr int FC_T = 32;
+constexpr int FC_BK = 128;
+constexpr int FC_LD = 36;
+constexpr int FC_LDS_FLOATS = 2 * FC_BK * FC_LD;
+
+struct FcOperand {
+    const float* p;
+    long long ld;
+    int R;
+};
+
+template <bool KC, bool VEC>
+__device__ __forceinline__ void fc_load(const FcOperand& o, int r0, int k0, int K, float4 (&v)[4]) {
+    const int t = threadIdx.x;
+#pragma unroll
+    for (int i = 0; i < 4; ++i) {
+        int r, k;
+        if (KC) {
+            const int l = t & 63, chunk = (t >> 6) + 4 * i;
+            r = r0 + (l >> 3) + 8 * (chunk & 3);
+            k = k0 + 4 * ((l & 7) + 8 * (chunk >> 2));
+        } else {
+            const int idx = t + 256 * i;
+            k = k0 + (idx >> 3);
+            r = r0 + 4 * (idx & 7);
+        }
+        const float* src = KC ? o.p + (long long)r * o.ld + k : o.p + (long long)k * o.ld + r;
+        const int lim = KC ? K - k : o.R - r;
+        const bool row_ok = KC ? r < o.R : k < K;
+        float4 q = make_float4(0.f, 0.f, 0.f, 0.f);
+        if (row_ok && lim > 0) {
+            if (VEC) {
+                q = *reinterpret_cast<const float4*>(src);
+            } else {
+                q.x = src[0];
+                if (lim > 1) q.y = src[1];
+                if (lim > 2) q.z = src[2];
+                if (lim > 3) q.w = src[3];
+            }
+        }
+        v[i] = q;
+    }
+}
+
+template <bool KC>
+__device__ __forceinline__ void fc_stage(float* tile, const float4 (&v)[4]) {
+    const int t = threadIdx.x;
+#pragma unroll
+    for (int i = 0; i < 4; ++i) {
+        if (KC) {
+            const int l = t & 63, chunk = (t >> 6) + 4 * i;
+            const int r = (l >> 3) + 8 * (chunk & 3), k = 4 * ((l & 7) + 8 * (chunk >> 2));
+            tile[(k + 0) * FC_LD + r] = v[i].x;
+            tile[(k + 1) * FC_LD + r] = v[i].y;
+            tile[(k + 2) * FC_LD + r] = v[i].z;
+            tile[(k + 3) * FC_LD + r] = v[i].w;
+        } else {
+            const int idx = t + 256 * i;
+            *reinterpret_cast<float4*>(tile + (idx >> 3) * FC_LD + 4 * (idx & 7)) = v[i];
+        }
+    }
+}
+
+enum { FC_EPI_BIAS_ACT = 0, FC_EPI_ACCUM = 1 };
+
+template <bool A_KC, bool B_KC, bool VEC, int EPI>
+__device__ __forceinline__ void fc_tile(const FcOperand A, const FcOperand B, int K, int m0, int n0, float* out, int ldo,
+                                        const float* bias, int act, float* lds) {
+    float* As = lds;
+    float* Bs = lds + FC_BK * FC_LD;
+    const int t = threadIdx.x, lane = t & 63, wave = t >> 6;
+    const int mi = 4 * (lane >> 3), ni = 4 * (lane & 7);
+    float acc[4][4];
+#pragma unroll
+    for (int i = 0; i < 4; ++i)
+#pragma unroll
+        for (int j = 0; j < 4; ++j) acc[i][j] = 0.f;
+    float4 ra[4], rb[4];
+    fc_load<A_KC, VEC>(A, m0, 0, K, ra);
+    fc_load<B_KC, VEC>(B, n0, 0, K, rb);
+    for (int k0 = 0; k0 < K; k0 += FC_BK) {
+        fc_stage<A_KC>(As, ra);
+        fc_stage<B_KC>(Bs, rb);
+        __syncthreads();
+        if (k0 + FC_BK < K) {
+            fc_load<A_KC, VEC>(A, m0, k0 + FC_BK, K, ra);
+            fc_load<B_KC, VEC>(B, n0, k0 + FC_BK, K, rb);
+        }
+        const float* pa = As + wave * (FC_BK / 4) * FC_LD + mi;
+        const float* pb = Bs + wave * (FC_BK / 4) * FC_LD + ni;
+#pragma unroll 8
+        for (int k = 0; k < FC_BK / 4; ++k) {
+            const float4 a = *reinterpret_cast<const float4*>(pa + k * FC_LD);
+            const float4 b = *reinterpret_cast<const float4*>(pb + k * FC_LD);
+            const float av[4] = {a.x, a.y, a.z, a.w}, bv[4] = {b.x, b.y, b.z, b.w};
+#pragma unroll
+            for (int i = 0; i < 4; ++i)
+#pragma unroll
+                for (int j = 0; j < 4; ++j) acc[i][j] = __builtin_fmaf(av[i], bv[j], acc[i][j]);
+        }
+        __syncthreads();
+    }
+    float* red = lds;
+#pragma unroll
+    for (int i = 0; i < 4; ++i)
+        *reinterpret_cast<float4*>(red + (wave * FC_T + mi + i) * FC_LD + ni) =
+            make_float4(acc[i][0], acc[i][1], acc[i][2], acc[i][3]);
+    __syncthreads();
+    const int m = t >> 3, nq = 4 * (t & 7);
+    const float4 s0 = *reinterpret_cast<const float4*>(red + (0 * FC_T + m) * FC_LD + nq);
+    const float4 s1 = *reinterpret_cast<const float4*>(red + (1 * FC_T + m) * FC_LD + nq);
+    const float4 s2 = *reinterpret_cast<const float4*>(red + (2 * FC_T + m) * FC_LD + nq);
+    const float4 s3 = *reinterpret_cast<const float4*>(red + (3 * FC_T + m) * FC_LD + nq);
+    float s[4] = {((s0.x + s1.x) + s2.x) + s3.x, ((s0.y + s1.y) + s2.y) + s3.y, ((s0.z + s1.z) + s2.z) + s3.z,
+                  ((s0.w + s1.w) + s2.w) + s3.w};
+    __syncthreads();
+    const int gm = m0 + m, gn = n0 + nq;
+    if (gm >= A.R || gn >= B.R) return;
+    float* po = out + (long long)gm * ldo + gn;
+    const int cnt = min(4, B.R - gn);
+    if (VEC) {
+        float4 o;
+        if (EPI == FC_EPI_BIAS_ACT) {
+            const float4 bq = *reinterpret_cast<const float4*>(bias + gn);
+            o.x = act_fwd_cheap(s[0] + bq.x, act, 0.f); o.y = act_fwd_cheap(s[1] + bq.y, act, 0.f);
+            o.z = act_fwd_cheap(s[2] + bq.z, act, 0.f); o.w = act_fwd_cheap(s[3] + bq.w, act, 0.f);
+        } else {
+            o = *reinterpret_cast<const float4*>(po);
+            o.x += s[0]; o.y += s[1]; o.z += s[2]; o.w += s[3];
+        }
+        *reinterpret_cast<float4*>(po) = o;
+    } else {
+        for (int j = 0; j < cnt; ++j)
+            po[j] = EPI == FC_EPI_BIAS_ACT ? act_fwd_cheap(s[j] + bias[gn + j], act, 0.f) : po[j] + s[j];
+    }
+}
+
+struct FcArgs {
+    const float *x, *w, *bias, *dy;
+    float *y, *dbias, *dw, *dx;
+    int B, S, P, act;
+    int tiles_b, tiles_s, tiles_p;
+    int n_dx, n_dw;
+};
+
+template <bool VEC>
+__global__ __launch_bounds__(256) void fc_forward_kernel(const FcArgs a) {
+    __shared__ __attribute__((aligned(16))) float lds[FC_LDS_FLOATS];
+    const int tb = blockIdx.x % a.tiles_b, tp = blockIdx.x / a.tiles_b;
+    fc_tile<true, true, VEC, FC_EPI_BIAS_ACT>(FcOperand{a.x, a.S, a.B}, FcOperand{a.w, a.S, a.P}, a.S, tb * FC_T, tp * FC_T, a.y,
+                                              a.P, a.bias, a.act, lds);
+}
+
+template <bool VEC>
+__global__ __launch_bounds__(256) void fc_backward_kernel(const FcArgs a) {
+    __shared__ __attribute__((aligned(16))) float lds[FC_LDS_FLOATS];
+    int blk = blockIdx.x;
+    if (blk < a.n_dx) {
+        const int tb = blk % a.tiles_b, ts = blk / a.tiles_b;
+        fc_tile<true, false, VEC, FC_EPI_ACCUM>(FcOperand{a.dy, a.P, a.B}, FcOperand{a.w, a.S, a.S}, a.P, tb * FC_T, ts * FC_T,
+                                                a.dx, a.S, nullptr, 0, lds);
+        return;
+    }
+    blk -= a.n_dx;
+    if (blk < a.n_dw) {
+        const int ts = blk % a.tiles_s, tp = blk / a.tiles_s;
+        fc_tile<false, false, VEC, FC_EPI_ACCUM>(FcOperand{a.dy, a.P, a.P}, FcOperand{a.x, a.S, a.S}, a.B, tp * FC_T, ts * FC_T,
+                                                 a.dw, a.S, nullptr, 0, lds);
+        return;
+    }
+    blk -= a.n_dw;
+    const int col = blk * 64 + (threadIdx.x & 63), g = threadIdx.x >> 6;
+    float sum = 0.f;
+    if (col < a.P)
+        for (int b = g; b < a.B; b += 4) sum += a.dy[(long long)b * a.P + col];
+    lds[threadIdx.x] = sum;
+    __syncthreads();
+    if (g == 0 && col < a.P)
+        a.dbias[col] += ((lds[threadIdx.x] + lds[threadIdx.x + 64]) + lds[threadIdx.x + 128]) + lds[threadIdx.x + 192];
+}
+
+static bool fc_shape_ok(int B, int S, int P) {
+    return B > 0 && S > 0 && P > 0 && (long long)B * P < (1ll << 30) && (long long)P * S < (1ll << 30) &&
+           (long long)B * S < (1ll << 30);
+}
+
+}
+
+using namespace bcnn_hip;
+
+extern "C" {
+
+void bcnn_hip_fc_forward(const float* x, const float* w, const float* bias, float* y, int B, int S, int P, int act) {
+    if (B <= 0 || P <= 0) return;
+    const int fused = (act_is_cheap(act) && act != BCNN_HIP_ACT_PRELU) ? act : BCNN_HIP_ACT_NONE;
+    if (fc_shape_ok(B, S, P) && al16(x) && al16(w) && al16(bias) && al16(y)) {
+        FcArgs a{};
+        a.x = x; a.w = w; a.bias = bias; a.y = y; a.B = B; a.S = S; a.P = P; a.act = fused;
+        a.tiles_b = ceil_div(B, FC_T); a.tiles_p = ceil_div(P, FC_T);
+        const unsigned grid = (unsigned)a.tiles_b * (unsigned)a.tiles_p;
+        if (S % 4 == 0 && P % 4 == 0) fc_forward_kernel<true><<<grid, 256, 0, current_stream()>>>(a);
+        else fc_forward_kernel<false><<<grid, 256, 0, current_stream()>>>(a);
+        KERNEL_CHECK();
+        if (fused != act) bcnn_hip_activation_forward(y, (size_t)B * P, act, nullptr, 1, P);
+        return;
+    }
+    bcnn_hip_gemm(0, 1, B, P, S, 1.0f, x, S, w, S, 0.0f, y, P);
+    bcnn_hip_add_rowvec(y, bias, B, P);
+    bcnn_hip_activation_forward(y, (size_t)B * P, act, nullptr, 1, P);
+}
+
+void bcnn_hip_fc_backward(const float* x, const float* w, const float* dy, float* dbias, float* dw, float* dx_or_null, int B,
+                          int S, int P) {
+    if (B <= 0 || P <= 0) return;
+    if (fc_shape_ok(B, S, P) && al16(x) && al16(w) && al16(dy) && al16(dbias) && al16(dw) && al16(dx_or_null)) {
+        FcArgs a{};
+        a.x = x; a.w = w; a.dy = dy; a.dbias = dbias; a.dw = dw; a.dx = dx_or_null; a.B = B; a.S = S; a.P = P;
+        a.tiles_b = ceil_div(B, FC_T); a.tiles_s = ceil_div(S, FC_T); a.tiles_p = ceil_div(P, FC_T);
+        a.n_dx = dx_or_null ? a.tiles_b * a.tiles_s : 0;
+        a.n_dw = a.tiles_p * a.tiles_s;
+        const unsigned grid = (unsigned)a.n_dx + (unsigned)a.n_dw + (unsigned)ceil_div(P, 64);
+        if (S % 4 == 0 && P % 4 == 0) fc_backward_kernel<true><<<grid, 256, 0, current_stream()>>>(a);
+        else fc_backward_kernel<false><<<grid, 256, 0, current_stream()>>>(a);
+        KERNEL_CHECK();
+        return;
+    }
+    bcnn_hip_grad_bias(dbias, dy, B, P, 1);
+    bcnn_hip_gemm(1, 0, P, S, B, 1.0f, dy, P, x, S, 1.0f, dw, S);
+    if (dx_or_null) bcnn_hip_gemm(0, 0, B, S, P, 1.0f, dy, P, w, S, 1.0f, dx_or_null, S);
+}
+
+}
diff --git a/bcnn_amd/csrc/next.hip b/bcnn_amd/csrc/next.hip
--- a/bcnn_amd/csrc/next.hip
+++ b/bcnn_amd/csrc/next.hip
@@ -177,6 +177,90 @@
     out[0] = (float)(metric == 3 ? t / per : t);
 }
 
+constexpr int kSoftmaxCostStage = 1024;
+__global__ __launch_bounds__(256) void softmax_cost_kernel(int metric, const float* __restrict__ x,
+                                                           const float* __restrict__ label, float* __restrict__ y,
+                                                           float* __restrict__ grad, int B, int C,
+                                                           double* __restrict__ partials) {
+    __shared__ double red[4];
+    __shared__ float sx[4][kSoftmaxCostStage], sl[4][kSoftmaxCostStage];
+    const int lane = threadIdx.x & 63, wid = threadIdx.x >> 6;
+    const int nwaves = gridDim.x * 4;
+    const bool staged = C <= kSoftmaxCostStage;
+    double acc = 0.0;
+    for (int t = blockIdx.x * 4 + wid; t < B; t += nwaves) {
+        const float* px = x + (size_t)t * C;
+        const float* pl = label + (size_t)t * C;
+        float* py = y + (size_t)t * C;
+        float* pg = grad + (size_t)t * C;
+        if (staged) {
+            for (int c = lane; c < C; c += 64) { sx[wid][c] = px[c]; sl[wid][c] = pl[c]; }
+            px = sx[wid];
+            pl = sl[wid];
+        }
+        float vmax = -FLT_MAX;
+        for (int c = lane; c < C; c += 64) vmax = fmaxf(vmax, px[c]);
+#pragma unroll
+        for (int o = 32; o > 0; o >>= 1) vmax = fmaxf(vmax, __shfl_xor(vmax, o));
+        double part = 0.0;
+        for (int c = lane; c < C; c += 64) part += (double)(float)exp((double)(px[c] - vmax));
+#pragma unroll
+        for (int o = 32; o > 0; o >>= 1) part += __shfl_xor(part, o);
+        float sum = (float)part;
+        sum = (sum != 0.f) ? vmax + (float)log((double)sum) : vmax - 100.0f;
+        float pm = FLT_MIN;
+        int best = 0, dn = 0, dd = 0;
+        for (int c = lane; c < C; c += 64) {
+            const float p = (float)exp((double)(px[c] - sum)), l = pl[c];
+            const float g = p + -1.0f * l;
+            py[c] = p;
+            pg[c] = g;
+            if (metric == 0) {
+                if (p > pm) { pm = p; best = c; }
+            } else if (metric == 5) {
+                const float th = p > 0.5f ? 1.f : 0.f;
+                dn += (int)(l * th);
+                dd += (int)(l + th);
+            } else if (metric == 1) {
+                if (l > 0.0f) {
+                    const float q = p < 1e-8f ? 1e-8f : (p > 1.0f - 1e-8f ? 1.0f - 1e-8f : p);
+                    acc += -log((double)q);
+                }
+            } else {
+                acc += (double)g * g;
+            }
+        }
+        if (metric == 0) {
+#pragma unroll
+            for (int off = 32; off > 0; off >>= 1) {
+                const float om = __shfl_xor(pm, off);
+                const int ob = __shfl_xor(best, off);
+                if (om > pm || (om == pm && ob < best)) { pm = om; best = ob; }
+            }
+            if (lane == 0 && label[(size_t)t * C + best] == 0) acc += 1.0;
+        } else if (metric == 5) {
+#pragma unroll
+            for (int off = 32; off > 0; off >>= 1) { dn += __shfl_xor(dn, off); dd += __shfl_xor(dd, off); }
+            if (lane == 0) acc += (2.0f * dn + 1.0f) / (dd + 1.0f);
+        }
+    }
+#pragma unroll
+    for (int off = 32; off > 0; off >>= 1) acc += __shfl_xor(acc, off);
+    if (lane == 0) red[wid] = acc;
+    __syncthreads();
+    if (threadIdx.x == 0) partials[blockIdx.x] = ((red[0] + red[1]) + red[2]) + red[3];
+}
+
+__global__ __launch_bounds__(256) void softmax_cost_bwd_kernel(float scale, const float* __restrict__ dcost,
+                                                               float* __restrict__ dpred, float* __restrict__ dx, size_t n) {
+    const size_t stride = (size_t)gridDim.x * blockDim.x;
+    for (size_t i = (size_t)blockIdx.x * blockDim.x + threadIdx.x; i < n; i += stride) {
+        const float g = dpred[i] + scale * dcost[i];
+        dpred[i] = g;
+        if (dx) dx[i] += g;
+    }
+}
+
 }
 
 using namespace bcnn_hip;
@@ -248,4 +332,24 @@
     KERNEL_CHECK();
 }
 
-}
+void bcnn_hip_softmax_cost_forward(int metric, const float* x, const float* label, float* pred, float* grad, int batch,
+                                   int c, float* out) {
+    if (batch <= 0 || c <= 0) return;
+    trace_kernel("softmax_cost:fwd");
+    int blocks = (batch + 3) / 4;
+    if (blocks > 64) blocks = 64;
+    double* partials = reinterpret_cast<double*>(scratch(SCRATCH_REDUCE, 2 * 64));
+    softmax_cost_kernel<<<blocks, 256, 0, current_stream()>>>(metric, x, label, pred, grad, batch, c, partials);
+    KERNEL_CHECK();
+    cost_metric_final_kernel<<<1, 1, 0, current_stream()>>>(metric, partials, blocks, c, out);
+    KERNEL_CHECK();
+}
+
+void bcnn_hip_softmax_cost_backward(size_t n, float scale, const float* dcost, float* dpred, float* dx_or_null) {
+    if (!n) return;
+    trace_kernel("softmax_cost:bwd");
+    softmax_cost_bwd_kernel<<<stream_grid(n, 256), 256, 0, current_stream()>>>(scale, dcost, dpred, dx_or_null, n);
+    KERNEL_CHECK();
+}
+
+}
diff --git a/bcnn_amd/csrc/runtime.hip b/bcnn_amd/csrc/runtime.hip
--- a/bcnn_amd/csrc/runtime.hip
+++ b/bcnn_amd/csrc/runtime.hip
@@ -189,6 +189,25 @@
     HIP_CHECK(hipStreamSynchronize(current_stream()));
 }
 
+void* bcnn_hip_host_alloc(size_t bytes) {
+    void* p = nullptr;
+    if (bytes == 0) return nullptr;
+    warm_device_keeping_rand_state();
+    HIP_CHECK(hipHostMalloc(&p, bytes, hipHostMallocDefault));
+    memset(p, 0, bytes);
+    return p;
+}
+
+void bcnn_hip_host_free(void* p) {
+    if (p) HIP_CHECK(hipHostFree(p));
+}
+
+void bcnn_hip_memcpy_d2h_pinned(void* pinned_dst, const void* src, size_t bytes, void* event) {
+    HIP_CHECK(hipMemcpyAsync(pinned_dst, src, bytes, hipMemcpyDeviceToHost, current_stream()));
+    HIP_CHECK(hipEventRecord((hipEvent_t)event, current_stream()));
+    HIP_CHECK(hipEventSynchronize((hipEvent_t)event));
+}
+
 void bcnn_hip_memcpy_d2d(void* dst, const void* src, size_t bytes) {
     HIP_CHECK(hipMemcpyAsync(dst, src, bytes, hipMemcpyDeviceToDevice, current_stream()));
 }
diff --git a/bcnn_amd/host/bcnn_core.c b/bcnn_amd/host/bcnn_core.c
--- a/bcnn_amd/host/bcnn_core.c
+++ b/bcnn_amd/host/bcnn_core.c
@@ -427,6 +427,7 @@
     bcnn_link_conv_maxpool(net);
     bcnn_link_conv_depthwise(net);
     bcnn_link_batchnorm_conv(net);
+    bcnn_link_softmax_cost(net);
     if (hc->fill_chunks_gpu) {
         bcnn_hip_sync();
         bcnn_hip_free(hc->fill_chunks_gpu);
diff --git a/bcnn_amd/host/bcnn_internal.h b/bcnn_amd/host/bcnn_internal.h
--- a/bcnn_amd/host/bcnn_internal.h
+++ b/bcnn_amd/host/bcnn_internal.h
@@ -330,6 +330,11 @@
     float *lifted_workspace_gpu;
     size_t lifted_workspace_size;
     void *lifted_record_gpu;
+    float *loss_staging;
+    void *loss_event;
+    int softmax_node;
+    int pair_forward;
+    int pair_backward_done;
 #endif
 } bcnn_cost_param;
 
@@ -433,6 +438,7 @@
 uint64_t bcnn_dropout_key(uint64_t seed, int node, int rank);
 
 void bcnn_link_depthwise_batchnorm(bcnn_net *net);
+void bcnn_link_softmax_cost(bcnn_net *net);
 void bcnn_link_conv_eltwise(bcnn_net *net);
 void bcnn_link_conv_maxpool(bcnn_net *net);
 void bcnn_link_conv_depthwise(bcnn_net *net);
diff --git a/bcnn_amd/host/bcnn_layers_next.c b/bcnn_amd/host/bcnn_layers_next.c
--- a/bcnn_amd/host/bcnn_layers_next.c
+++ b/bcnn_amd/host/bcnn_layers_next.c
@@ -144,9 +144,7 @@
     bcnn_tensor *x = &net->tensors[node->src[0]], *w = &net->tensors[node->src[1]];
     bcnn_tensor *b = &net->tensors[node->src[2]], *y = &net->tensors[node->dst[0]];
     const int B = y->n, S = bcnn_tensor_size3d(x), P = y->c;
-    bcnn_hip_gemm(0, 1, B, P, S, 1.0f, x->data_gpu, S, w->data_gpu, S, 0.0f, y->data_gpu, P);
-    bcnn_hip_add_rowvec(y->data_gpu, b->data_gpu, B, P);
-    bcnn_hip_activation_forward(y->data_gpu, (size_t)B * P, (int)p->activation, NULL, 1, P);
+    bcnn_hip_fc_forward(x->data_gpu, w->data_gpu, b->data_gpu, y->data_gpu, B, S, P, (int)p->activation);
 }
 
 void bcnn_backward_fullc_layer(bcnn_net *net, bcnn_node *node) {
@@ -155,10 +153,8 @@
     bcnn_tensor *b = &net->tensors[node->src[2]], *y = &net->tensors[node->dst[0]];
     const int B = y->n, S = bcnn_tensor_size3d(x), P = y->c;
     bcnn_hip_activation_backward(y->data_gpu, y->grad_data_gpu, (size_t)B * P, (int)p->activation, NULL, NULL, 1, P);
-    bcnn_hip_grad_bias(b->grad_data_gpu, y->grad_data_gpu, B, P, 1);
-    bcnn_hip_gemm(1, 0, P, S, B, 1.0f, y->grad_data_gpu, P, x->data_gpu, S, 1.0f, w->grad_data_gpu, S);
-    if (x->grad_data_gpu)
-        bcnn_hip_gemm(0, 0, B, S, P, 1.0f, y->grad_data_gpu, P, w->data_gpu, S, 1.0f, x->grad_data_gpu, S);
+    bcnn_hip_fc_backward(x->data_gpu, w->data_gpu, y->grad_data_gpu, b->grad_data_gpu, w->grad_data_gpu, x->grad_data_gpu, B, S,
+                         P);
 }
 
 void bcnn_update_fullc_layer(bcnn_net *net, bcnn_node *node) {
@@ -191,13 +187,43 @@
     return BCNN_SUCCESS;
 }
 
+static bcnn_cost_param *paired_cost(bcnn_net *net, bcnn_node *node) {
+    if (node < net->nodes || node >= net->nodes + net->num_nodes) return NULL;
+    const int i = (int)(node - net->nodes);
+    if (i + 1 >= net->num_nodes || net->nodes[i + 1].type != BCNN_LAYER_COST) return NULL;
+    bcnn_cost_param *cp = (bcnn_cost_param *)net->nodes[i + 1].param;
+    return cp->softmax_node == i ? cp : NULL;
+}
+
+static int host_cost_metric(void) {
+    static int host_loop = -1;
+    if (host_loop < 0) host_loop = BCNN_EXP_ENV("BCNN_HOST_COST_METRIC") != NULL;
+    return host_loop;
+}
+
+static int pair_runs_forward(bcnn_net *net, const bcnn_node *cost) {
+    const bcnn_tensor *label = &net->tensors[1], *dst = &net->tensors[cost->dst[0]];
+    return hctx(net)->in_pass == 1 && net->mode == BCNN_MODE_TRAIN && label->data && label->data_gpu && dst->grad_data_gpu &&
+           !host_cost_metric();
+}
+
 void bcnn_forward_softmax_layer(bcnn_net *net, bcnn_node *node) {
     bcnn_tensor *x = &net->tensors[node->src[0]], *y = &net->tensors[node->dst[0]];
+    bcnn_cost_param *cp = paired_cost(net, node);
+    if (cp && pair_runs_forward(net, node + 1)) {
+        cp->pair_forward = 1;
+        return;
+    }
     bcnn_hip_softmax_forward(x->data_gpu, y->data_gpu, x->n, x->c, x->h * x->w);
 }
 
 void bcnn_backward_softmax_layer(bcnn_net *net, bcnn_node *node) {
     bcnn_tensor *x = &net->tensors[node->src[0]], *y = &net->tensors[node->dst[0]];
+    bcnn_cost_param *cp = paired_cost(net, node);
+    if (cp && cp->pair_backward_done) {
+        cp->pair_backward_done = 0;
+        return;
+    }
     if (x->grad_data_gpu) bcnn_hip_axpy((size_t)bcnn_tensor_size(x), 1.0f, y->grad_data_gpu, x->grad_data_gpu);
 }
 
@@ -222,6 +248,7 @@
     bcnn_cost_param *param = (bcnn_cost_param *)calloc(1, node.param_size);
     node.param = param;
     param->scale = scale; param->loss = loss; param->loss_metric = loss_metric;
+    param->softmax_node = -1;
     node.forward = bcnn_forward_cost_layer;
     node.backward = bcnn_backward_cost_layer;
     node.release_param = bcnn_release_param_cost_layer;
@@ -274,11 +301,28 @@
     return 0.f;
 }
 
+static void read_back_metric(bcnn_cost_param *p, bcnn_tensor *dst) {
+    if (!p->loss_staging) {
+        p->loss_staging = (float *)bcnn_hip_host_alloc(sizeof(float));
+        p->loss_event = bcnn_hip_event_create();
+    }
+    bcnn_hip_memcpy_d2h_pinned(p->loss_staging, dst->data_gpu, sizeof(float), p->loss_event);
+    dst->data[0] = p->loss_staging[0];
+}
+
 void bcnn_forward_cost_layer(bcnn_net *net, bcnn_node *node) {
     bcnn_cost_param *p = (bcnn_cost_param *)node->param;
     bcnn_tensor *pred = &net->tensors[node->src[0]], *label = &net->tensors[1], *dst = &net->tensors[node->dst[0]];
     if (!label->data) return;
     const size_t sz = (size_t)bcnn_tensor_size(pred);
+    if (p->pair_forward) {
+        bcnn_tensor *x = &net->tensors[net->nodes[p->softmax_node].src[0]];
+        p->pair_forward = 0;
+        bcnn_hip_softmax_cost_forward((int)p->loss_metric, x->data_gpu, label->data_gpu, pred->data_gpu, dst->grad_data_gpu,
+                                      pred->n, pred->c, dst->data_gpu);
+        read_back_metric(p, dst);
+        return;
+    }
     if (p->loss == BCNN_LOSS_LIFTED_STRUCT) {
         if (pred->grad_data_gpu && label->data_gpu && net->mode != BCNN_MODE_PREDICT) {
             const size_t need = bcnn_hip_lifted_struct_workspace_size(pred->n, pred->c);
@@ -298,9 +342,7 @@
         bcnn_hip_axpy(sz, -1.0f, label->data_gpu, dst->grad_data_gpu);
     }
     if (net->mode == BCNN_MODE_PREDICT) return;
-    static int host_loop = -1;
-    if (host_loop < 0) host_loop = BCNN_EXP_ENV("BCNN_HOST_COST_METRIC") != NULL;
-    if (host_loop || !label->data_gpu || !dst->grad_data_gpu) {
+    if (host_cost_metric() || !label->data_gpu || !dst->grad_data_gpu) {
         if (dst->grad_data_gpu) bcnn_hip_memcpy_d2h(dst->grad_data, dst->grad_data_gpu, sz * sizeof(float));
         bcnn_hip_memcpy_d2h(pred->data, pred->data_gpu, sz * sizeof(float));
         dst->data[0] = host_metric(p, pred, label, dst);
@@ -309,7 +351,7 @@
     }
     bcnn_hip_cost_metric((int)p->loss_metric, pred->data_gpu, label->data_gpu, dst->grad_data_gpu, pred->n,
                          pred->w * pred->h * pred->c, dst->data_gpu);
-    bcnn_hip_memcpy_d2h(dst->data, dst->data_gpu, sizeof(float));
+    read_back_metric(p, dst);
 }
 
 void bcnn_backward_cost_layer(bcnn_net *net, bcnn_node *node) {
@@ -321,14 +363,49 @@
                                             (const bcnn_hip_lifted_struct_record *)p->lifted_record_gpu);
         return;
     }
-    if (pred->grad_data_gpu)
-        bcnn_hip_axpy((size_t)bcnn_tensor_size(pred), p->scale, dst->grad_data_gpu, pred->grad_data_gpu);
+    if (!pred->grad_data_gpu) return;
+    if (p->softmax_node >= 0 && hctx(net)->in_pass == 2) {
+        bcnn_tensor *x = &net->tensors[net->nodes[p->softmax_node].src[0]];
+        bcnn_hip_softmax_cost_backward((size_t)bcnn_tensor_size(pred), p->scale, dst->grad_data_gpu, pred->grad_data_gpu,
+                                       x->grad_data_gpu);
+        p->pair_backward_done = 1;
+        return;
+    }
+    bcnn_hip_axpy((size_t)bcnn_tensor_size(pred), p->scale, dst->grad_data_gpu, pred->grad_data_gpu);
 }
 
 void bcnn_release_param_cost_layer(bcnn_node *node) {
     bcnn_cost_param *p = (bcnn_cost_param *)node->param;
     bcnn_hip_free(p->lifted_workspace_gpu);
     bcnn_hip_free(p->lifted_record_gpu);
+    bcnn_hip_host_free(p->loss_staging);
+    bcnn_hip_event_destroy(p->loss_event);
+}
+
+void bcnn_link_softmax_cost(bcnn_net *net) {
+    for (int i = 0; i < net->num_nodes; ++i) {
+        if (net->nodes[i].type != BCNN_LAYER_COST) continue;
+        bcnn_cost_param *cp = (bcnn_cost_param *)net->nodes[i].param;
+        cp->softmax_node = -1;
+        cp->pair_forward = cp->pair_backward_done = 0;
+    }
+    if (BCNN_EXP_ENV("BCNN_NO_NODE_FUSION")) return;
+    for (int c = 1; c < net->num_nodes; ++c) {
+        bcnn_node *cn = &net->nodes[c], *sn = &net->nodes[c - 1];
+        if (cn->type != BCNN_LAYER_COST || sn->type != BCNN_LAYER_SOFTMAX) continue;
+        bcnn_cost_param *cp = (bcnn_cost_param *)cn->param;
+        const int t = sn->dst[0];
+        if (cp->loss != BCNN_LOSS_EUCLIDEAN || cn->src[0] != t || sn->src[0] == t || cn->dst[0] == t) continue;
+        int writers = 0, consumers = 0;
+        for (int i = 0; i < net->num_nodes; ++i) {
+            for (int k = 0; k < net->nodes[i].num_dst; ++k) writers += net->nodes[i].dst[k] == t;
+            for (int k = 0; k < net->nodes[i].num_src; ++k) consumers += net->nodes[i].src[k] == t;
+        }
+        if (writers != 1 || consumers != 1) continue;
+        const bcnn_tensor *pred = &net->tensors[t], *x = &net->tensors[sn->src[0]];
+        if (pred->h * pred->w != 1 || bcnn_tensor_size(pred) != bcnn_tensor_size(x)) continue;
+        cp->softmax_node = c - 1;
+    }
 }
 
 bcnn_status bcnn_get_lifted_struct_loss(bcnn_net *net, float *loss, int *num_constraints) {
diff --git a/include/bcnn_hip.h b/include/bcnn_hip.h
--- a/include/bcnn_hip.h
+++ b/include/bcnn_hip.h
@@ -25,6 +25,9 @@
 void bcnn_hip_memcpy_h2d(void *dst_d, const void *src_h, size_t bytes);
 void bcnn_hip_memcpy_d2h(void *dst_h, const void *src_d, size_t bytes);
 void bcnn_hip_memcpy_d2d(void *dst_d, const void *src_d, size_t bytes);
+void *bcnn_hip_host_alloc(size_t bytes);
+void bcnn_hip_host_free(void *p);
+void bcnn_hip_memcpy_d2h_pinned(void *pinned_dst, const void *src_d, size_t bytes, void *event);
 void bcnn_hip_fill_f32(float *x_d, size_t n, float value);
 void bcnn_hip_sync(void);
 void *bcnn_hip_stream_create(void);
@@ -65,6 +68,11 @@
                      int stride, float *col_d);
 void bcnn_hip_col2im(const float *col_d, int channels, int height, int width, int ksize, int pad,
                      int stride, float *im_d);
+
+void bcnn_hip_fc_forward(const float *x_d, const float *w_d, const float *bias_d, float *y_d, int B, int S, int P,
+                         int act);
+void bcnn_hip_fc_backward(const float *x_d, const float *w_d, const float *dy_d, float *dbias_d, float *dw_d,
+                          float *dx_or_null_d, int B, int S, int P);
 
 void bcnn_hip_activation_forward(float *x_d, size_t size, int act, const float *slopes_d,
                                  int spatial, int channels);
@@ -265,6 +273,9 @@
                            int min_h, int min_w);
 void bcnn_hip_add_rowvec(float *y_d, const float *v_d, int rows, int cols);
 void bcnn_hip_softmax_forward(const float *x_d, float *y_d, int n, int c, int hw);
+void bcnn_hip_softmax_cost_forward(int metric, const float *x_d, const float *label_d, float *pred_d, float *grad_d,
+                                   int batch, int c, float *out_d);
+void bcnn_hip_softmax_cost_backward(size_t n, float scale, const float *dcost_d, float *dpred_d, float *dx_or_null_d);
 
 void bcnn_hip_concat_forward(int num_src, const float *const *src_d, const int *src_size3d, float *dst_d,
                              int dst_size3d, int n);
```

After: 14220 images/s, median of 6. About the same (+0.5%).
